# jaredhuling/oem

Measured on AMD Instinct MI355X. Metric: full-lambda-path solves/sec (n=1e6 p=100 lasso, 100 lambdas, tol 1e-10), higher is better.
Workload: dtype f64; 1 GPU; config 1: oem() lasso (penalty='elastic.net', alpha=1), dense Gaussian X~N(0,9), intercept, no standardize, 100-lambda path supplied, tol 1e-10 (README benchmark); n=1000000, p=100, nlambda=100, rows_per_gpu=1000000

## Files before the change

### include/oemgpu.h

```cpp
#ifndef OEMGPU_H
#define OEMGPU_H

#include <stdint.h>

#ifdef __cplusplus
extern "C" {
#endif

#define OEMGPU_OK              0
#define OEMGPU_ERR_ARG        -1
#define OEMGPU_ERR_NO_DEVICE  -2
#define OEMGPU_ERR_HIP        -3
#define OEMGPU_ERR_UNSUPPORTED -4
#define OEMGPU_ERR_INTERNAL   -5
#define OEMGPU_ERR_INTERRUPTED -6

enum {
    OEMGPU_ELASTIC_NET = 0, OEMGPU_LASSO = 1, OEMGPU_OLS = 2, OEMGPU_MCP = 3, OEMGPU_SCAD = 4,
    OEMGPU_MCP_NET = 5, OEMGPU_SCAD_NET = 6, OEMGPU_GRP_LASSO = 7, OEMGPU_GRP_LASSO_NET = 8,
    OEMGPU_GRP_MCP = 9, OEMGPU_GRP_SCAD = 10, OEMGPU_GRP_MCP_NET = 11, OEMGPU_GRP_SCAD_NET = 12,
    OEMGPU_SPARSE_GRP_LASSO = 13, OEMGPU_NPENALTIES = 14
};

typedef struct oemgpu_opts {
// ... 103 lines not shown
int oemgpu_fit_dense_rm_dev(oemgpu_ctx *ctx, const void *x_dev, int32_t dtype, int64_t n, int64_t ldr, int32_t p, const double *y_dev,
                            int32_t standardize, int32_t intercept, const oemgpu_opts *o,
                            double *beta, double *lambda_out, int32_t *niter, double *loss, double *d);
int oemgpu_selftest_gram_rm_plan(int64_t n, int32_t p, int32_t num_cu, int64_t *out );

int oemgpu_fit_dense_multi_dev(oemgpu_ctx *ctx, const double *x_dev, int64_t n, int64_t ld, int32_t p,
                               const double *y_dev, int64_t y_rs, int64_t y_cs, int32_t m,
                               int32_t standardize, int32_t intercept, const oemgpu_opts *o,
                               double *beta, double *lambda_out, int32_t *niter, double *loss, double *d, int32_t *route);
int oemgpu_fit_dense_multi_rm_dev(oemgpu_ctx *ctx, const void *x_dev, int32_t dtype, int64_t n, int64_t ldr, int32_t p,
                                  const double *y_dev, int64_t y_rs, int64_t y_cs, int32_t m,
                                  int32_t standardize, int32_t intercept, const oemgpu_opts *o,
                                  double *beta, double *lambda_out, int32_t *niter, double *loss, double *d, int32_t *route);
int oemgpu_selftest_multi_plan(int64_t n, int32_t p, int32_t m, int32_t npen, int32_t layout, int32_t num_cu, int64_t *out );
int oemgpu_selftest_multi_moments_dev(oemgpu_ctx *ctx, const void *x_dev, int32_t dtype, int64_t n, int64_t ld, int32_t p,
                                      const double *y_dev, int64_t y_rs, int64_t y_cs, int32_t m, double *moments_out_dev);

int oemgpu_fit_dense_weighted_dev(oemgpu_ctx *ctx, const double *x_dev, int64_t n, int64_t ld, int32_t p, const double *y_dev,
                                  const double *weights_dev, int32_t standardize, int32_t intercept, const oemgpu_opts *opts,
                                  double *beta, double *lambda_out, int32_t *niter, double *loss, double *d);

int oemgpu_fit_xtx_dev(oemgpu_ctx *ctx, const double *xtx_dev, const double *xty_dev, int32_t p,
                       const double *scale_factor, const oemgpu_opts *o,
                       double *beta, double *lambda_out, int32_t *niter, double *loss, double *d);

int oemgpu_last_shift_advised(oemgpu_ctx *ctx);

int oemgpu_xval_dense_dev(oemgpu_ctx *ctx, const double *x_dev, int64_t n, int64_t ld, int32_t p, const double *y_dev,
                          const double *weights_dev , const int32_t *foldid_dev, int32_t nfolds, int32_t standardize, int32_t intercept,
                          int32_t type_measure, const oemgpu_opts *o,
                          double *beta, double *lambda_out, int32_t *niter, double *loss, double *d,
                          double *cvm, double *cvsd);

int64_t oemgpu_xval_moments_len(int32_t p, int32_t nfolds, int32_t weighted);
int oemgpu_xval_fold_moments_dev(oemgpu_ctx *ctx, const double *x_dev, int64_t n_local, int64_t ld, int32_t p, const double *y_dev,
                                 const double *weights_dev , const int32_t *foldid_dev, int32_t nfolds, const oemgpu_opts *o,
                                 double *fold_moments_dev, int64_t *fold_n);
int oemgpu_xval_solve_folds_dev(oemgpu_ctx *ctx, const double *fold_moments_dev, const int64_t *fold_n_total, int64_t n_local, int32_t p,
                                int32_t nfolds, int32_t weighted, int32_t standardize, int32_t intercept, const oemgpu_opts *o,
                                double *beta, double *lambda_out, int32_t *niter, double *loss, double *d);
int oemgpu_xval_cv_triples_dev(oemgpu_ctx *ctx, int64_t n_local, int32_t p, int32_t nfolds, int32_t weighted, int32_t type_measure,
                               const oemgpu_opts *o, double *triples);
int oemgpu_xval_merge(const double *triples, int32_t nsets, const oemgpu_opts *o, double *cvm, double *cvsd);

int oemgpu_selftest_xval_cv_error_dev(oemgpu_ctx *ctx, const double *x_dev, int64_t n, int64_t ld, int32_t p, const double *y_dev,
                                      const double *weights_dev , const int32_t *foldid_dev, int32_t nfolds,
                                      const double *coef, int32_t npen, int32_t nl, int32_t type_measure, double *cvm, double *cvsd,
                                      double *triples );
int oemgpu_cv_fold_fits_dev(oemgpu_ctx *ctx, const double *x_dev, int64_t n, int64_t ld, int32_t p, const double *y_dev,
                            const int32_t *foldid_dev, int32_t nfolds, int32_t standardize, int32_t intercept, const oemgpu_opts *o,
                            double *beta, double *lambda_out, int32_t *niter, double *loss, double *d, int64_t *fold_n);
int oemgpu_cv_score_dev(oemgpu_ctx *ctx, int64_t n, int32_t p, int32_t nfolds, const double *coef, int32_t npen, int32_t nl,
                        const int32_t *ncol, int32_t type_measure, double *triples, double *predmat_dev );
int oemgpu_selftest_cv_score_dev(oemgpu_ctx *ctx, const double *x_dev, int64_t n, int64_t ld, int32_t p, const double *y_dev,
                                 const int32_t *foldid_dev, int32_t nfolds, const double *coef, int32_t npen, int32_t nl,
                                 const int32_t *ncol, int32_t type_measure, double *triples, double *predmat_dev );
int oemgpu_xval_dense_rm_dev(oemgpu_ctx *ctx, const void *x_dev, int32_t dtype, int64_t n, int64_t ldr, int32_t p, const double *y_dev,
                             const double *weights_dev , const int32_t *foldid_dev, int32_t nfolds, int32_t standardize,
                             int32_t intercept, int32_t type_measure, const oemgpu_opts *o,
                             double *beta, double *lambda_out, int32_t *niter, double *loss, double *d,
                             double *cvm, double *cvsd);
int oemgpu_cv_fold_fits_rm_dev(oemgpu_ctx *ctx, const void *x_dev, int32_t dtype, int64_t n, int64_t ldr, int32_t p, const double *y_dev,
                               const int32_t *foldid_dev, int32_t nfolds, int32_t standardize, int32_t intercept, const oemgpu_opts *o,
                               double *beta, double *lambda_out, int32_t *niter, double *loss, double *d, int64_t *fold_n);
int oemgpu_selftest_fold_gather_rm_dev(oemgpu_ctx *ctx, const void *x_dev, int32_t dtype, int64_t n, int64_t ldr, int32_t p,
                                       const double *y_dev, const int32_t *foldid_dev, int32_t nfolds, double *xo_dev, int64_t ldo,
                                       double *yo_dev, int64_t *fold_n, int64_t *fold_start);
int oemgpu_selftest_xval_cv_plan(int64_t n, int32_t p, int32_t nfolds, int32_t npen, int32_t nl, int32_t num_cu, int64_t *out );

int oemgpu_xval_dense_multi_dev(oemgpu_ctx *ctx, const double *x_dev, int64_t n, int64_t ld, int32_t p,
                                const double *y_dev, int64_t y_rs, int64_t y_cs, int32_t m,
                                const int32_t *foldid_dev, int32_t nfolds, int32_t standardize, int32_t intercept,
                                int32_t type_measure, const oemgpu_opts *o,
                                double *beta, double *lambda_out, int32_t *niter, double *loss, double *d,
                                double *cvm, double *cvsd, int32_t *route);
int oemgpu_xval_dense_multi_rm_dev(oemgpu_ctx *ctx, const void *x_dev, int32_t dtype, int64_t n, int64_t ldr, int32_t p,
                                   const double *y_dev, int64_t y_rs, int64_t y_cs, int32_t m,
                                   const int32_t *foldid_dev, int32_t nfolds, int32_t standardize, int32_t intercept,
                                   int32_t type_measure, const oemgpu_opts *o,
                                   double *beta, double *lambda_out, int32_t *niter, double *loss, double *d,
                                   double *cvm, double *cvsd, int32_t *route);
#define OEMGPU_XVM_NPHASES 6
int oemgpu_last_xval_multi_timings(double *ms );
#define OEMGPU_XVM_PLAN_LEN 20
int oemgpu_selftest_xval_multi_plan(int64_t n, int32_t p, int32_t nfolds, int32_t m, int32_t npen, int32_t nl, int32_t num_cu,
                                    int64_t *out );
int oemgpu_selftest_xval_multi_fold_moments_dev(oemgpu_ctx *ctx, const void *x_dev, int32_t dtype, int64_t n, int64_t ld, int32_t p,
                                                const double *y_dev, int64_t y_rs, int64_t y_cs, int32_t m,
                                                const int32_t *foldid_dev, int32_t nfolds, double *moments_out_dev);

int oemgpu_last_eigen_info(oemgpu_ctx *ctx, int32_t *steps, int32_t *capped);

enum {
    OEMGPU_ENGINE_NONE = 0,
    OEMGPU_ENGINE_ROWS = 1,
    OEMGPU_ENGINE_COOP = 2,
    OEMGPU_ENGINE_ROWCOOP = 3,
    OEMGPU_ENGINE_SYMCOOP = 4,
    OEMGPU_ENGINE_LAUNCHES = 5,
    OEMGPU_ENGINE_WCOOP = 6,
    OEMGPU_ENGINE_WRES = 7,
    OEMGPU_ENGINE_WSTREAM = 8,
    OEMGPU_ENGINE_WLAUNCHES = 9,
    OEMGPU_ENGINE_SPARSE_WIDE = 10
};
int oemgpu_last_path_engine(oemgpu_ctx *ctx, int32_t *engine, int32_t *persistent_fallbacks);
int oemgpu_last_host_path_engine(int32_t *engine);
int oemgpu_last_placement(oemgpu_ctx *ctx);

int oemgpu_last_path_rounds(oemgpu_ctx *ctx, int64_t *short_rounds, int64_t *rounds);

int oemgpu_last_shift_in_effect(oemgpu_ctx *ctx);

int oemgpu_eig_max_dev(oemgpu_ctx *ctx, const double *a_dev, int32_t p, double *lambda_max);

#define OEMGPU_T_SHIFT   0
#define OEMGPU_T_MOMENTS 1
#define OEMGPU_T_FINAL   2
#define OEMGPU_T_EIGPATH 3
#define OEMGPU_T_GRAMK   4
#define OEMGPU_T_FOLDORDER 5
#define OEMGPU_T_PATHCYC 6
#define OEMGPU_T_PATHTICKS 7
#define OEMGPU_NTIMERS   8
int oemgpu_last_timings(oemgpu_ctx *ctx, double *ms );
int oemgpu_set_timing(oemgpu_ctx *ctx, int32_t on);

void oemgpu_row_split(int64_t n, int32_t G, int32_t g, int64_t *r0, int64_t *r1);

#define OEMGPU_NHOSTSTATS 9
int oemgpu_last_host_stats(double *out );

void oemgpu_release_cache(void);

int oemgpu_selftest_wcoop_sizing(int32_t n, int32_t p, int32_t npen, int32_t num_cu);

int oemgpu_selftest_plan(int32_t p, int32_t q, int32_t semantics, int32_t intercept, const oemgpu_opts *o, int32_t has_scale, int32_t nbatch,
                         int64_t wide_n, int32_t num_cu, int32_t *engine, int64_t *frame_bytes, int64_t *reserved_bytes,
                         int64_t *scratch_need_doubles, int64_t *scratch_have_doubles);

int oemgpu_selftest_gram_plan(int64_t n, int32_t p, int32_t num_cu, int64_t *out );

enum {
    OEMGPU_GRAM_FORM_TRI = 0,
    OEMGPU_GRAM_FORM_RING_SADDR = 1,
    OEMGPU_GRAM_FORM_RING_LANE = 2,
    OEMGPU_GRAM_FORM_SB = 3,
    OEMGPU_GRAM_FORM_WD3 = 4,
    OEMGPU_GRAM_FORM_WD4 = 5,
    OEMGPU_GRAM_FORM_WD_UNITS = 6,
    OEMGPU_GRAM_FORM_BLK = 7
};
int oemgpu_selftest_gram_form(int64_t n, int64_t ld, int32_t p, int32_t aligned, int32_t num_cu, int64_t *out );

int oemgpu_fit_logistic_dense(const double *x, int64_t n, int32_t p, const double *y, int32_t standardize, int32_t intercept,
                              int32_t hessian_full, int32_t irls_maxit, double irls_tol, const oemgpu_opts *opts,
                              double *beta, double *lambda_out, int32_t *niter, double *loss, double *d);
int oemgpu_fit_logistic_dense_dev(oemgpu_ctx *ctx, const double *x_dev, int64_t n, int64_t ld, int32_t p, const double *y_dev,
                                  int32_t standardize, int32_t intercept, int32_t hessian_full, int32_t irls_maxit, double irls_tol,
                                  const oemgpu_opts *opts, double *beta, double *lambda_out, int32_t *niter, double *loss, double *d);
int oemgpu_fit_logistic_dense_fold_dev(oemgpu_ctx *ctx, const double *x_dev, int64_t n, int64_t ld, int32_t p, const double *y_dev,
                                       const int32_t *foldid_dev, int32_t nfolds, int32_t leave_out, int32_t standardize, int32_t intercept,
                                       int32_t hessian_full, int32_t irls_maxit, double irls_tol, const oemgpu_opts *opts,
                                       double *beta, double *lambda_out, int32_t *niter, double *loss, double *d);
int oemgpu_logistic_cv_score_dev(oemgpu_ctx *ctx, const double *x_dev, int64_t n, int64_t ld, int32_t p, const double *y_dev, double y_hi,
                                 const int32_t *foldid_dev, int32_t nfolds, const double *coef, int32_t ncol, double *sums, int64_t *counts,
                                 double *predmat_dev);
int oemgpu_selftest_cv_score_plan(int64_t n, int32_t p, int32_t ncol, int32_t num_cu, int64_t *out );
int oemgpu_logistic_cv_auc_dev(oemgpu_ctx *ctx, const double *predmat_dev, int64_t n, int32_t ncol, const double *y_dev, double y_hi,
                               const int32_t *foldid_dev, int32_t nfolds, int64_t *u, int64_t *n1, int64_t *n0);
int oemgpu_selftest_cv_auc_plan(int64_t n, int32_t nfolds, int32_t ncol, int32_t num_cu, int64_t longest_fold, int64_t *out );
int oemgpu_selftest_logistic_plan(int64_t n, int32_t p, int32_t intercept, int32_t hessian_full, int32_t num_cu, int64_t *out );
int oemgpu_fit_logistic_dense_rm_dev(oemgpu_ctx *ctx, const void *x_dev, int32_t dtype, int64_t n, int64_t ldr, int32_t p, const double *y_dev,
                                     int32_t standardize, int32_t intercept, int32_t hessian_full, int32_t irls_maxit, double irls_tol,
                                     const oemgpu_opts *opts, double *beta, double *lambda_out, int32_t *niter, double *loss, double *d);
int oemgpu_fit_logistic_dense_fold_rm_dev(oemgpu_ctx *ctx, const void *x_dev, int32_t dtype, int64_t n, int64_t ldr, int32_t p, const double *y_dev,
                                          const int32_t *foldid_dev, int32_t nfolds, int32_t leave_out, int32_t standardize, int32_t intercept,
                                          int32_t hessian_full, int32_t irls_maxit, double irls_tol, const oemgpu_opts *opts,
                                          double *beta, double *lambda_out, int32_t *niter, double *loss, double *d);
int oemgpu_logistic_cv_score_rm_dev(oemgpu_ctx *ctx, const void *x_dev, int32_t dtype, int64_t n, int64_t ldr, int32_t p, const double *y_dev,
                                    double y_hi, const int32_t *foldid_dev, int32_t nfolds, const double *coef, int32_t ncol, double *sums,
                                    int64_t *counts, double *predmat_dev);
int oemgpu_selftest_logistic_rm_plan(int64_t n, int32_t p, int32_t dtype, int32_t intercept, int32_t num_cu, int64_t *out );
int oemgpu_fit_logistic_sparse(int64_t n, int32_t p, const int64_t *colptr, const int32_t *rowidx, const double *values, const double *y,
                               int32_t standardize, int32_t intercept, int32_t irls_maxit, double irls_tol, const oemgpu_opts *opts,
                               double *beta, double *lambda_out, int32_t *niter, double *loss, double *d);
int oemgpu_selftest_logistic_sparse_plan(int64_t n, int32_t p, int64_t nnz, int32_t intercept, int32_t num_cu, int64_t *out );
typedef struct oemgpu_sparse_x oemgpu_sparse_x;
int oemgpu_sparse_x_create(oemgpu_ctx *ctx, int64_t n, int32_t p, const int64_t *colptr, const int32_t *rowidx, const double *values,
                           oemgpu_sparse_x **out);
void oemgpu_sparse_x_destroy(oemgpu_sparse_x *x);
int64_t oemgpu_sparse_x_bytes(const oemgpu_sparse_x *x);
#define OEMGPU_SPARSE_CSC 0
#define OEMGPU_SPARSE_CSR 1
#define OEMGPU_I32 0
#define OEMGPU_I64 1
int oemgpu_sparse_x_create_dev(oemgpu_ctx *ctx, int64_t n, int32_t p, int32_t layout, const void *ptr_dev, int32_t ptr_dtype,
                               const void *idx_dev, int32_t idx_dtype, const void *val_dev, int32_t val_dtype, int64_t nnz,
                               oemgpu_sparse_x **out);
int oemgpu_selftest_sparse_build_plan(int64_t n, int32_t p, int64_t nnz, int32_t layout, int32_t num_cu, int64_t *out );
int oemgpu_sparse_x_export(const oemgpu_sparse_x *x, int64_t *colptr, int32_t *rowidx, double *val, int64_t *rowptr, int32_t *ccol,
                           double *cval, int32_t *cptr);
int oemgpu_sparse_x_dims(const oemgpu_sparse_x *x, int64_t *out );
int oemgpu_last_sparse_build_timings(double *ms );
int oemgpu_fit_sparse_res(oemgpu_ctx *ctx, const oemgpu_sparse_x *x, const double *y_dev, int32_t standardize, int32_t intercept,
                          const oemgpu_opts *opts, double *beta, double *lambda_out, int32_t *niter, double *loss, double *d);
int oemgpu_xval_sparse_res(oemgpu_ctx *ctx, const oemgpu_sparse_x *x, const double *y_dev, const int32_t *foldid_dev, int32_t nfolds,
                           int32_t standardize, int32_t intercept, int32_t type_measure, const oemgpu_opts *opts, double *beta,
                           double *lambda_out, int32_t *niter, double *loss, double *d, double *cvm, double *cvsd);
int oemgpu_fit_logistic_sparse_fold_res(oemgpu_ctx *ctx, const oemgpu_sparse_x *x, const double *y_dev, const int32_t *foldid_dev, int32_t nfolds,
                                        int32_t leave_out, int32_t standardize, int32_t intercept, int32_t irls_maxit, double irls_tol,
                                        const oemgpu_opts *opts, double *beta, double *lambda_out, int32_t *niter, double *loss, double *d);
int oemgpu_fit_sparse_wide_res(oemgpu_ctx *ctx, const oemgpu_sparse_x *x, const double *y_dev, int32_t standardize, const oemgpu_opts *opts,
                               double *beta, double *lambda_out, int32_t *niter, double *loss, double *d);
int oemgpu_selftest_sparse_wide_plan(int64_t n, int32_t p, int64_t nnz, int64_t longest_row, int64_t longest_col, int32_t num_cu,
                                     int64_t *out );
int oemgpu_fit_sparse_wide_fold_res(oemgpu_ctx *ctx, const oemgpu_sparse_x *x, const double *y_dev, const int32_t *foldid_dev, int32_t nfolds,
                                    int32_t leave_out, int32_t standardize, const oemgpu_opts *opts, double *beta, double *lambda_out,
                                    int32_t *niter, double *loss, double *d, int64_t *kept);
enum { OEMGPU_SPW_PASS_ROWS = 0, OEMGPU_SPW_PASS_COLS = 1, OEMGPU_SPW_PASS_STATS = 2, OEMGPU_SPW_PASS_LOSS = 3 };
int oemgpu_selftest_sparse_wide_pass(oemgpu_ctx *ctx, const oemgpu_sparse_x *x, int32_t pass, int32_t row_lanes, int32_t col_lanes,
                                     const int32_t *foldid_dev, int32_t nfolds, int32_t leave_out, int32_t standardize, double scale,
                                     const double *in_dev, const double *coef_dev, int32_t ncoef, double *out_dev, double *out2_dev,
                                     double *stats_dev, int64_t *info , int32_t *long_rows, int32_t *long_cols);
int oemgpu_cv_sparse_wide_score_res(oemgpu_ctx *ctx, const oemgpu_sparse_x *x, const double *y_dev, const int32_t *foldid_dev, int32_t nfolds,
                                    const double *coef, int32_t npen, int32_t nl, const int32_t *ncol, int32_t type_measure, double *triples,
                                    double *predmat_dev );
int oemgpu_selftest_cv_sparse_wide_score_plan(int64_t n, int32_t p, int32_t nfolds, int32_t npen, int32_t nl, int32_t num_cu,
                                              int64_t *out );
int oemgpu_logistic_cv_score_sparse_res(oemgpu_ctx *ctx, const oemgpu_sparse_x *x, const double *y_dev, double y_hi, const int32_t *foldid_dev,
                                        int32_t nfolds, const double *coef, int32_t ncol, double *sums, int64_t *counts, double *predmat_dev);
int oemgpu_selftest_logistic_sparse_res_plan(int64_t n, int32_t p, int64_t nnz, int32_t intercept, int32_t num_cu, int64_t *out );
int oemgpu_cv_sparse_fold_fits_res(oemgpu_ctx *ctx, const oemgpu_sparse_x *x, const double *y_dev, const int32_t *foldid_dev, int32_t nfolds,
                                   int32_t standardize, int32_t intercept, const oemgpu_opts *opts,
                                   double *beta, double *lambda_out, int32_t *niter, double *loss, double *d, int64_t *fold_n);
int oemgpu_cv_sparse_score_res(oemgpu_ctx *ctx, int64_t n, int32_t p, int32_t nfolds, const double *coef, int32_t npen, int32_t nl,
                               const int32_t *ncol, int32_t type_measure, double *triples, double *predmat_dev );
int oemgpu_selftest_cv_sparse_score(oemgpu_ctx *ctx, const oemgpu_sparse_x *x, const double *y_dev, const int32_t *foldid_dev, int32_t nfolds,
                                    const double *coef, int32_t npen, int32_t nl, const int32_t *ncol, int32_t type_measure, double *triples,
                                    double *predmat_dev );
int oemgpu_selftest_cv_sparse_plan(int64_t n, int32_t p, int64_t nnz, int32_t nfolds, int32_t npen, int32_t nl, int32_t num_cu,
                                   int64_t *out );
int oemgpu_selftest_csc_plan(int64_t n, int32_t p, int64_t *out );
int oemgpu_last_logistic_stats(double *out );

int oemgpu_predict_dev(oemgpu_ctx *ctx, const double *x_dev, int64_t n, int64_t ld, int32_t p, const double *coef, int32_t ncol, int32_t type,
                       double *out_dev);
int oemgpu_predict_rm_dev(oemgpu_ctx *ctx, const void *x_dev, int32_t dtype, int64_t n, int64_t ldr, int32_t p, const double *coef, int32_t ncol,
                          int32_t type, double *out_dev);
int oemgpu_predict_sparse_res(oemgpu_ctx *ctx, const oemgpu_sparse_x *x, const double *coef, int32_t ncol, int32_t type, double *out_dev);
int oemgpu_selftest_predict_plan(int64_t n, int32_t p, int32_t ncol, int32_t layout, int32_t num_cu, int64_t *out );

int oemgpu_selftest_hold_cus(oemgpu_ctx *ctx, int32_t blocks, double ms);

int oemgpu_selftest_group_permutation(const oemgpu_opts *o, int32_t q, int32_t *perm);

int oemgpu_selftest_symcoop_owners(int32_t q, int32_t num_cu, const int32_t *runs, int32_t nruns, int32_t *owner_c0, int32_t *owner_n, int32_t *frag,
                                   int32_t *nowners, int32_t *split);

int oemgpu_selftest_coop_slots(int32_t num_cu, int32_t W, int32_t ninst, int32_t calls, int32_t *bases, int32_t *peak);

int oemgpu_selftest_sympk_gemv(oemgpu_ctx *ctx, const double *xx_dev, int32_t q, const double *vec_dev, double *out_dev, int32_t reps,
                               double *us_per_product);

void        oemgpu_reload_switches(void);
const char *oemgpu_switch_names(void);

const char *oemgpu_last_error(void);
const char *oemgpu_version(void);
int         oemgpu_device_count(void);

#ifdef __cplusplus
}
#endif
#endif
```

### oem_amd/_lib.py

```python
import ctypes as C
import os
from pathlib import Path

_HERE = Path(__file__).resolve().parent
LIB_PATH = Path(os.environ.get("OEMGPU_LIB", _HERE / "liboemgpu.so"))

_dp = C.POINTER(C.c_double)
_ip = C.POINTER(C.c_int32)

PENALTIES = ["elastic.net", "lasso", "ols", "mcp", "scad", "mcp.net", "scad.net",
             "grp.lasso", "grp.lasso.net", "grp.mcp", "grp.scad", "grp.mcp.net",
             "grp.scad.net", "sparse.grp.lasso"]

OEMGPU_SEM_DENSE, OEMGPU_SEM_BIG = 0, 1
OEMGPU_F64, OEMGPU_F32 = 0, 1
OEMGPU_SPARSE_CSC, OEMGPU_SPARSE_CSR = 0, 1
OEMGPU_I32, OEMGPU_I64 = 0, 1
RM_P_MAX = 1024
ERR_INTERRUPTED = -6
NHOSTSTATS = 9
NTIMERS = 8
T_SHIFT, T_MOMENTS, T_FINAL, T_EIGPATH, T_GRAMK = 0, 1, 2, 3, 4


# ... 34 lines not shown
                                                 C.c_int32, C.c_int32, C.c_double, C.POINTER(OemgpuOpts)] + _OUT),
    "oemgpu_fit_logistic_dense_fold_dev": (C.c_int, [C.c_void_p, C.c_void_p, C.c_int64, C.c_int64, C.c_int32, C.c_void_p, C.c_void_p, C.c_int32,
                                                      C.c_int32, C.c_int32, C.c_int32, C.c_int32, C.c_int32, C.c_double, C.POINTER(OemgpuOpts)] + _OUT),
    "oemgpu_logistic_cv_score_dev": (C.c_int, [C.c_void_p, C.c_void_p, C.c_int64, C.c_int64, C.c_int32, C.c_void_p, C.c_double, C.c_void_p, C.c_int32,
                                                _dp, C.c_int32, _dp, C.POINTER(C.c_int64), C.c_void_p]),
    "oemgpu_fit_logistic_dense_rm_dev": (C.c_int, [C.c_void_p, C.c_void_p, C.c_int32, C.c_int64, C.c_int64, C.c_int32, C.c_void_p, C.c_int32, C.c_int32,
                                                    C.c_int32, C.c_int32, C.c_double, C.POINTER(OemgpuOpts)] + _OUT),
    "oemgpu_fit_logistic_dense_fold_rm_dev": (C.c_int, [C.c_void_p, C.c_void_p, C.c_int32, C.c_int64, C.c_int64, C.c_int32, C.c_void_p, C.c_void_p,
                                                         C.c_int32, C.c_int32, C.c_int32, C.c_int32, C.c_int32, C.c_int32, C.c_double,
                                                         C.POINTER(OemgpuOpts)] + _OUT),
    "oemgpu_logistic_cv_score_rm_dev": (C.c_int, [C.c_void_p, C.c_void_p, C.c_int32, C.c_int64, C.c_int64, C.c_int32, C.c_void_p, C.c_double, C.c_void_p,
                                                   C.c_int32, _dp, C.c_int32, _dp, C.POINTER(C.c_int64), C.c_void_p]),
    "oemgpu_selftest_logistic_rm_plan": (C.c_int, [C.c_int64, C.c_int32, C.c_int32, C.c_int32, C.c_int32, C.POINTER(C.c_int64)]),
    "oemgpu_selftest_cv_score_plan": (C.c_int, [C.c_int64, C.c_int32, C.c_int32, C.c_int32, C.POINTER(C.c_int64)]),
    "oemgpu_logistic_cv_auc_dev": (C.c_int, [C.c_void_p, C.c_void_p, C.c_int64, C.c_int32, C.c_void_p, C.c_double, C.c_void_p, C.c_int32,
                                              C.POINTER(C.c_int64), C.POINTER(C.c_int64), C.POINTER(C.c_int64)]),
    "oemgpu_selftest_cv_auc_plan": (C.c_int, [C.c_int64, C.c_int32, C.c_int32, C.c_int32, C.c_int64, C.POINTER(C.c_int64)]),
    "oemgpu_selftest_logistic_plan": (C.c_int, [C.c_int64, C.c_int32, C.c_int32, C.c_int32, C.c_int32, C.POINTER(C.c_int64)]),
    "oemgpu_fit_logistic_sparse": (C.c_int, [C.c_int64, C.c_int32, C.c_void_p, C.c_void_p, C.c_void_p, C.c_void_p, C.c_int32, C.c_int32, C.c_int32, C.c_double,
                                              C.POINTER(OemgpuOpts)] + _OUT),
    "oemgpu_selftest_logistic_sparse_plan": (C.c_int, [C.c_int64, C.c_int32, C.c_int64, C.c_int32, C.c_int32, C.POINTER(C.c_int64)]),
    "oemgpu_selftest_logistic_sparse_res_plan": (C.c_int, [C.c_int64, C.c_int32, C.c_int64, C.c_int32, C.c_int32, C.POINTER(C.c_int64)]),
    "oemgpu_sparse_x_create": (C.c_int, [C.c_void_p, C.c_int64, C.c_int32, C.c_void_p, C.c_void_p, C.c_void_p, C.POINTER(C.c_void_p)]),
    "oemgpu_sparse_x_destroy": (None, [C.c_void_p]),
    "oemgpu_sparse_x_bytes": (C.c_int64, [C.c_void_p]),
    "oemgpu_sparse_x_create_dev": (C.c_int, [C.c_void_p, C.c_int64, C.c_int32, C.c_int32, C.c_void_p, C.c_int32, C.c_void_p, C.c_int32, C.c_void_p,
                                             C.c_int32, C.c_int64, C.POINTER(C.c_void_p)]),
    "oemgpu_selftest_sparse_build_plan": (C.c_int, [C.c_int64, C.c_int32, C.c_int64, C.c_int32, C.c_int32, C.POINTER(C.c_int64)]),
    "oemgpu_sparse_x_export": (C.c_int, [C.c_void_p] + [C.c_void_p] * 7),
    "oemgpu_sparse_x_dims": (C.c_int, [C.c_void_p, C.POINTER(C.c_int64)]),
    "oemgpu_last_sparse_build_timings": (C.c_int, [_dp]),
    "oemgpu_fit_sparse_res": (C.c_int, [C.c_void_p, C.c_void_p, C.c_void_p, C.c_int32, C.c_int32, C.POINTER(OemgpuOpts)] + _OUT),
    "oemgpu_xval_sparse_res": (C.c_int, [C.c_void_p, C.c_void_p, C.c_void_p, C.c_void_p, C.c_int32, C.c_int32, C.c_int32, C.c_int32,
                                         C.POINTER(OemgpuOpts)] + _OUT + [_dp, _dp]),
    "oemgpu_fit_logistic_sparse_fold_res": (C.c_int, [C.c_void_p, C.c_void_p, C.c_void_p, C.c_void_p, C.c_int32, C.c_int32, C.c_int32, C.c_int32, C.c_int32,
                                                       C.c_double, C.POINTER(OemgpuOpts)] + _OUT),
    "oemgpu_logistic_cv_score_sparse_res": (C.c_int, [C.c_void_p, C.c_void_p, C.c_void_p, C.c_double, C.c_void_p, C.c_int32, _dp, C.c_int32, _dp,
                                                       C.POINTER(C.c_int64), C.c_void_p]),
    "oemgpu_predict_dev": (C.c_int, [C.c_void_p, C.c_void_p, C.c_int64, C.c_int64, C.c_int32, _dp, C.c_int32, C.c_int32, C.c_void_p]),
    "oemgpu_predict_rm_dev": (C.c_int, [C.c_void_p, C.c_void_p, C.c_int32, C.c_int64, C.c_int64, C.c_int32, _dp, C.c_int32, C.c_int32, C.c_void_p]),
    "oemgpu_predict_sparse_res": (C.c_int, [C.c_void_p, C.c_void_p, _dp, C.c_int32, C.c_int32, C.c_void_p]),
    "oemgpu_selftest_predict_plan": (C.c_int, [C.c_int64, C.c_int32, C.c_int32, C.c_int32, C.c_int32, C.POINTER(C.c_int64)]),
    "oemgpu_selftest_csc_plan": (C.c_int, [C.c_int64, C.c_int32, C.POINTER(C.c_int64)]),
    "oemgpu_last_logistic_stats": (C.c_int, [_dp]),
    "oemgpu_fit_xtx": (C.c_int, [_dp, _dp, C.c_int32, _dp, C.POINTER(OemgpuOpts)] + _OUT),
    "oemgpu_fit_big": (C.c_int, [C.POINTER(_dp), C.POINTER(C.c_int64), C.c_int32, C.c_int32, C.POINTER(_dp), C.c_int32,
                                 C.c_int32, C.POINTER(OemgpuOpts)] + _OUT),
    "oemgpu_create": (C.c_void_p, [C.c_int32, C.c_void_p]),
    "oemgpu_destroy": (None, [C.c_void_p]),
    "oemgpu_synchronize": (C.c_int, [C.c_void_p]),
    "oemgpu_shift_sums_dev": (C.c_int, [C.c_void_p, C.c_void_p, C.c_int64, C.c_int64, C.c_int32, C.c_void_p, C.c_void_p]),
    "oemgpu_moments_dev": (C.c_int, [C.c_void_p, C.c_void_p, C.c_int64, C.c_int64, C.c_int32, C.c_void_p, C.c_void_p, C.c_void_p]),
    "oemgpu_sum_in_order_dev": (C.c_int, [C.c_void_p, C.c_void_p, C.c_int32, C.c_int64, C.c_void_p]),
    "oemgpu_solve_moments_dev": (C.c_int, [C.c_void_p, C.c_void_p, C.c_void_p, C.c_int32, C.c_int32, C.c_int32, C.c_int32,
                                           C.POINTER(OemgpuOpts)] + _OUT),
    "oemgpu_fit_dense_dev": (C.c_int, [C.c_void_p, C.c_void_p, C.c_int64, C.c_int64, C.c_int32, C.c_void_p, C.c_int32,
                                       C.c_int32, C.POINTER(OemgpuOpts)] + _OUT),
    "oemgpu_shift_sums_rm_dev": (C.c_int, [C.c_void_p, C.c_void_p, C.c_int32, C.c_int64, C.c_int64, C.c_int32, C.c_void_p, C.c_void_p]),
    "oemgpu_moments_rm_dev": (C.c_int, [C.c_void_p, C.c_void_p, C.c_int32, C.c_int64, C.c_int64, C.c_int32, C.c_void_p, C.c_void_p, C.c_void_p]),
    "oemgpu_fit_dense_rm_dev": (C.c_int, [C.c_void_p, C.c_void_p, C.c_int32, C.c_int64, C.c_int64, C.c_int32, C.c_void_p, C.c_int32,
                                          C.c_int32, C.POINTER(OemgpuOpts)] + _OUT),
    "oemgpu_selftest_gram_rm_plan": (C.c_int, [C.c_int64, C.c_int32, C.c_int32, C.POINTER(C.c_int64)]),
    "oemgpu_fit_dense_multi_dev": (C.c_int, [C.c_void_p, C.c_void_p, C.c_int64, C.c_int64, C.c_int32, C.c_void_p, C.c_int64, C.c_int64, C.c_int32,
                                             C.c_int32, C.c_int32, C.POINTER(OemgpuOpts)] + _OUT + [_ip]),
    "oemgpu_fit_dense_multi_rm_dev": (C.c_int, [C.c_void_p, C.c_void_p, C.c_int32, C.c_int64, C.c_int64, C.c_int32, C.c_void_p, C.c_int64, C.c_int64,
                                                C.c_int32, C.c_int32, C.c_int32, C.POINTER(OemgpuOpts)] + _OUT + [_ip]),
    "oemgpu_selftest_multi_plan": (C.c_int, [C.c_int64, C.c_int32, C.c_int32, C.c_int32, C.c_int32, C.c_int32, C.POINTER(C.c_int64)]),
    "oemgpu_selftest_multi_moments_dev": (C.c_int, [C.c_void_p, C.c_void_p, C.c_int32, C.c_int64, C.c_int64, C.c_int32, C.c_void_p, C.c_int64, C.c_int64,
                                                    C.c_int32, C.c_void_p]),
    "oemgpu_xval_dense_multi_dev": (C.c_int, [C.c_void_p, C.c_void_p, C.c_int64, C.c_int64, C.c_int32, C.c_void_p, C.c_int64, C.c_int64, C.c_int32,
                                              C.c_void_p, C.c_int32, C.c_int32, C.c_int32, C.c_int32, C.POINTER(OemgpuOpts)] + _OUT + [_dp, _dp, _ip]),
    "oemgpu_xval_dense_multi_rm_dev": (C.c_int, [C.c_void_p, C.c_void_p, C.c_int32, C.c_int64, C.c_int64, C.c_int32, C.c_void_p, C.c_int64, C.c_int64,
                                                 C.c_int32, C.c_void_p, C.c_int32, C.c_int32, C.c_int32, C.c_int32, C.POINTER(OemgpuOpts)] + _OUT +
                                       [_dp, _dp, _ip]),
    "oemgpu_last_xval_multi_timings": (C.c_int, [_dp]),
    "oemgpu_selftest_xval_multi_plan": (C.c_int, [C.c_int64, C.c_int32, C.c_int32, C.c_int32, C.c_int32, C.c_int32, C.c_int32, C.POINTER(C.c_int64)]),
    "oemgpu_selftest_xval_multi_fold_moments_dev": (C.c_int, [C.c_void_p, C.c_void_p, C.c_int32, C.c_int64, C.c_int64, C.c_int32, C.c_void_p, C.c_int64,
                                                              C.c_int64, C.c_int32, C.c_void_p, C.c_int32, C.c_void_p]),
    "oemgpu_fit_xtx_dev": (C.c_int, [C.c_void_p, C.c_void_p, C.c_void_p, C.c_int32, _dp, C.POINTER(OemgpuOpts)] + _OUT),
    "oemgpu_last_shift_in_effect": (C.c_int, [C.c_void_p]),
    "oemgpu_last_shift_advised": (C.c_int, [C.c_void_p]),
    "oemgpu_last_eigen_info": (C.c_int, [C.c_void_p, C.POINTER(C.c_int32), C.POINTER(C.c_int32)]),
    "oemgpu_last_path_engine": (C.c_int, [C.c_void_p, C.POINTER(C.c_int32), C.POINTER(C.c_int32)]),
    "oemgpu_last_host_path_engine": (C.c_int, [C.POINTER(C.c_int32)]),
    "oemgpu_last_placement": (C.c_int, [C.c_void_p]),
    "oemgpu_last_path_rounds": (C.c_int, [C.c_void_p, C.POINTER(C.c_int64), C.POINTER(C.c_int64)]),
    "oemgpu_fit_sparse": (C.c_int, [C.c_int64, C.c_int32, C.c_void_p, C.c_void_p, C.c_void_p, C.c_void_p, C.c_int32, C.c_int32,
                                    C.POINTER(OemgpuOpts)] + _OUT),
    "oemgpu_fit_sparse_wide_res": (C.c_int, [C.c_void_p, C.c_void_p, C.c_void_p, C.c_int32, C.POINTER(OemgpuOpts)] + _OUT),
    "oemgpu_selftest_sparse_wide_plan": (C.c_int, [C.c_int64, C.c_int32, C.c_int64, C.c_int64, C.c_int64, C.c_int32, C.POINTER(C.c_int64)]),
    "oemgpu_fit_sparse_wide_fold_res": (C.c_int, [C.c_void_p, C.c_void_p, C.c_void_p, C.c_void_p, C.c_int32, C.c_int32, C.c_int32,
                                                  C.POINTER(OemgpuOpts)] + _OUT + [C.POINTER(C.c_int64)]),
    "oemgpu_selftest_sparse_wide_pass": (C.c_int, [C.c_void_p, C.c_void_p, C.c_int32, C.c_int32, C.c_int32, C.c_void_p, C.c_int32, C.c_int32, C.c_int32,
                                                   C.c_double, C.c_void_p, C.c_void_p, C.c_int32, C.c_void_p, C.c_void_p, C.c_void_p,
                                                   C.POINTER(C.c_int64), C.c_void_p, C.c_void_p]),
    "oemgpu_cv_sparse_wide_score_res": (C.c_int, [C.c_void_p, C.c_void_p, C.c_void_p, C.c_void_p, C.c_int32, _dp, C.c_int32, C.c_int32, _ip,
                                                  C.c_int32, _dp, C.c_void_p]),
    "oemgpu_selftest_cv_sparse_wide_score_plan": (C.c_int, [C.c_int64, C.c_int32, C.c_int32, C.c_int32, C.c_int32, C.c_int32, C.POINTER(C.c_int64)]),
    "oemgpu_xval_dense": (C.c_int, [C.c_void_p, C.c_int64, C.c_int32, C.c_void_p, C.c_void_p, C.c_void_p, C.c_int32, C.c_int32, C.c_int32,
                                    C.c_int32, C.POINTER(OemgpuOpts)] + _OUT + [_dp, _dp]),
    "oemgpu_xval_sparse": (C.c_int, [C.c_int64, C.c_int32, C.c_void_p, C.c_void_p, C.c_void_p, C.c_void_p, C.c_void_p, C.c_int32, C.c_int32, C.c_int32,
                                     C.c_int32, C.POINTER(OemgpuOpts)] + _OUT + [_dp, _dp]),
    "oemgpu_last_xval_sparse_timings": (C.c_int, [_dp]),
    "oemgpu_selftest_xval_sparse_plan": (C.c_int, [C.c_int64, C.c_int32, C.c_int64, C.c_int32, C.c_int32, C.c_int32, C.c_int32, C.POINTER(C.c_int64)]),
    "oemgpu_selftest_xval_sparse_fold_moments": (C.c_int, [C.c_int64, C.c_int32, C.c_void_p, C.c_void_p, C.c_void_p, C.c_void_p, C.c_void_p, C.c_int32, _dp]),
    "oemgpu_selftest_xval_sparse_cv_error": (C.c_int, [C.c_int64, C.c_int32, C.c_void_p, C.c_void_p, C.c_void_p, C.c_void_p, C.c_void_p, C.c_int32, _dp,
                                                       C.c_int32, C.c_int32, C.c_int32, _dp, _dp, _dp]),
    "oemgpu_xval_dense_dev": (C.c_int, [C.c_void_p, C.c_void_p, C.c_int64, C.c_int64, C.c_int32, C.c_void_p, C.c_void_p, C.c_void_p, C.c_int32,
                                        C.c_int32, C.c_int32, C.c_int32, C.POINTER(OemgpuOpts)] + _OUT + [_dp, _dp]),
    "oemgpu_xval_moments_len": (C.c_int64, [C.c_int32, C.c_int32, C.c_int32]),
    "oemgpu_xval_fold_moments_dev": (C.c_int, [C.c_void_p, C.c_void_p, C.c_int64, C.c_int64, C.c_int32, C.c_void_p, C.c_void_p, C.c_void_p,
                                               C.c_int32, C.POINTER(OemgpuOpts), C.c_void_p, C.POINTER(C.c_int64)]),
    "oemgpu_xval_solve_folds_dev": (C.c_int, [C.c_void_p, C.c_void_p, C.POINTER(C.c_int64), C.c_int64, C.c_int32, C.c_int32, C.c_int32,
                                              C.c_int32, C.c_int32, C.POINTER(OemgpuOpts)] + _OUT),
    "oemgpu_xval_cv_triples_dev": (C.c_int, [C.c_void_p, C.c_int64, C.c_int32, C.c_int32, C.c_int32, C.c_int32, C.POINTER(OemgpuOpts), _dp]),
    "oemgpu_selftest_xval_cv_error_dev": (C.c_int, [C.c_void_p, C.c_void_p, C.c_int64, C.c_int64, C.c_int32, C.c_void_p, C.c_void_p, C.c_void_p, C.c_int32,
                                                    _dp, C.c_int32, C.c_int32, C.c_int32, _dp, _dp, _dp]),
    "oemgpu_selftest_xval_cv_plan": (C.c_int, [C.c_int64, C.c_int32, C.c_int32, C.c_int32, C.c_int32, C.c_int32, C.POINTER(C.c_int64)]),
    "oemgpu_cv_fold_fits_dev": (C.c_int, [C.c_void_p, C.c_void_p, C.c_int64, C.c_int64, C.c_int32, C.c_void_p, C.c_void_p, C.c_int32, C.c_int32,
                                          C.c_int32, C.POINTER(OemgpuOpts)] + _OUT + [C.POINTER(C.c_int64)]),
    "oemgpu_cv_score_dev": (C.c_int, [C.c_void_p, C.c_int64, C.c_int32, C.c_int32, _dp, C.c_int32, C.c_int32, _ip, C.c_int32, _dp,
                                      C.c_void_p]),
    "oemgpu_selftest_cv_score_dev": (C.c_int, [C.c_void_p, C.c_void_p, C.c_int64, C.c_int64, C.c_int32, C.c_void_p, C.c_void_p, C.c_int32, _dp,
                                               C.c_int32, C.c_int32, _ip, C.c_int32, _dp, C.c_void_p]),
    "oemgpu_xval_dense_rm_dev": (C.c_int, [C.c_void_p, C.c_void_p, C.c_int32, C.c_int64, C.c_int64, C.c_int32, C.c_void_p, C.c_void_p, C.c_void_p,
                                           C.c_int32, C.c_int32, C.c_int32, C.c_int32, C.POINTER(OemgpuOpts)] + _OUT + [_dp, _dp]),
    "oemgpu_cv_fold_fits_rm_dev": (C.c_int, [C.c_void_p, C.c_void_p, C.c_int32, C.c_int64, C.c_int64, C.c_int32, C.c_void_p, C.c_void_p, C.c_int32,
                                             C.c_int32, C.c_int32, C.POINTER(OemgpuOpts)] + _OUT + [C.POINTER(C.c_int64)]),
    "oemgpu_selftest_fold_gather_rm_dev": (C.c_int, [C.c_void_p, C.c_void_p, C.c_int32, C.c_int64, C.c_int64, C.c_int32, C.c_void_p, C.c_void_p,
                                                     C.c_int32, C.c_void_p, C.c_int64, C.c_void_p, C.POINTER(C.c_int64), C.POINTER(C.c_int64)]),
    "oemgpu_cv_sparse_fold_fits_res": (C.c_int, [C.c_void_p, C.c_void_p, C.c_void_p, C.c_void_p, C.c_int32, C.c_int32, C.c_int32,
                                                 C.POINTER(OemgpuOpts)] + _OUT + [C.POINTER(C.c_int64)]),
    "oemgpu_cv_sparse_score_res": (C.c_int, [C.c_void_p, C.c_int64, C.c_int32, C.c_int32, _dp, C.c_int32, C.c_int32, _ip, C.c_int32, _dp,
                                             C.c_void_p]),
    "oemgpu_selftest_cv_sparse_score": (C.c_int, [C.c_void_p, C.c_void_p, C.c_void_p, C.c_void_p, C.c_int32, _dp, C.c_int32, C.c_int32, _ip,
                                                  C.c_int32, _dp, C.c_void_p]),
    "oemgpu_selftest_cv_sparse_plan": (C.c_int, [C.c_int64, C.c_int32, C.c_int64, C.c_int32, C.c_int32, C.c_int32, C.c_int32, C.POINTER(C.c_int64)]),
    "oemgpu_xval_merge": (C.c_int, [_dp, C.c_int32, C.POINTER(OemgpuOpts), _dp, _dp]),
    "oemgpu_eig_max_dev": (C.c_int, [C.c_void_p, C.c_void_p, C.c_int32, _dp]),
    "oemgpu_last_timings": (C.c_int, [C.c_void_p, _dp]),
    "oemgpu_set_timing": (C.c_int, [C.c_void_p, C.c_int32]),
    "oemgpu_row_split": (None, [C.c_int64, C.c_int32, C.c_int32, C.POINTER(C.c_int64), C.POINTER(C.c_int64)]),
    "oemgpu_last_host_stats": (C.c_int, [_dp]),
    "oemgpu_release_cache": (None, []),
    "oemgpu_selftest_hold_cus": (C.c_int, [C.c_void_p, C.c_int32, C.c_double]),
    "oemgpu_selftest_group_permutation": (C.c_int, [C.c_void_p, C.c_int32, C.POINTER(C.c_int32)]),
    "oemgpu_selftest_symcoop_owners": (C.c_int, [C.c_int32, C.c_int32, C.POINTER(C.c_int32), C.c_int32, C.POINTER(C.c_int32), C.POINTER(C.c_int32),
                                       C.POINTER(C.c_int32), C.POINTER(C.c_int32), C.POINTER(C.c_int32)]),
    "oemgpu_selftest_coop_slots": (C.c_int, [C.c_int32, C.c_int32, C.c_int32, C.c_int32, C.POINTER(C.c_int32), C.POINTER(C.c_int32)]),
    "oemgpu_selftest_sympk_gemv": (C.c_int, [C.c_void_p, C.c_void_p, C.c_int32, C.c_void_p, C.c_void_p, C.c_int32, C.POINTER(C.c_double)]),
    "oemgpu_selftest_wcoop_sizing": (C.c_int, [C.c_int32, C.c_int32, C.c_int32, C.c_int32]),
    "oemgpu_selftest_gram_plan": (C.c_int, [C.c_int64, C.c_int32, C.c_int32, C.POINTER(C.c_int64)]),
    "oemgpu_selftest_gram_form": (C.c_int, [C.c_int64, C.c_int64, C.c_int32, C.c_int32, C.c_int32, C.POINTER(C.c_int64)]),
    "oemgpu_selftest_plan": (C.c_int, [C.c_int32, C.c_int32, C.c_int32, C.c_int32, C.c_void_p, C.c_int32, C.c_int32, C.c_int64, C.c_int32,
                             C.POINTER(C.c_int32), C.POINTER(C.c_int64), C.POINTER(C.c_int64), C.POINTER(C.c_int64), C.POINTER(C.c_int64)]),
    "oemgpu_reload_switches": (None, []),
    "oemgpu_switch_names": (C.c_char_p, []),
    "oemgpu_last_error": (C.c_char_p, []),
    "oemgpu_version": (C.c_char_p, []),
    "oemgpu_device_count": (C.c_int, []),
}
EXPORTS = sorted(_SIGS)


def lib():
    global _lib
    if _lib is None:
        try:
            import torch
        except ImportError:
            pass
        if not LIB_PATH.exists():
            raise OSError(f"{LIB_PATH} is missing: build it with `python -m oem_amd.build` "
                          "(oem_amd has no CPU fallback)")
        L = C.CDLL(str(LIB_PATH))
        for name, (res, args) in _SIGS.items():
            fn = getattr(L, name)
            fn.restype = res
            fn.argtypes = args
        _lib = L
    return _lib


_env_seen = None


def sync_switches():
    global _env_seen
    cur = tuple(sorted((k, v) for k, v in os.environ.items() if k.startswith(("OEM_", "OEMGPU_"))))
    if cur != _env_seen:
        _env_seen = cur
        reload_switches()


def reload_switches():
    if _lib is not None:
        _lib.oemgpu_reload_switches()


def check(rc):
    if rc != 0:
        raise OemgpuError(rc, lib().oemgpu_last_error().decode())


def host_stats():
    out = (C.c_double * NHOSTSTATS)()
    check(lib().oemgpu_last_host_stats(out))
    keys = ["call_ms", "upload_moments_ms", "solve_ms", "bytes_staged", "devices", "row_blocks", "resident", "allocations", "host_staged_handovers"]
    return dict(zip(keys, list(out)))


def sums_len(p):
    return 2 * (p + 1) + 2


def moments_len(p):
    return (p + 2) * (p + 2)
```

### oem_amd/csrc/api.hip

```cpp
#include "paths.hpp"
#include "dense_src.hpp"
#include "multi.hpp"
#include "logistic.hpp"

#include <atomic>
#include <cmath>
#include <cstdarg>
#include <cstdio>
#include <cstring>
#include <functional>
#include <mutex>
#include <string>
#include <thread>
#include <vector>

namespace oemgpu {

static std::mutex g_sw_mu;
static std::atomic<const Switches *> g_sw{nullptr};
static unsigned g_sw_generation = 0;
static const Switches *sw_parse()
{
    Switches *t = new Switches();
    auto read = [](const char *name, Switch &v) {
// ... 23 lines not shown
}

static thread_local char g_err[512] = "";
void set_error(const char *fmt, ...)
{
    va_list ap;
    va_start(ap, fmt);
    vsnprintf(g_err, sizeof g_err, fmt, ap);
    va_end(ap);
}

int lds_limit_once(const void *fn, size_t bytes)
{
    struct Key { const void *fn; int dev; size_t bytes; };
    static std::mutex mu;
    static std::vector<Key> seen;
    int dev = 0;
    (void)hipGetDevice(&dev);
    {
        std::lock_guard<std::mutex> lk(mu);
        for (const Key &k : seen) if (k.fn == fn && k.dev == dev && k.bytes >= bytes) return 0;
    }
    OEM_HIP(hipFuncSetAttribute(fn, hipFuncAttributeMaxDynamicSharedMemorySize, (int)bytes));
    std::lock_guard<std::mutex> lk(mu);
    for (Key &k : seen) if (k.fn == fn && k.dev == dev) { if (k.bytes < bytes) k.bytes = bytes; return 0; }
    seen.push_back(Key{fn, dev, bytes});
    return 0;
}

}

using namespace oemgpu;

namespace oemgpu {

int ctx_reserve(oemgpu_ctx *c, size_t bytes)
{
    if (bytes <= c->ws_bytes) return 0;
    if (c->ws) { OEM_HIP(hipStreamSynchronize(c->stream)); OEM_HIP(hipFree(c->ws)); c->ws = nullptr; c->ws_bytes = 0; }
    bytes = bytes + bytes / 8 + (1 << 20);
    OEM_HIP(hipMalloc((void **)&c->ws, bytes)); ++g_alloc_count;
    c->ws_bytes = bytes;
    return 0;
}

int ctx_grow(oemgpu_ctx *c, char **buf, size_t *have, size_t bytes)
{
    if (bytes <= *have) return 0;
    if (*buf) { OEM_HIP(hipStreamSynchronize(c->stream)); OEM_HIP(hipFree(*buf)); *buf = nullptr; *have = 0; }
    OEM_HIP(hipMalloc((void **)buf, bytes)); ++g_alloc_count;
    *have = bytes;
    return 0;
}

int set_device(const oemgpu_ctx *c) { OEM_HIP(hipSetDevice(c->device)); return 0; }

static std::mutex g_cache_mu;
static std::vector<oemgpu_ctx *> g_cache;

oemgpu_ctx *ctx_acquire(int device)
{
    if (device < 0) { if (hipGetDevice(&device) != hipSuccess) device = 0; }
    {
        std::lock_guard<std::mutex> lk(g_cache_mu);
        for (oemgpu_ctx *c : g_cache)
            if (c->device == device && !c->busy) { c->busy = true; (void)hipSetDevice(device); return c; }
    }
    oemgpu_ctx *c = oemgpu_create(device, nullptr);
    if (!c) return nullptr;
    c->cached = true; c->busy = true;
    std::lock_guard<std::mutex> lk(g_cache_mu);
    g_cache.push_back(c);
    return c;
}

void ctx_release(oemgpu_ctx *c)
{
    if (!c) return;
    size_t keep = c->hbm_total / 8;
    if (sw().OEMGPU_CACHE_KEEP_BYTES.set && sw().OEMGPU_CACHE_KEEP_BYTES.num >= 0) keep = (size_t)sw().OEMGPU_CACHE_KEEP_BYTES.num;
    if (c->xres_bytes > keep || c->aux_bytes > keep || c->pack_bytes > keep) {
        (void)hipSetDevice(c->device);
        if (c->xres_bytes > keep) { (void)hipFree(c->xres); c->xres = nullptr; c->xres_bytes = 0; }
        if (c->aux_bytes > keep) { (void)hipFree(c->aux); c->aux = nullptr; c->aux_bytes = 0; }
        if (c->pack_bytes > keep) { (void)hipFree(c->pack_buf); c->pack_buf = nullptr; c->pack_bytes = 0; }
    }
    std::lock_guard<std::mutex> lk(g_cache_mu);
    c->busy = false;
}

int ctx_pinned(oemgpu_ctx *c, size_t bytes)
{
    if (bytes <= c->pinned_bytes) return 0;
    if (c->pinned) { OEM_HIP(hipStreamSynchronize(c->stream)); OEM_HIP(hipHostFree(c->pinned)); c->pinned = nullptr; c->pinned_bytes = 0; }
    bytes = bytes + bytes / 8 + 4096;
    OEM_HIP(hipHostMalloc((void **)&c->pinned, bytes, hipHostMallocDefault)); ++g_alloc_count;
    c->pinned_bytes = bytes;
    return 0;
}

}

namespace {

int check_opts(const oemgpu_opts *o, int p, int ngroupvars_expected)
{
    if (!o) { set_error("opts is NULL"); return OEMGPU_ERR_ARG; }
    if (o->npen < 1 || !o->penalty) { set_error("at least one penalty is required"); return OEMGPU_ERR_ARG; }
    bool any_grp = false;
    for (int k = 0; k < o->npen; ++k) {
        if (o->penalty[k] < 0 || o->penalty[k] >= OEMGPU_NPENALTIES) { set_error("unknown penalty code %d", o->penalty[k]); return OEMGPU_ERR_ARG; }
        any_grp |= pen_is_grp(o->penalty[k]);
    }
    if (p < 2) { set_error("x must have at least two columns"); return OEMGPU_ERR_ARG; }
    if (nl_of(o) < 1) { set_error("nlambda must be a positive integer"); return OEMGPU_ERR_ARG; }
    if (!(o->lambda_user && o->nlambda_user > 0) && !(o->lambda_min_ratio > 0.0 && o->lambda_min_ratio < 1.0)) {
        set_error("lambda.min.ratio must be between 0 and 1"); return OEMGPU_ERR_ARG;
    }
    if (o->maxit <= 0) { set_error("maxit and irls.maxit should be positive"); return OEMGPU_ERR_ARG; }
    if (o->tol < 0) { set_error("tol and irls.tol should be nonnegative"); return OEMGPU_ERR_ARG; }
    if (!o->penalty_factor) { set_error("penalty.factor must have same length as number of columns in x"); return OEMGPU_ERR_ARG; }
    if (any_grp) {
        if (!o->groups || o->ngroupvars != ngroupvars_expected) {
            set_error("If any group penalty is used groups must have same length as number of columns in x");
            return OEMGPU_ERR_ARG;
        }
        if (!o->unique_groups || o->ngroups < 1) { set_error("unique_groups is empty"); return OEMGPU_ERR_ARG; }
        if (o->n_group_weights > 0 && o->n_group_weights != o->ngroups) {
            set_error("group.weights must have same length as the number of groups"); return OEMGPU_ERR_ARG;
        }
    }
    return 0;
}

}

int oemgpu::check_opts_export(const oemgpu_opts *o, int p, int ngroupvars_expected) { return check_opts(o, p, ngroupvars_expected); }

#ifdef OEM_HOST_TIMING
namespace { struct HostT { double acc[8] = {0}; long n = 0; ~HostT() { if (n) fprintf(stderr, "host timing over %ld calls (us): entry->moments enqueued %.2f | ->path enqueued %.2f | ->copy enqueued %.2f | ->synced %.2f | ->unpacked/returned %.2f\n", n, acc[0] / n, acc[1] / n, acc[2] / n, acc[3] / n, acc[4] / n); } } g_ht; }
double oemgpu::g_tp[6];
#endif
namespace oemgpu {
__global__ __launch_bounds__(256) void sum_in_order_kernel(const double *__restrict__ parts, int nparts, size_t len, double *__restrict__ out)
{
    for (size_t i = (size_t)blockIdx.x * blockDim.x + threadIdx.x; i < len; i += (size_t)gridDim.x * blockDim.x) {
        double s = parts[i];
        for (int r = 1; r < nparts; ++r) s += parts[(size_t)r * len + i];
        out[i] = s;
    }
}

int shard_moments(oemgpu_ctx *c, const GramPlan &pl, const double *x, int64_t n, int64_t ld, const double *y,
                  const double *sums, double *tpart, double *vpart, double *moments)
{
    {
        Timer t(c, OEMGPU_T_GRAMK);
        int rc = launch_gram(c->stream, pl, x, n, ld, y, sums, tpart, vpart);
        if (rc) return rc;
    }
    return launch_moments_reduce(c->stream, pl, tpart, vpart, moments);
}

static_assert(GRAM_RM_P_MAX == OEMGPU_RM_P_MAX, "the header's limit is the kernel's");

int dense_src_check(const char *who, const DenseSrc &X, int64_t n, int32_t p)
{
    if (X.colmajor()) {
        if (X.ld < n) { set_error("%s: ld < n", who); return OEMGPU_ERR_ARG; }
        return 0;
    }
    if (X.dtype != OEMGPU_F64 && X.dtype != OEMGPU_F32) { set_error("%s: dtype is neither OEMGPU_F64 nor OEMGPU_F32", who); return OEMGPU_ERR_ARG; }
    if (X.ld < p) { set_error("%s: ldr < p", who); return OEMGPU_ERR_ARG; }
    const int el = X.dtype == OEMGPU_F32 ? 4 : 8;
    if ((uintptr_t)X.x % el) { set_error("%s: x_dev is not aligned to its %d-byte elements", who, el); return OEMGPU_ERR_ARG; }
    return 0;
}

int dense_src_shift_sums(hipStream_t s, const DenseSrc &X, int64_t n, int p, const double *y, double *sums)
{
    if (X.colmajor()) return launch_shift_sums(s, X.cm(), n, X.ld, p, y, sums);
    return launch_shift_sums_rm(s, X.x, X.dtype, n, X.ld, p, y, sums);
}

int dense_src_gather(hipStream_t s, const DenseSrc &X, int64_t n, int p, const double *y, const int32_t *foldid, int K, const int *pos,
                     double *xo, int64_t ldo, double *yo)
{
    if (X.colmajor()) return launch_gather_rows(s, X.cm(), n, X.ld, p, y, pos, xo, ldo, yo);
    return launch_gather_rows_rm(s, X.x, X.dtype, n, X.ld, p, y, foldid, K, pos, xo, ldo, yo);
}

static int rm_p_refusal(const char *who, int32_t p)
{
    if (p <= GRAM_RM_P_MAX) return 0;
    set_error("%s: the row-major pass takes p <= %d; larger p takes the column-major entry (oemgpu_fit_dense_dev / oemgpu_moments_dev)", who, GRAM_RM_P_MAX);
    return OEMGPU_ERR_UNSUPPORTED;
}

static int moment_plan_cus(const char *who, int num_cu, bool colmajor, int64_t n, int32_t p, MomentPlan *pl)
{
    Bump B;
    if (colmajor) {
        pl->cm = gram_plan(n, p, num_cu);
        B.take(pl->cm.tpart_doubles * 8); B.take(pl->cm.vpart_doubles * 8);
    } else {
        if (int rc = rm_p_refusal(who, p)) return rc;
        pl->rm = gram_rm_plan(n, p, num_cu);
        B.take(pl->rm.tpart_doubles * 8);
    }
    pl->scratch_bytes = B.off;
    return 0;
}

int dense_src_moment_plan(const char *who, const oemgpu_ctx *c, const DenseSrc &X, int64_t n, int32_t p, MomentPlan *pl)
{
    if (!X.colmajor()) if (int rc = rm_p_refusal(who, p)) return rc;
    return moment_plan_cus(who, c->num_cu, X.colmajor(), n, p, pl);
}

int dense_src_moments(oemgpu_ctx *c, const MomentPlan &pl, const DenseSrc &X, int64_t n, const double *y, const double *sums, char *scratch,
                      double *moments)
{
    double *tpart = (double *)scratch;
    if (X.colmajor()) {
        Bump B; B.take(pl.cm.tpart_doubles * 8);
        return shard_moments(c, pl.cm, X.cm(), n, X.ld, y, sums, tpart, (double *)(scratch + B.off), moments);
    }
    {
        Timer t(c, OEMGPU_T_GRAMK);
        int rc = launch_gram_rm(c->stream, pl.rm, X.x, X.dtype, n, X.ld, y, sums, tpart);
        if (rc) return rc;
    }
    return launch_gram_rm_reduce(c->stream, pl.rm, tpart, moments);
}

__global__ __launch_bounds__(256) void hold_cus_kernel(unsigned long long ticks, int *sink)
{
    extern __shared__ int hold_lds[];
    hold_lds[threadIdx.x] = (int)threadIdx.x;
    const unsigned long long t0 = __builtin_amdgcn_s_memrealtime();
    while (__builtin_amdgcn_s_memrealtime() - t0 < ticks) __builtin_amdgcn_s_sleep(32);
    if (hold_lds[threadIdx.x] == -1 && sink) *sink = 1;
}
}

#pragma GCC visibility push(default)
extern "C" {

void oemgpu_reload_switches(void) { sw_reload(); }

const char *oemgpu_switch_names(void)
{
#define OEM_SW_NAME(name) #name " "
    return OEM_SWITCH_TABLE(OEM_SW_NAME);
#undef OEM_SW_NAME
}

const char *oemgpu_last_error(void) { return g_err; }
const char *oemgpu_version(void) { return "oemgpu 0.1 (gfx950)"; }

int oemgpu_device_count(void)
{
    int n = 0;
    if (hipGetDeviceCount(&n) != hipSuccess) return 0;
    return n;
}

oemgpu_ctx *oemgpu_create(int32_t device, void *stream)
{
    int n = 0;
    if (hipGetDeviceCount(&n) != hipSuccess || n < 1) { set_error("no HIP device available (liboemgpu has no CPU fallback)"); return nullptr; }
    if (device < 0) { if (hipGetDevice(&device) != hipSuccess) device = 0; }
    if (device >= n) { set_error("device %d out of range (%d devices)", device, n); return nullptr; }
    hipDeviceProp_t prop;
    if (hipGetDeviceProperties(&prop, device) != hipSuccess) { set_error("hipGetDeviceProperties failed"); return nullptr; }
    if (strncmp(prop.gcnArchName, "gfx950", 6) != 0) {
        set_error("device %d is %s; liboemgpu is built for gfx950 only", device, prop.gcnArchName);
        return nullptr;
    }
    if (hipSetDevice(device) != hipSuccess) { set_error("hipSetDevice(%d) failed", device); return nullptr; }
    oemgpu_ctx *c = new oemgpu_ctx();
    c->device = device;
    c->num_cu = prop.multiProcessorCount;
    c->hbm_total = prop.totalGlobalMem;
    if (stream) { c->stream = (hipStream_t)stream; c->own_stream = false; }
    else {
        if (hipStreamCreateWithFlags(&c->stream, hipStreamNonBlocking) != hipSuccess) { set_error("hipStreamCreate failed"); delete c; return nullptr; }
        c->own_stream = true; ++g_alloc_count;
    }
    for (int i = 0; i < OEMGPU_NTIMERS; ++i) { c->ev_used[i] = false; c->ms[i] = 0.0; }
    return c;
}

void oemgpu_destroy(oemgpu_ctx *c)
{
    if (!c) return;
    (void)hipSetDevice(c->device);
    (void)hipStreamSynchronize(c->stream);
    if (c->ws) (void)hipFree(c->ws);
    if (c->pinned) (void)hipHostFree(c->pinned);
    if (c->pinned_in) (void)hipHostFree(c->pinned_in);
    if (c->aux) (void)hipFree(c->aux);
    if (c->xres) (void)hipFree(c->xres);
    if (c->blob_buf) (void)hipFree(c->blob_buf);
    if (c->pack_buf) (void)hipFree(c->pack_buf);
    if (c->perm_buf) (void)hipFree(c->perm_buf);
    if (c->abort_host) (void)hipHostFree(c->abort_host);
    if (c->acc) (void)hipFree(c->acc);
    for (oemgpu_lane &l : c->lanes) {
        for (int k = 0; k < 2; ++k) {
            if (l.slot[k]) (void)hipHostFree(l.slot[k]);
            if (l.slot_ev[k]) (void)hipEventDestroy(l.slot_ev[k]);
            if (l.blk_ev[k]) (void)hipEventDestroy(l.blk_ev[k]);
        }
        if (l.s) (void)hipStreamDestroy(l.s);
    }
    for (int k = 0; k < 2; ++k) if (c->done_ev[k]) (void)hipEventDestroy(c->done_ev[k]);
    if (c->xfer_ev) (void)hipEventDestroy(c->xfer_ev);
    if (c->xfer_host) (void)hipHostFree(c->xfer_host);
    for (oemgpu_ctx *k : c->kids) oemgpu_destroy(k);
    if (c->fork_ev) (void)hipEventDestroy(c->fork_ev);
    if (c->ev_made) for (int i = 0; i < 2 * OEMGPU_NTIMERS; ++i) (void)hipEventDestroy(c->ev[i]);
    if (c->xvs_ev_made) for (int i = 0; i <= OEMGPU_XVS_NPHASES; ++i) (void)hipEventDestroy(c->xvs_ev[i]);
    if (c->own_stream) (void)hipStreamDestroy(c->stream);
    delete c;
}

void oemgpu_release_cache(void)
{
    std::vector<oemgpu_ctx *> drop;
    {
        std::lock_guard<std::mutex> lk(g_cache_mu);
        std::vector<oemgpu_ctx *> keep;
        for (oemgpu_ctx *c : g_cache) (c->busy ? keep : drop).push_back(c);
        g_cache.swap(keep);
    }
    for (oemgpu_ctx *c : drop) oemgpu_destroy(c);
}

int oemgpu_synchronize(oemgpu_ctx *c)
{
    if (!c) { set_error("ctx is NULL"); return OEMGPU_ERR_ARG; }
    OEM_HIP(hipStreamSynchronize(c->stream));
    return 0;
}

int oemgpu_selftest_gram_plan(int64_t n, int32_t p, int32_t num_cu, int64_t *out)
{
    if (n < 1 || p < 1 || num_cu < 1 || !out) { set_error("selftest_gram_plan: bad argument"); return OEMGPU_ERR_ARG; }
    const GramPlan pl = gram_plan(n, p, num_cu);
    const int64_t n8 = pl.n8, n6 = pl.n6, n4 = pl.n4;
    out[0] = pl.ntc; out[1] = n8; out[2] = n6; out[3] = pl.nchunk; out[4] = pl.steps;
    out[5] = 64 * (n8 * (n8 - 1) / 2) + 48 * n8 * n6 + 32 * n8 * n4 + 24 * n6 * n4 + 36 * n8 + 24 * n6 + 12 * n4;
    out[7] = n4;
    if (pl.wd) { out[1] = out[2] = out[7] = -1; out[5] = pl.wd == 4 ? 136 * pl.wd_units + 128 * pl.wd_units * (pl.wd_units - 1) : 80; }
    out[6] = (int64_t)pl.ntc * (pl.ntc + 1) / 2;
    const GramPlan bd = gram_plan_bound(n, p, num_cu);
    for (int64_t d = 1; d <= 4096 && n / d >= 1; d = d < 16 ? d + 1 : d * 2) {
        for (int64_t m : {n / d, n / d + 1, n - n / (d + 1)}) {
            if (m < 1 || m > n) continue;
            const GramPlan q = gram_plan(m, p, num_cu);
            if (q.tpart_doubles > bd.tpart_doubles || q.vpart_doubles > bd.vpart_doubles) {
                set_error("selftest_gram_plan: the plan of %lld rows (%d chunks) does not fit the bound for %lld (%d chunks)", (long long)m, q.nchunk, (long long)n, bd.nchunk);
                return OEMGPU_ERR_INTERNAL;
            }
        }
    }
    return 0;
}

int oemgpu_selftest_gram_form(int64_t n, int64_t ld, int32_t p, int32_t aligned, int32_t num_cu, int64_t *out)
{
    if (n < 1 || ld < 1 || p < 1 || num_cu < 1 || !out) { set_error("selftest_gram_form: bad argument"); return OEMGPU_ERR_ARG; }
    const GramForm f = gram_form(gram_plan(n, p, num_cu), n, ld, aligned != 0);
    out[0] = f.form; out[1] = f.strips;
    return 0;
}

int oemgpu_selftest_hold_cus(oemgpu_ctx *c, int32_t blocks, double ms)
{
    if (!c || blocks < 1 || blocks > 4096 || !(ms > 0.0) || ms > 30000.0) { set_error("hold_cus: bad argument"); return OEMGPU_ERR_ARG; }
    if (set_device(c)) return OEMGPU_ERR_HIP;
    const int lds = 150 * 1024;
    OEM_HIP(hipFuncSetAttribute(reinterpret_cast<const void *>(&hold_cus_kernel), hipFuncAttributeMaxDynamicSharedMemorySize, lds));
    hipLaunchKernelGGL(hold_cus_kernel, dim3(blocks), dim3(256), lds, c->stream, (unsigned long long)(ms * 1e5), (int *)nullptr);
    OEM_HIP(hipGetLastError());
    return 0;
}

int oemgpu_sum_in_order_dev(oemgpu_ctx *c, const double *parts_dev, int32_t nparts, int64_t len, double *out_dev)
{
    if (!c || !parts_dev || !out_dev || nparts < 1 || len < 1) { set_error("sum_in_order: bad argument"); return OEMGPU_ERR_ARG; }
    if (set_device(c)) return OEMGPU_ERR_HIP;
    const int blocks = (int)std::min<int64_t>((len + 255) / 256, 2048);
    hipLaunchKernelGGL(sum_in_order_kernel, dim3(blocks), dim3(256), 0, c->stream, parts_dev, (int)nparts, (size_t)len, out_dev);
    OEM_HIP(hipGetLastError());
    return 0;
}

int oemgpu_selftest_sympk_gemv(oemgpu_ctx *c, const double *xx_dev, int32_t q, const double *vec_dev, double *out_dev, int32_t reps, double *us_per_product)
{
    if (!c || !xx_dev || !vec_dev || !out_dev || q <= 4096 || reps < 0 || reps > 100000) { set_error("selftest_sympk_gemv: bad argument (q > 4096)"); return OEMGPU_ERR_ARG; }
    if (set_device(c)) return OEMGPU_ERR_HIP;
    if (ctx_grow(c, &c->pack_buf, &c->pack_bytes, sympk_doubles(q) * sizeof(double))) return OEMGPU_ERR_HIP;
    return sympk_gemv_probe(c->stream, xx_dev, q, (double *)c->pack_buf, vec_dev, out_dev, reps, us_per_product);
}

int oemgpu_set_timing(oemgpu_ctx *c, int32_t on)
{
    if (!c) { set_error("ctx is NULL"); return OEMGPU_ERR_ARG; }
    if (set_device(c)) return OEMGPU_ERR_HIP;
    if (on && !c->ev_made) {
        for (int i = 0; i < 2 * OEMGPU_NTIMERS; ++i) OEM_HIP(hipEventCreate(&c->ev[i]));
        c->ev_made = true;
    }
    c->timing = on != 0;
    return 0;
}

int oemgpu_last_timings(oemgpu_ctx *c, double *ms)
{
    if (!c || !ms) { set_error("NULL argument"); return OEMGPU_ERR_ARG; }
    OEM_HIP(hipStreamSynchronize(c->stream));
    for (int i = 0; i < OEMGPU_NTIMERS; ++i) {
        ms[i] = 0.0;
        if (c->ev_made && c->ev_used[i]) {
            float f = 0.f;
            if (hipEventElapsedTime(&f, c->ev[2 * i], c->ev[2 * i + 1]) == hipSuccess) ms[i] = f;
        }
    }
    ms[OEMGPU_T_PATHCYC] = c->diag[0];
    ms[OEMGPU_T_PATHTICKS] = c->diag[1];
    return 0;
}

static int src_args_check(const char *who, const oemgpu_ctx *c, const DenseSrc &X, int64_t n, int32_t p, const void *y_dev, bool outputs)
{
    if (!c || !X.x || !y_dev || !outputs) { set_error("%s: NULL argument", who); return OEMGPU_ERR_ARG; }
    if (n < 1 || p < 1) { set_error("%s: bad n / p (n >= 1, p >= 1)", who); return OEMGPU_ERR_ARG; }
    return dense_src_check(who, X, n, p);
}

static int shift_sums_src(const char *who, oemgpu_ctx *c, const DenseSrc &X, int64_t n, int32_t p, const double *y_dev, double *sums_dev)
{
    if (int rc = src_args_check(who, c, X, n, p, y_dev, sums_dev != nullptr)) return rc;
    if (set_device(c)) return OEMGPU_ERR_HIP;
    Timer t(c, OEMGPU_T_SHIFT);
    return dense_src_shift_sums(c->stream, X, n, p, y_dev, sums_dev);
}

int oemgpu_shift_sums_dev(oemgpu_ctx *c, const double *x_dev, int64_t n, int64_t ld, int32_t p, const double *y_dev,
                          double *sums_dev)
{
    return shift_sums_src("shift_sums", c, dense_src_cm(x_dev, ld), n, p, y_dev, sums_dev);
}

int oemgpu_shift_sums_rm_dev(oemgpu_ctx *c, const void *x_dev, int32_t dtype, int64_t n, int64_t ldr, int32_t p, const double *y_dev,
                             double *sums_dev)
{
    return shift_sums_src("shift_sums_rm", c, dense_src_rm(x_dev, dtype, ldr), n, p, y_dev, sums_dev);
}

static int moments_src(const char *who, oemgpu_ctx *c, const DenseSrc &X, int64_t n, int32_t p, const double *y_dev, const double *sums_dev,
                       double *moments_dev)
{
    if (int rc = src_args_check(who, c, X, n, p, y_dev, moments_dev != nullptr)) return rc;
    MomentPlan pl;
    if (int rc = dense_src_moment_plan(who, c, X, n, p, &pl)) return rc;
    if (set_device(c)) return OEMGPU_ERR_HIP;
    if (ctx_reserve(c, pl.scratch_bytes)) return OEMGPU_ERR_HIP;
    Timer t(c, OEMGPU_T_MOMENTS);
    return dense_src_moments(c, pl, X, n, y_dev, sums_dev, c->ws, moments_dev);
}

int oemgpu_moments_dev(oemgpu_ctx *c, const double *x_dev, int64_t n, int64_t ld, int32_t p, const double *y_dev,
                       const double *sums_dev, double *moments_dev)
{
    return moments_src("moments", c, dense_src_cm(x_dev, ld), n, p, y_dev, sums_dev, moments_dev);
}

int oemgpu_moments_rm_dev(oemgpu_ctx *c, const void *x_dev, int32_t dtype, int64_t n, int64_t ldr, int32_t p, const double *y_dev,
                          const double *sums_dev, double *moments_dev)
{
    return moments_src("moments_rm", c, dense_src_rm(x_dev, dtype, ldr), n, p, y_dev, sums_dev, moments_dev);
}

static int run_paths_parts(oemgpu_ctx *c, Bump B, const double *xx, const double *xy, const double *st, int p, int q, int sem, int standardize, int intercept,
                           const oemgpu_opts *o, double *beta, double *lambda_out, int32_t *niter, double *loss, double *d,
                           const WideArgs *wd, const double *lmax_xy);

static int solve_moments_impl(oemgpu_ctx *c, const double *moments_dev, const double *sums_dev, int32_t p,
                              int32_t semantics, int32_t standardize, int32_t intercept, const oemgpu_opts *o,
                              double *beta, double *lambda_out, int32_t *niter, double *loss, double *d, const double *wpatch,
                              const PathExtras *ex = nullptr, const double *lmax_xy = nullptr, size_t extra_ws = 0, double *big_xy_std = nullptr);

int oemgpu_solve_moments_dev(oemgpu_ctx *c, const double *moments_dev, const double *sums_dev, int32_t p,
                             int32_t semantics, int32_t standardize, int32_t intercept, const oemgpu_opts *o,
                             double *beta, double *lambda_out, int32_t *niter, double *loss, double *d)
{
    return solve_moments_impl(c, moments_dev, sums_dev, p, semantics, standardize, intercept, o, beta, lambda_out, niter, loss, d, nullptr);
}

static int solve_moments_impl(oemgpu_ctx *c, const double *moments_dev, const double *sums_dev, int32_t p,
                              int32_t semantics, int32_t standardize, int32_t intercept, const oemgpu_opts *o,
                              double *beta, double *lambda_out, int32_t *niter, double *loss, double *d, const double *wpatch,
                              const PathExtras *ex, const double *lmax_xy, size_t extra_ws, double *big_xy_std)
{
    if (!c || !moments_dev || !beta || !lambda_out || !niter || !loss || !d) { set_error("solve_moments: NULL argument"); return OEMGPU_ERR_ARG; }
    if (semantics != OEMGPU_SEM_DENSE && semantics != OEMGPU_SEM_BIG && semantics != OEMGPU_SEM_XVAL) { set_error("unknown semantics %d", semantics); return OEMGPU_ERR_ARG; }
    const int q = p + ((semantics != OEMGPU_SEM_DENSE && intercept) ? 1 : 0);
    int rc = check_opts(o, p, q);
    if (rc) return rc;
    if (semantics == OEMGPU_SEM_BIG && o->compute_loss) {
        set_error("compute.loss is not available for big.oem: the reference expression is ill-formed (src/oem_big.h:899-921)");
        return OEMGPU_ERR_UNSUPPORTED;
    }
    if (set_device(c)) return OEMGPU_ERR_HIP;
    Bump B;
    const size_t a_xx = B.take((size_t)q * q * 8), a_xy = B.take((size_t)q * 8), a_st = B.take((size_t)stats_len(p) * 8);
    size_t base = 0;
    if ((const char *)moments_dev >= c->ws && (const char *)moments_dev < c->ws + c->ws_bytes)
        base = ((const char *)moments_dev - c->ws) + (size_t)oemgpu_moments_len(p) * 8;
    if (sums_dev && (const char *)sums_dev >= c->ws && (const char *)sums_dev < c->ws + c->ws_bytes) {
        size_t e = ((const char *)sums_dev - c->ws) + (size_t)oemgpu_sums_len(p) * 8;
        if (e > base) base = e;
    }
    base = (base + 255) / 256 * 256;
    const size_t need = base + B.off + paths_ws_bytes(p, q, o) + extra_ws + 4096;
    if (need > c->ws_bytes) {
        if (base != 0) { set_error("internal: workspace frame too small"); return OEMGPU_ERR_INTERNAL; }
        if (ctx_reserve(c, need)) return OEMGPU_ERR_HIP;
    }
    Bump B2; B2.off = base + B.off;
    double *xx = (double *)(c->ws + base + a_xx), *xy = (double *)(c->ws + base + a_xy), *st = (double *)(c->ws + base + a_st);
    {
        Timer t(c, OEMGPU_T_FINAL);
        const bool plain = wpatch || big_xy_std;
        rc = launch_finalize(c->stream, moments_dev, sums_dev, p, semantics, plain ? 0 : standardize, plain ? 0 : intercept, xx, xy, st);
        if (!rc && wpatch) rc = launch_weighted_patch_stats(c->stream, wpatch, p, st);
        if (!rc && big_xy_std) { rc = launch_big_gram_scales(c->stream, xx, xy, p, standardize, st, big_xy_std); lmax_xy = big_xy_std; }
        if (rc) return rc;
    }
    if (!ex) return run_paths_parts(c, B2, xx, xy, st, p, q, semantics, standardize, intercept, o, beta, lambda_out, niter, loss, d, nullptr, lmax_xy);
    PathExtras x = *ex;
    x.lmax_xy_dev = lmax_xy;
    return run_paths(c, B2, xx, xy, st, p, q, semantics, standardize, intercept, o, nullptr, beta, lambda_out, niter, loss, d, x);
}

static bool wide_pays(int64_t n, int32_t p, const oemgpu_opts *o)
{
    if (n > p || n > WIDE_MAX_N) return false;
    if (sw().OEM_NO_WIDE.set) return false;
    if (sw().OEM_WIDE.set) return true;
    if (p > 1024 && p <= 2048 && o && o->npen == 1 && !pen_is_grp(o->penalty[0]) && !o->accelerate && !o->compute_loss &&
        !sw().OEM_NO_ROWCOOP.set && !sw().OEM_NO_SYMCOOP.set && !sw().OEM_NO_COOP.set) return false;
    if (p <= 1024) return false;
    const int g = path_wcoop_workgroups((int)n, p);
    const bool wc = n <= 1024 && g >= 1 && g <= WCOOP_GMAX && !sw().OEM_NO_WCOOP.set;
    if (p <= 4096 && !sw().OEM_NO_SYMCOOP.set && !sw().OEM_NO_COOP.set) return wc;
    if (2 * n < p) return true;
    return wc;
}

static int run_paths_parts(oemgpu_ctx *c, Bump B, const double *xx, const double *xy, const double *st, int p, int q, int sem, int standardize, int intercept,
                           const oemgpu_opts *o, double *beta, double *lambda_out, int32_t *niter, double *loss, double *d,
                           const WideArgs *wd, const double *lmax_xy)
{
    std::vector<int> ie, ig;
    for (int k = 0; k < o->npen; ++k) (pen_is_grp(o->penalty[k]) ? ig : ie).push_back(k);
    bool split = !ie.empty() && !ig.empty() && !o->accelerate && !sw().OEM_NO_PENALTY_SPLIT.set;
    if (split && wd && wd->sparse) split = false;
    else if (split && wd) {
        const int gw = path_wres_workgroups(wd->n, p);
        const bool wcoop_fits = path_wcoop_workgroups(wd->n, p) >= 1 && path_wcoop_workgroups(wd->n, p) <= (c->num_cu * 3 / 4 < WCOOP_GMAX ? c->num_cu * 3 / 4 : WCOOP_GMAX);
        split = !wcoop_fits && gw >= 1 && gw <= c->num_cu - 8 && path_wres_xchg_doubles(wd->n, p) > 0 && !sw().OEM_NO_WRES.set && !sw().OEM_NO_WCOOP.set;
    } else if (split)
        split = q > 1024 && q <= 2048 && sem == OEMGPU_SEM_DENSE && path_rowcoop_workgroups(q) <= c->num_cu * 3 / 4 &&
                !sw().OEM_NO_ROWCOOP.set && !sw().OEM_NO_SYMCOOP.set && !sw().OEM_NO_COOP.set;
    PathExtras x;
    x.wide = wd; x.lmax_xy_dev = lmax_xy;
    if (!split) return run_paths(c, B, xx, xy, st, p, q, sem, standardize, intercept, o, nullptr, beta, lambda_out, niter, loss, d, x);
    const int nl = nl_of(o), rows = p + 1;
    const bool user = o->lambda_user && o->nlambda_user > 0;
    bool first = true;
    for (const std::vector<int> *part : {&ie, &ig}) {
        const int m = (int)part->size();
        std::vector<int32_t> pen(m);
        std::vector<double> lam(user ? (size_t)m * nl : 0);
        for (int k = 0; k < m; ++k) {
            pen[k] = o->penalty[(*part)[k]];
            if (user) memcpy(&lam[(size_t)k * nl], o->lambda_user + (size_t)(*part)[k] * nl, sizeof(double) * nl);
        }
        oemgpu_opts os = *o;
        os.npen = m; os.penalty = pen.data(); os.lambda_user = user ? lam.data() : nullptr;
        std::vector<double> b((size_t)m * nl * rows), lo((size_t)m * nl), ls((size_t)m * nl);
        std::vector<int32_t> ni((size_t)m * nl);
        double dd = 0.0;
        Bump Bp = B;
        const int rc = run_paths(c, Bp, xx, xy, st, p, q, sem, standardize, intercept, &os, nullptr, b.data(), lo.data(), ni.data(), ls.data(), &dd, x);
        if (rc) return rc;
        for (int k = 0; k < m; ++k) {
            const size_t dst = (size_t)(*part)[k] * nl, src = (size_t)k * nl;
            memcpy(beta + dst * rows, &b[src * rows], sizeof(double) * (size_t)nl * rows);
            memcpy(lambda_out + dst, &lo[src], sizeof(double) * nl);
            memcpy(loss + dst, &ls[src], sizeof(double) * nl);
            memcpy(niter + dst, &ni[src], sizeof(int32_t) * nl);
        }
        if (first) *d = dd;
        first = false;
    }
    return 0;
}

static size_t moments_solve_ws(size_t frame, size_t pass_end, int32_t p, const oemgpu_opts *o, size_t extra = 0)
{
    const size_t solve = frame + ((size_t)p * p + p + stats_len(p)) * 8 + 1024 + paths_ws_bytes(p, p, o) + extra + 4096;
    return solve > pass_end ? solve : pass_end;
}

static int wide_stage(oemgpu_ctx *c, int64_t n, int32_t p, WideArgs *wd, double **xs, double **ys)
{
    const WideLayout lay = wide_layout(n);
    Bump X;
    const size_t a_xs = X.take(sizeof(double) * (size_t)lay.rows() * p), a_ys = X.take(sizeof(double) * (size_t)lay.rows()),
                 a_sc = X.take(sizeof(double) * wide_scratch_doubles((int)n, p));
    ctx_void_cv(c);
    if (ctx_grow(c, &c->aux, &c->aux_bytes, X.off)) return OEMGPU_ERR_HIP;
    *xs = (double *)(c->aux + a_xs); *ys = (double *)(c->aux + a_ys);
    wd->xs = *xs; wd->ys = *ys; wd->lay = lay; wd->n = (int)n; wd->scratch = (double *)(c->aux + a_sc);
    return 0;
}

static int fit_dense_wide_dev(oemgpu_ctx *c, const double *x_dev, int64_t n, int64_t ld, int32_t p, const double *y_dev,
                              int32_t standardize, int32_t intercept, const oemgpu_opts *o,
                              double *beta, double *lambda_out, int32_t *niter, double *loss, double *d)
{
    if (set_device(c)) return OEMGPU_ERR_HIP;
    WideArgs wd;
    double *xs, *ys;
    int rc = wide_stage(c, n, p, &wd, &xs, &ys);
    if (rc) return rc;
    Bump B;
    const size_t a_xy = B.take((size_t)p * 8), a_st = B.take((size_t)stats_len(p) * 8);
    if (ctx_reserve(c, B.off + paths_ws_bytes(p, p, o) + 4096)) return OEMGPU_ERR_HIP;
    double *xy = (double *)(c->ws + a_xy), *st = (double *)(c->ws + a_st);
    {
        Timer t(c, OEMGPU_T_MOMENTS);
        rc = launch_wide_standardize(c->stream, x_dev, n, ld, p, y_dev, standardize, intercept, wd.lay, xs, ys, xy, st);
        if (rc) return rc;
    }
    return run_paths_parts(c, B, nullptr, xy, st, p, p, OEMGPU_SEM_DENSE, standardize, intercept, o, beta, lambda_out, niter, loss, d, &wd, nullptr);
}

static int big_wide_sparse_loss(oemgpu_ctx *c, const double *x_dev, int64_t n, int64_t ld, int32_t p, const double *y_dev, const oemgpu_opts *o,
                                const double *beta, const int32_t *niter, double *loss)
{
    const size_t nk = (size_t)o->npen * nl_of(o), nchunk = (size_t)((n + 2047) / 2048);
    Bump L;
    const size_t a_b = L.take(nk * (size_t)(p + 1) * 8), a_p = L.take(nk * nchunk * 8), a_l = L.take(nk * 8);
    if (ctx_reserve(c, L.off + 4096)) return OEMGPU_ERR_HIP;
    double *bd = (double *)(c->ws + a_b), *ld_ = (double *)(c->ws + a_l);
    OEM_HIP(hipMemcpyAsync(bd, beta, nk * (size_t)(p + 1) * 8, hipMemcpyHostToDevice, c->stream));
    int rc;
    if ((rc = launch_resid_loss(c->stream, x_dev, n, ld, p, y_dev, bd, p + 1, (int)nk, (double *)(c->ws + a_p), ld_))) return rc;
    OEM_HIP(hipMemcpyAsync(loss, ld_, nk * 8, hipMemcpyDeviceToHost, c->stream));
    OEM_HIP(hipStreamSynchronize(c->stream));
    for (size_t k = 0; k < nk; ++k) if (niter[k] == 0) loss[k] = 1e99;
    return 0;
}

static int fit_big_wide_dev(oemgpu_ctx *c, const double *x_dev, int64_t n, int64_t ld, int32_t p, const double *y_dev, int32_t standardize,
                            const oemgpu_opts *o, double *beta, double *lambda_out, int32_t *niter, double *loss, double *d, bool sparse_loss = false)
{
    if (set_device(c)) return OEMGPU_ERR_HIP;
    if (n < 2) { set_error("big.oem / sparse x with p >= n: at least two rows"); return OEMGPU_ERR_UNSUPPORTED; }
    int rc;
    if (!wide_pays(n, p, o)) {
        const GramPlan pl = gram_plan(n, p, c->num_cu);
        Bump B;
        const size_t a_xs2 = B.take((size_t)p * 8), a_mom = B.take((size_t)oemgpu_moments_len(p) * 8);
        const size_t frame = B.off;
        const size_t a_t = B.take(pl.tpart_doubles * 8), a_v = B.take(pl.vpart_doubles * 8);
        if (ctx_reserve(c, moments_solve_ws(frame, B.off, p, o))) return OEMGPU_ERR_HIP;
        double *mom = (double *)(c->ws + a_mom);
        {
            Timer t(c, OEMGPU_T_MOMENTS);
            rc = shard_moments(c, pl, x_dev, n, ld, y_dev, nullptr, (double *)(c->ws + a_t), (double *)(c->ws + a_v), mom);
            if (rc) return rc;
        }
        oemgpu_opts og = *o;
        og.compute_loss = 0;
        rc = solve_moments_impl(c, mom, nullptr, p, OEMGPU_SEM_BIG, standardize, 0, &og, beta, lambda_out, niter, loss, d, nullptr, nullptr, nullptr, 0,
                                (double *)(c->ws + a_xs2));
        return (rc || !sparse_loss) ? rc : big_wide_sparse_loss(c, x_dev, n, ld, p, y_dev, o, beta, niter, loss);
    }
    WideArgs wd;
    double *xs, *ys;
    if ((rc = wide_stage(c, n, p, &wd, &xs, &ys))) return rc;
    Bump B;
    const size_t a_xs2 = B.take((size_t)p * 8), a_xy = B.take((size_t)p * 8), a_st = B.take((size_t)stats_len(p) * 8);
    if (ctx_reserve(c, B.off + paths_ws_bytes(p, p, o) + 4096)) return OEMGPU_ERR_HIP;
    double *xy = (double *)(c->ws + a_xy), *st = (double *)(c->ws + a_st), *xy_std = (double *)(c->ws + a_xs2);
    {
        Timer t(c, OEMGPU_T_MOMENTS);
        rc = launch_wide_standardize(c->stream, x_dev, n, ld, p, y_dev, 0, 0, wd.lay, xs, ys, xy, st);
        if (!rc && standardize) rc = launch_big_wide_scales(c->stream, x_dev, n, ld, p, xy, st, xy_std);
        if (rc) return rc;
    }
    rc = run_paths_parts(c, B, nullptr, xy, st, p, p, OEMGPU_SEM_BIG, standardize, 0, o, beta, lambda_out, niter, loss, d, &wd, standardize ? xy_std : nullptr);
    return (rc || !sparse_loss) ? rc : big_wide_sparse_loss(c, x_dev, n, ld, p, y_dev, o, beta, niter, loss);
}

static int fit_big_wide_host(const double *x, int64_t n, int32_t p, const double *y, int32_t standardize, const oemgpu_opts *o,
                             double *beta, double *lambda_out, int32_t *niter, double *loss, double *d, bool sparse_loss = false)
{
    oemgpu_ctx *c = ctx_acquire(o->device);
    if (!c) return OEMGPU_ERR_NO_DEVICE;
    double *xd = nullptr, *yd = nullptr;
    int64_t ld = 0;
    int rc = host_upload_resident(c, x, n, p, y, o, &xd, &ld, &yd, 0, true);
    if (!rc) rc = fit_big_wide_dev(c, xd, n, ld, p, yd, standardize, o, beta, lambda_out, niter, loss, d, sparse_loss);
    (void)hipStreamSynchronize(c->stream);
    ctx_release(c);
    return rc;
}

static int fit_dense_src(const char *who, oemgpu_ctx *c, const DenseSrc &X, int64_t n, int32_t p, const double *y_dev,
                         int32_t standardize, int32_t intercept, const oemgpu_opts *o,
                         double *beta, double *lambda_out, int32_t *niter, double *loss, double *d)
{
    HT(0);
    int rc = src_args_check(who, c, X, n, p, y_dev, beta && lambda_out && niter && loss && d);
    if (!rc) rc = check_opts(o, p, p);
    if (rc) return rc;
    if (wide_pays(n, p, o)) {
        if (X.colmajor()) return fit_dense_wide_dev(c, X.cm(), n, X.ld, p, y_dev, standardize, intercept, o, beta, lambda_out, niter, loss, d);
        set_error("%s: %lld x %d is a shape of the p >= n engines, which read a column-major x: it takes the column-major entry "
                  "(oemgpu_fit_dense_dev)", who, (long long)n, p);
        return OEMGPU_ERR_UNSUPPORTED;
    }
    MomentPlan pl;
    if ((rc = dense_src_moment_plan(who, c, X, n, p, &pl))) return rc;
    if (set_device(c)) return OEMGPU_ERR_HIP;
    Bump B;
    const size_t a_sums = B.take((size_t)oemgpu_sums_len(p) * 8), a_mom = B.take((size_t)oemgpu_moments_len(p) * 8);
    const size_t frame = B.off;
    const size_t a_scr = B.take(pl.scratch_bytes);
    if (ctx_reserve(c, moments_solve_ws(frame, B.off, p, o))) return OEMGPU_ERR_HIP;
    double *sums = (double *)(c->ws + a_sums), *mom = (double *)(c->ws + a_mom);
    {
        Timer t(c, OEMGPU_T_MOMENTS);
        rc = dense_src_moments(c, pl, X, n, y_dev, nullptr, c->ws + a_scr, mom);
        if (rc) return rc;
    }
    HT(1);
    rc = oemgpu_solve_moments_dev(c, mom, nullptr, p, OEMGPU_SEM_DENSE, standardize, intercept, o, beta, lambda_out, niter, loss, d);
#ifdef OEM_HOST_TIMING
    HT(5); g_ht.acc[0] += g_tp[1] - g_tp[0]; g_ht.acc[1] += g_tp[2] - g_tp[1]; g_ht.acc[2] += g_tp[3] - g_tp[2]; g_ht.acc[3] += g_tp[4] - g_tp[3]; g_ht.acc[4] += g_tp[5] - g_tp[4]; ++g_ht.n;
#endif
    if (rc || !c->shift_advised) return rc;
    {
        Timer t(c, OEMGPU_T_SHIFT);
        rc = dense_src_shift_sums(c->stream, X, n, p, y_dev, sums);
        if (rc) return rc;
    }
    {
        Timer t(c, OEMGPU_T_MOMENTS);
        rc = dense_src_moments(c, pl, X, n, y_dev, sums, c->ws + a_scr, mom);
        if (rc) return rc;
    }
    return oemgpu_solve_moments_dev(c, mom, sums, p, OEMGPU_SEM_DENSE, standardize, intercept, o, beta, lambda_out, niter, loss, d);
}

int oemgpu_fit_dense_dev(oemgpu_ctx *c, const double *x_dev, int64_t n, int64_t ld, int32_t p, const double *y_dev,
                         int32_t standardize, int32_t intercept, const oemgpu_opts *o,
                         double *beta, double *lambda_out, int32_t *niter, double *loss, double *d)
{
    return fit_dense_src("fit_dense", c, dense_src_cm(x_dev, ld), n, p, y_dev, standardize, intercept, o, beta, lambda_out, niter, loss, d);
}

int oemgpu_fit_dense_rm_dev(oemgpu_ctx *c, const void *x_dev, int32_t dtype, int64_t n, int64_t ldr, int32_t p, const double *y_dev,
                            int32_t standardize, int32_t intercept, const oemgpu_opts *o,
                            double *beta, double *lambda_out, int32_t *niter, double *loss, double *d)
{
    return fit_dense_src("fit_dense_rm", c, dense_src_rm(x_dev, dtype, ldr), n, p, y_dev, standardize, intercept, o, beta, lambda_out, niter, loss, d);
}

int oemgpu_selftest_gram_rm_plan(int64_t n, int32_t p, int32_t num_cu, int64_t *out)
{
    if (n < 1 || p < 1 || num_cu < 1 || !out) { set_error("selftest_gram_rm_plan: bad argument"); return OEMGPU_ERR_ARG; }
    if (int rc = rm_p_refusal("selftest_gram_rm_plan", p)) return rc;
    const GramRmPlan pl = gram_rm_plan(n, p, num_cu);
    out[0] = pl.ntc; out[1] = pl.nblk; out[2] = pl.nchunk; out[3] = pl.steps; out[4] = (int64_t)pl.nchunk * pl.nblk;
    out[5] = (int64_t)pl.tpart_doubles; out[6] = (int64_t)(pl.nchunk - 1) * pl.steps * 16; out[7] = GRAM_RM_P_MAX;
    return 0;
}

static int fit_dense_weighted_impl(oemgpu_ctx *c, const double *x_dev, int64_t n, int64_t ld, int32_t p, const double *y_dev, const double *w_dev,
                                   const double *w_host, int32_t standardize, int32_t intercept, const oemgpu_opts *o,
                                   double *beta, double *lambda_out, int32_t *niter, double *loss, double *d)
{
    if (!c || !x_dev || !y_dev || (!w_dev && !w_host)) { set_error("fit_dense_weighted: NULL argument"); return OEMGPU_ERR_ARG; }
    int rc = check_opts(o, p, p);
    if (rc) return rc;
    if (n < 1 || ld < n) { set_error("fit_dense_weighted: bad n / ld"); return OEMGPU_ERR_ARG; }
    const bool wide = n <= p;
    if (set_device(c)) return OEMGPU_ERR_HIP;
    const int flag = (standardize ? 1 : 0) + 2 * (intercept ? 1 : 0);
    const int64_t ldz = (n + 63) / 64 * 64;
    Bump Z;
    const size_t a_z = Z.take(sizeof(double) * (size_t)ldz * p), a_yz = Z.take(sizeof(double) * (size_t)ldz), a_ws = Z.take(sizeof(double) * (size_t)(2 + 2 * p)),
                 a_w = Z.take(sizeof(double) * (size_t)n);
    const size_t a_xx1 = wide ? Z.take(sizeof(double) * (size_t)p * p) : 0, a_xy1 = wide ? Z.take(sizeof(double) * (size_t)p) : 0,
                 a_st1 = wide ? Z.take(sizeof(double) * (size_t)stats_len(p)) : 0;
    ctx_void_cv(c);
    if (ctx_grow(c, &c->aux, &c->aux_bytes, Z.off)) return OEMGPU_ERR_HIP;
    double *z = (double *)(c->aux + a_z), *yz = (double *)(c->aux + a_yz), *wsd = (double *)(c->aux + a_ws);
    if (w_host) {
        for (int64_t i = 0; i < n; ++i)
            if (!(w_host[i] >= 0.0) || !std::isfinite(w_host[i])) { set_error("fit_dense_weighted: weights must be finite and >= 0"); return OEMGPU_ERR_ARG; }
        OEM_HIP(hipMemcpyAsync(c->aux + a_w, w_host, sizeof(double) * (size_t)n, hipMemcpyHostToDevice, c->stream));
        w_dev = (const double *)(c->aux + a_w);
    }
    const GramPlan pl = gram_plan(n, p, c->num_cu);
    Bump B;
    const size_t a_mom = B.take((size_t)oemgpu_moments_len(p) * 8);
    const size_t frame = B.off;
    const size_t a_t = B.take(pl.tpart_doubles * 8), a_v = B.take(pl.vpart_doubles * 8);
    const size_t large_ws = wide ? path_large_work_doubles(p, 128) * 8 + 4096 : 0;
    const size_t need = moments_solve_ws(frame, B.off, p, o, large_ws);
    if (ctx_reserve(c, need)) return OEMGPU_ERR_HIP;
    double *mom = (double *)(c->ws + a_mom);
    {
        Timer t(c, OEMGPU_T_MOMENTS);
        rc = launch_weighted_stats(c->stream, x_dev, n, ld, p, y_dev, w_dev, flag, wsd);
        if (!rc) rc = launch_weighted_apply(c->stream, x_dev, n, ld, p, y_dev, w_dev, flag, wsd, 0, z, ldz, yz);
        if (!rc) rc = shard_moments(c, pl, z, n, ldz, yz, nullptr, (double *)(c->ws + a_t), (double *)(c->ws + a_v), mom);
        if (rc) return rc;
    }
    if (!wide) return solve_moments_impl(c, mom, nullptr, p, OEMGPU_SEM_DENSE, standardize, intercept, o, beta, lambda_out, niter, loss, d, wsd);
    double *xx1 = (double *)(c->aux + a_xx1), *xy1 = (double *)(c->aux + a_xy1), *st1 = (double *)(c->aux + a_st1);
    rc = launch_finalize(c->stream, mom, nullptr, p, OEMGPU_SEM_DENSE, 0, 0, xx1, xy1, st1);
    if (!rc) rc = launch_weighted_patch_stats(c->stream, wsd, p, st1);
    double lam1 = 0.0;
    if (!rc) rc = oemgpu_eig_max_dev(c, xx1, p, &lam1);
    if (rc) return rc;
    if (ctx_reserve(c, need)) return OEMGPU_ERR_HIP;
    mom = (double *)(c->ws + a_mom);
    {
        Timer t(c, OEMGPU_T_MOMENTS);
        rc = launch_weighted_apply(c->stream, x_dev, n, ld, p, y_dev, w_dev, flag, wsd, 1, z, ldz, yz);
        if (!rc) rc = shard_moments(c, pl, z, n, ldz, yz, nullptr, (double *)(c->ws + a_t), (double *)(c->ws + a_v), mom);
        if (rc) return rc;
    }
    PathExtras ex;
    ex.d_fixed = lam1 * 1.005;
    ex.loss_xx = xx1; ex.loss_xy = xy1; ex.loss_stats = st1;
    return solve_moments_impl(c, mom, nullptr, p, OEMGPU_SEM_DENSE, standardize, intercept, o, beta, lambda_out, niter, loss, d, wsd, &ex, xy1, large_ws);
}

int oemgpu_fit_dense_weighted_dev(oemgpu_ctx *c, const double *x_dev, int64_t n, int64_t ld, int32_t p, const double *y_dev, const double *w_dev,
                                  int32_t standardize, int32_t intercept, const oemgpu_opts *o,
                                  double *beta, double *lambda_out, int32_t *niter, double *loss, double *d)
{
    return fit_dense_weighted_impl(c, x_dev, n, ld, p, y_dev, w_dev, nullptr, standardize, intercept, o, beta, lambda_out, niter, loss, d);
}

int oemgpu_fit_dense_weighted(const double *x, int64_t n, int32_t p, const double *y, const double *weights, int32_t standardize, int32_t intercept,
                              const oemgpu_opts *o, double *beta, double *lambda_out, int32_t *niter, double *loss, double *d)
{
    if (!x || !y || !weights || !o || !beta || !lambda_out || !niter || !loss || !d) { set_error("fit_dense_weighted: NULL argument"); return OEMGPU_ERR_ARG; }
    int rc = check_opts(o, p, p);
    if (rc) return rc;
    if (n < 1) { set_error("fit_dense_weighted: bad n"); return OEMGPU_ERR_ARG; }
    oemgpu_ctx *c = ctx_acquire(o->device);
    if (!c) return OEMGPU_ERR_NO_DEVICE;
    double *xd = nullptr, *yd = nullptr;
    int64_t ld = 0;
    rc = host_upload_resident(c, x, n, p, y, o, &xd, &ld, &yd, 0, true);
    if (!rc) rc = fit_dense_weighted_impl(c, xd, n, ld, p, yd, nullptr, weights, standardize, intercept, o, beta, lambda_out, niter, loss, d);
    (void)hipStreamSynchronize(c->stream);
    ctx_release(c);
    return rc;
}

int oemgpu_fit_xtx_dev(oemgpu_ctx *c, const double *xtx_dev, const double *xty_dev, int32_t p, const double *scale_factor,
                       const oemgpu_opts *o, double *beta, double *lambda_out, int32_t *niter, double *loss, double *d)
{
    if (!c || !xtx_dev || !xty_dev || !beta || !lambda_out || !niter || !loss || !d) { set_error("fit_xtx: NULL argument"); return OEMGPU_ERR_ARG; }
    int rc = check_opts(o, p, p);
    if (rc) return rc;
    if (set_device(c)) return OEMGPU_ERR_HIP;
    Bump B;
    const size_t a_xx = B.take((size_t)p * p * 8), a_xy = B.take((size_t)p * 8), a_sf = B.take((size_t)p * 8),
                 a_st = B.take((size_t)stats_len(p) * 8);
    if (ctx_reserve(c, B.off + paths_ws_bytes(p, p, o) + 4096)) return OEMGPU_ERR_HIP;
    double *xx = (double *)(c->ws + a_xx), *xy = (double *)(c->ws + a_xy), *st = (double *)(c->ws + a_st), *sf = (double *)(c->ws + a_sf);
    std::vector<double> sinv;
    if (scale_factor) {
        sinv.resize(p);
        for (int j = 0; j < p; ++j) sinv[j] = 1 / scale_factor[j];
        OEM_HIP(hipMemcpyAsync(sf, sinv.data(), sizeof(double) * p, hipMemcpyHostToDevice, c->stream));
        OEM_HIP(hipStreamSynchronize(c->stream));
    }
    {
        Timer t(c, OEMGPU_T_FINAL);
        rc = launch_xtx_prepare(c->stream, xtx_dev, xty_dev, scale_factor ? sf : nullptr, p, xx, xy, st);
        if (rc) return rc;
    }
    return run_paths(c, B, xx, xy, st, p, p, SEM_XTX, 0, 0, o, scale_factor, beta, lambda_out, niter, loss, d);
}

int oemgpu_last_shift_in_effect(oemgpu_ctx *c) { return c ? c->shifted : -1; }
int oemgpu_last_shift_advised(oemgpu_ctx *c) { return c ? c->shift_advised : -1; }

int oemgpu_eig_max_dev(oemgpu_ctx *c, const double *a_dev, int32_t p, double *lambda_max)
{
    if (!c || !a_dev || !lambda_max || p < 1) { set_error("eig_max: bad argument"); return OEMGPU_ERR_ARG; }
    if (set_device(c)) return OEMGPU_ERR_HIP;
    Bump B;
    const size_t a_z = B.take((size_t)(p + 8) * 8), a_o = B.take(256);
    const int lan = 2 * p < 32 ? 32 : (2 * p < 288 ? 2 * p : 288);
    size_t work_d = p <= SMALL_P_MAX ? path_small_xchg_bytes() / 8 : path_large_work_doubles(p, lan);
    const bool coop = path_coop_eligible(p, false, false, 0, 1);
// ... 2206 lines not shown
```

### oem_amd/csrc/common.hpp

```cpp
#pragma once

#include <hip/hip_runtime.h>
#include <stdint.h>

#include <vector>

#include "../../include/oemgpu.h"
#include "path_large_layout.hpp"
#include "switches.hpp"

namespace oemgpu {

typedef double v4d __attribute__((ext_vector_type(4)));
typedef double v2d __attribute__((ext_vector_type(2)));

void set_error(const char *fmt, ...);
#define OEM_HIP(call)                                                                         \
    do {                                                                                      \
        hipError_t e__ = (call);                                                              \
        if (e__ != hipSuccess) {                                                              \
            oemgpu::set_error("%s failed: %s (%s:%d)", #call, hipGetErrorString(e__), __FILE__, __LINE__); \
            return OEMGPU_ERR_HIP;                                                            \
        }                                                                                     \
    } while (0)

struct GramPlan {
    int p;
    int ntc;
    int ntile;
    int tri;
    int nblk;
    int wd_units;
    int wd;
    int n8, n6, n4;
    int nchunk;
    int steps;
    size_t tpart_doubles;
    size_t vpart_doubles;
};
GramPlan gram_plan(int64_t n, int p, int num_cu);
GramPlan gram_plan_bound(int64_t nmax, int p, int num_cu);
void gram_sb_deal(int ntc, int *n8, int *n6, int *n4);
enum { GRAM_FORM_TRI = OEMGPU_GRAM_FORM_TRI, GRAM_FORM_RING_SADDR = OEMGPU_GRAM_FORM_RING_SADDR, GRAM_FORM_RING_LANE = OEMGPU_GRAM_FORM_RING_LANE,
       GRAM_FORM_SB = OEMGPU_GRAM_FORM_SB, GRAM_FORM_WD3 = OEMGPU_GRAM_FORM_WD3, GRAM_FORM_WD4 = OEMGPU_GRAM_FORM_WD4,
       GRAM_FORM_WD_UNITS = OEMGPU_GRAM_FORM_WD_UNITS, GRAM_FORM_BLK = OEMGPU_GRAM_FORM_BLK };
struct GramForm { int form, strips; };
GramForm gram_form(const GramPlan &pl, int64_t n, int64_t ld, bool aligned);

int launch_shift_sums(hipStream_t s, const double *x, int64_t n, int64_t ld, int p, const double *y, double *sums);
int launch_gram(hipStream_t s, const GramPlan &pl, const double *x, int64_t n, int64_t ld, const double *y,
                const double *sums , double *tpart, double *vpart);
int launch_moments_reduce(hipStream_t s, const GramPlan &pl, const double *tpart, const double *vpart, double *moments);

constexpr int GRAM_RM_P_MAX = 1024;
constexpr int GRAM_RM_MIN_ROWS = 1024;
constexpr int64_t GRAM_RM_PART_BYTES = 512 << 20;
constexpr int64_t GRAM_RM_CHUNK_BYTES = 16 << 20;
struct GramRmPlan {
    int p;
    int ntc;
    int nb;
    int nblk;
    int nchunk;
    int64_t steps;
    size_t tpart_doubles;
};
GramRmPlan gram_rm_plan(int64_t n, int p, int num_cu);
int launch_shift_sums_rm(hipStream_t s, const void *x, int dtype, int64_t n, int64_t ldr, int p, const double *y, double *sums);
int launch_gram_rm(hipStream_t s, const GramRmPlan &pl, const void *x, int dtype, int64_t n, int64_t ldr, const double *y,
                   const double *sums , double *tpart);
int launch_gram_rm_reduce(hipStream_t s, const GramRmPlan &pl, const double *tpart, double *moments);

__host__ __device__ static inline int stats_len(int p) { return 4 + 2 * p + 2; }
__host__ __device__ static inline int stats_shift_flag(int p) { return 4 + 2 * p; }
int launch_finalize(hipStream_t s, const double *moments, const double *sums, int p, int sem, int standardize,
                    int intercept, double *xx , double *xy , double *stats);
int launch_xtx_prepare(hipStream_t s, const double *xtx, const double *xty, const double *sf_inv , int p,
                       double *xx, double *xy, double *stats);

int shard_moments(oemgpu_ctx *c, const GramPlan &pl, const double *x, int64_t n, int64_t ld, const double *y, const double *sums,
                  double *tpart, double *vpart, double *moments);
int launch_moments_add(hipStream_t s, double *acc, const double *m, size_t len, bool first);

int64_t csc_check(const char *who, int64_t n, int p, const int64_t *colptr, const int32_t *rowidx, const double *values,
                  std::vector<int64_t> *rowcount);
constexpr int CSC_CHUNK = 8192;
struct SparseRoute { bool csc; int64_t rows, ld; };
SparseRoute sparse_route(int64_t n, int p, int64_t nnz);
bool sparse_wide_route(int64_t n, int p, int64_t nnz);
int csc_tile_moments(oemgpu_ctx *c, const SparseRoute &R, const int64_t *colptr, const int32_t *rowidx, const double *val, const double *w,
                     const double *y, int64_t n, int p, int64_t maxcol, double *tile, double *tpart, double *vpart, double *mtile, double *M,
                     int64_t row0 = 0, int64_t nrows = -1);
int64_t csc_tiles(const SparseRoute &R, int64_t nrows);
void csc_tile_rows(const SparseRoute &R, int64_t row0, int64_t nrows, int64_t t, int64_t *r0, int64_t *r1);
size_t csc_moments_work_bytes(int64_t n, int p);
bool csc_moments_fits(int p);
int launch_csc_moments(hipStream_t s, const int64_t *colptr, const int32_t *rowidx, const double *val, const double *y, int64_t n, int p,
                       void *work, double *moments);
int csc_chunks(int64_t n);
size_t csc_wgram_work_bytes(int64_t n, int p);
int launch_csc_chunk_ptr(hipStream_t s, const int64_t *colptr, const int32_t *rowidx, int64_t n, int p, int32_t *cptr);
int launch_csc_to_csr(hipStream_t s, const int64_t *colptr, const int32_t *rowidx, const double *val, const int32_t *cptr, int64_t n, int p,
                      const int64_t *rowptr, int32_t *ccol, double *cval);
int launch_csc_wgram(hipStream_t s, const int64_t *colptr, const int32_t *rowidx, const double *val, const double *w, const int32_t *cptr,
                     int64_t n, int p, double *part, double *M);
int launch_weighted_stats(hipStream_t s, const double *x, int64_t n, int64_t ld, int p, const double *y, const double *w, int flag, double *ws);
int launch_weighted_apply(hipStream_t s, const double *x, int64_t n, int64_t ld, int p, const double *y, const double *w, int flag, const double *ws,
                          int squared, double *z, int64_t ldz, double *yz);
int launch_weighted_patch_stats(hipStream_t s, const double *ws, int p, double *stats);
int launch_gram_loss(hipStream_t s, const double *xx, const double *xy, const double *stats, int q, const double *beta, const double *sinv,
                     const int *niter, double *loss, int nk);
int launch_resid_loss(hipStream_t s, const double *x, int64_t n, int64_t ld, int p, const double *y, const double *beta, int rows, int nk,
                      double *part, double *loss);

size_t fold_layout_ints(int64_t n, int K);
int launch_fold_layout(hipStream_t s, const int *foldid, int64_t n, int K, int *blockcnt, int64_t *fold_n, int64_t *fold_start,
                       int *pos, int *bad, int align = 16);
int launch_gather_rows(hipStream_t s, const double *x, int64_t n, int64_t ld, int p, const double *y, const int *pos,
                       double *xo, int64_t ldo, double *yo);
int launch_gather_rows_rm(hipStream_t s, const void *x, int dtype, int64_t n, int64_t ldr, int p, const double *y, const int *foldid, int K,
                          const int *pos, double *xo, int64_t ldo, double *yo);
int launch_gather_responses(hipStream_t s, const double *y, int64_t rs, int64_t cs, int64_t n, int m, const int *pos, double *yo, int64_t ldo);
int launch_fold_sum(hipStream_t s, const double *M, int K, size_t len, int skip , double *out);
enum { CV_FORM_SINGLE = 0, CV_FORM_MULTI = 1, CV_FORM_CHUNK = 2 };
struct CvErrPlan {
    int K4, ntile, lt, passes, form, chunks, last, nwg;
    size_t lds;
};
CvErrPlan cv_error_plan(int64_t n, int p, int K, int npen, int nl, int num_cu);
size_t cv_part_doubles(int nwg, int K, int npen, int nl);
int launch_cv_error(hipStream_t s, const double *xp, int64_t ldp, const double *yp, const int64_t *fold_start, const int64_t *fold_n,
                    int K, int p, const double *B, int npen, int nl, int mae, int wmode, const CvErrPlan &P, double n, double *part, double *out,
                    bool triples = false);
int launch_cv_finish(hipStream_t s, const double *part, int nparts, int npen, int nl, double n, double *out, bool triples);
CvErrPlan cv_error_plan_many(int64_t n, int p, int K, int npen, int nl, int nb, int num_cu);
int launch_cv_error_many(hipStream_t s, const double *xp, int64_t ldp, const double *Yp, const int64_t *fold_start, const int64_t *fold_n,
                         int K, int p, const double *B, int npen, int nl, int mae, const CvErrPlan &P, double n, int nb, double *part, double *out);
int launch_fold_inverse(hipStream_t s, const int *pos, int64_t n, int64_t ldp, int *inv);
int launch_cv_fold_error(hipStream_t s, const double *xp, int64_t ldp, const double *yp, const int64_t *fold_start, const int64_t *fold_n,
                         int K, int p, const double *B, int npen, int nl, int mae, const CvErrPlan &P, double *part, const int *ncol,
                         double *triples, double *predmat, const int *inv, int64_t n);
int launch_cv_fold_finish(hipStream_t s, const double *part, int per_fold, int K, int npen, int nl, const int *ncol, double *triples);

constexpr int XVS_CVW = 4;
struct XvalSparsePlan {
    SparseRoute R;
    int64_t n, nnz, npad_max;
    int p, K, npen, nl, nl16;
    int nchunk_max, per, nrange_max, rpf_max, cv_nwg, cv_waves, cv_lblk;
    GramPlan plmax;
    size_t a_col, a_row, a_val, a_y, a_fid, a_prow, a_pval, a_cfo, a_cptr, a_rowptr, a_ccol, a_cval, a_gpart, a_ypart, a_rtab, a_bt, a_tile,
           a_mtile, bytes;
};
XvalSparsePlan xval_sparse_plan(int64_t n, int p, int64_t nnz, int K, int npen, int nl, int num_cu, bool resident = false);
int xval_sparse_ranges(const XvalSparsePlan &P, const int64_t *fold_n, std::vector<int32_t> &rtab, std::vector<int32_t> &frange, int64_t *npad);
int launch_csc_fold_permute(hipStream_t s, const int64_t *colptr, const int32_t *rowidx, const double *val, const double *y, const int32_t *foldid,
                            const int *pos, int64_t n, int p, int K, int64_t npad, int32_t *cfo, int32_t *prow, double *pval, double *yp);
int launch_csc_fold_moments(hipStream_t s, const int64_t *colptr, const int32_t *prow, const double *pval, const double *yp, const int32_t *cptr,
                            const int32_t *cfo, const int64_t *fold_start, const int64_t *fold_n, int p, int K, int nchunk, int nrange,
                            const int32_t *rtab, const int32_t *frange, double *gpart, double *ypart, double *mfold);
int launch_csr_rowptr(hipStream_t s, const int64_t *colptr, const int32_t *prow, const int32_t *cptr, int p, int nchunk, int64_t *rowptr);
int launch_csr_cv_error(hipStream_t s, const XvalSparsePlan &P, const int64_t *rowptr, const int32_t *ccol, const double *cval, const double *yp,
                        const int64_t *fold_start, const int64_t *fold_n, const double *B, double *bt, int mae, double *part, double *out,
                        bool triples);
constexpr size_t CVS_PART_MAX = 64000000;
struct CvSparseScorePlan {
    int K, npen, nl, nl16, nwg, waves, lblk;
    size_t part_bytes;
};
CvSparseScorePlan cv_sparse_score_plan(int64_t n, int K, int npen, int nl, int num_cu);
int launch_csr_cv_fold_score(hipStream_t s, const CvSparseScorePlan &P, int p, const int64_t *rowptr, const int32_t *ccol, const double *cval,
                             const double *yp, const int64_t *fold_start, const int64_t *fold_n, const double *B, double *bt, int mae,
                             double *part, const int *ncol, double *triples, double *predmat, const int *inv, int64_t n);
struct CvWideScorePlan {
    int K, npen, nl, nl16, nwg, waves, lblk;
    size_t table_bytes, part_bytes, a_list, a_raw, a_bt, a_part, a_tri, a_ncol, bytes;
};
CvWideScorePlan cv_wide_score_plan(int64_t n, int p, int K, int npen, int nl, int num_cu);
int launch_csr_cv_wide_score_fold(hipStream_t s, const CvWideScorePlan &P, int p, const int64_t *rowptr, const int32_t *ccol, const double *cval,
                                  const double *y, const int32_t *list, int nk, const double *raw, double *bt, int mae, const int *ncol,
                                  double *part_k, double *predmat, int64_t n);
int launch_csc_gram_ranges(hipStream_t s, const int64_t *colptr, const int32_t *rowidx, const double *val, const int32_t *cptr, int p, int nchunk,
                           int nrange, const int32_t *rtab, double *part);
size_t csc_gram_lds_bytes(int p);
int csc_range_budget(int64_t n, int p);

int launch_weight_scale(hipStream_t s, double *xp, int64_t ldp, double *yp, int p, int K, const int64_t *fold_start, const int64_t *fold_n,
                        double *csq);
int launch_finalize_weighted(hipStream_t s, const double *Mw, const double *cs, int p, int standardize, int intercept, double *xx,
                             double *xy, double *stats);

struct PathArgs {
    int p;
    int npen, nl, user_lambda, maxit, accelerate, compute_loss;
    int ngroups;
    int lanczos_steps;
    int yscale;
    int lmax_from;
    double alpha, gamma, tau, tol, lambda_min_ratio;
    const double *xx;
    const double *xy;
    const double *stats;
    const int *penalty;
    const double *lambda_user;
    const double *pf;
    const double *sinv;
    const int *gid;
    const int *gstart;
    const int *gidx;
    const double *gw;
    const int *gzero;
    int grp_head;
    const int *grun;
    const double *gwc;
    double *beta;
    double *lambda_out;
    int *niter;
    double *loss;
    double *d_out;
    double *work;
    double *sympk;
    int nbatch;
    long long bs_xx, bs_xy, bs_stats, bs_out, bs_work;
    int pen_split, pen_lo, pen_hi;
    int lmax_group;
    const double *lmax_xy;
    double *stats_out;
    int stats_n;
    double d_fixed;
    const int *abort_word;
    int one_xcd, xcd_base;
    int no_active_prefix;
};

// ... 146 lines not shown
```

### oem_amd/csrc/dense_src.hpp

```cpp
#pragma once

#include "ctx.hpp"

namespace oemgpu {

struct DenseSrc {
    const void *x;
    int dtype;
    int64_t ld;
    bool colmajor() const { return dtype < 0; }
    const double *cm() const { return (const double *)x; }
};
inline DenseSrc dense_src_cm(const double *x_dev, int64_t ld) { return DenseSrc{x_dev, -1, ld}; }
inline DenseSrc dense_src_rm(const void *x_dev, int dtype, int64_t ldr) { return DenseSrc{x_dev, dtype < 0 ? INT32_MAX : dtype, ldr}; }

int dense_src_check(const char *who, const DenseSrc &X, int64_t n, int32_t p);
int dense_src_shift_sums(hipStream_t s, const DenseSrc &X, int64_t n, int p, const double *y, double *sums);
int dense_src_gather(hipStream_t s, const DenseSrc &X, int64_t n, int p, const double *y, const int32_t *foldid, int K, const int *pos,
                     double *xo, int64_t ldo, double *yo);
struct MomentPlan {
    GramPlan cm{};
    GramRmPlan rm{};
    size_t scratch_bytes = 0;
};
int dense_src_moment_plan(const char *who, const oemgpu_ctx *c, const DenseSrc &X, int64_t n, int32_t p, MomentPlan *pl);
int dense_src_moments(oemgpu_ctx *c, const MomentPlan &pl, const DenseSrc &X, int64_t n, const double *y, const double *sums, char *scratch,
                      double *moments);

}
```

### oem_amd/csrc/gram.hip

```cpp
#include <cstdlib>
#include "common.hpp"
#include "gram_dev.hpp"
#include <vector>

#include <type_traits>

namespace oemgpu {

__global__ __launch_bounds__(256) void shift_sums_kernel(const double *__restrict__ x, int64_t n, int64_t ld, int p,
                                                          const double *__restrict__ y, double *__restrict__ sums)
{
    __shared__ double sh[3][256];
    const int j = blockIdx.x;
    const double *col = (j < p) ? x + (size_t)j * ld : y;
    const int64_t nch = (n + 15) / 16;
    const int64_t nsamp = nch < 256 ? nch : 256;
    const int k = threadIdx.x;
    double s = 0.0, ss = 0.0, cnt = 0.0;
    if (k < nsamp) {
        const int64_t c = (nsamp > 1) ? ((int64_t)k * (nch - 1)) / (nsamp - 1) : 0;
        const int64_t r0 = c * 16;
        if (r0 + 16 <= n) {
            double v[16];
#pragma unroll
// ... 465 lines not shown
        fetch(sa, ua, ra1, ra2, 0);
        slot = next(slot);
    }
    GSTAMP(0);
    auto steady = [&](Slab<NF> &use, Slab<NF> &nxt, v2d (&uuse)[SB > 0 ? SB : 1], v2d (&unxt)[SB > 0 ? SB : 1],
                      v2d (&r1use)[NR], v2d (&r2use)[NR], v2d (&r1nxt)[NR], v2d (&r2nxt)[NR]) {
        const unsigned dst = ring + (unsigned)islot * SLOT_B;
        const v2d *src = ring_rd + (slot * SLOT_B) / 16;
        const v2d *srcA = ring_rdA + (slot * SLOT_B) / 16;
        const v2d *src1 = ring_rd1 + (slot * SLOT_B) / 16;
        const int sl16 = (slot * SLOT_B) / 16;
        auto hook = [&](auto M_) {
            constexpr int m = decltype(M_)::value;
            if constexpr (OEM_GRAM_EXP != 1 && m == 1) set_m0(dst + CEN * 1024);
            if constexpr (OEM_GRAM_EXP != 1 && m >= 1 && m <= NF) dma(std::integral_constant<int, m - 1>{});
            if constexpr (m == NF + 1) {
                if constexpr (OEM_GRAM_EXP != 4) bump();
                if constexpr (OEM_GRAM_EXP != 3 && OEM_GRAM_EXP != 1) wait_vm<(NSLOT - 2) * NF>();
            }
            if constexpr (OEM_GRAM_EXP != 2 && m >= NF + 2 && m <= 2 * NF + 1) nxt.v[m - NF - 2] = src[((m - NF - 2) * 1024) / 16];
            if constexpr (OEM_GRAM_EXP != 2 && SB > 0 && m >= 2 * NF + 2 && m < 2 * NF + 2 + SB) unxt[m - 2 * NF - 2] = srcA[4 * (m - 2 * NF - 2)];
            if constexpr (DG && m >= 2 * NF + 2 + SB && m < 2 * NF + 2 + SB + (NT - 1)) {
                constexpr int f = m - (2 * NF + 2 + SB);
                r1nxt[DG ? f : 0] = src1[(f * 1024) / 16]; r2nxt[DG ? f : 0] = r2_src(std::integral_constant<int, DG ? f : 0>{})[sl16];
            }
        };
        if constexpr (DG) consume_ring_dg<NT, SB, (SB == 0)>(use, uuse, r1use, r2use, hook);
        else if constexpr (SB > 0) consume_ring_strip<NT, SB>(use, uuse, hook);
        else consume_slab<NT, NT, true, false, false, true, SHIFT>(V, use, X, cy, 0, n, hook);
        islot = next(islot); slot = next(slot);
    };
    static_assert(SB == 0 || 2 * NF + 2 + SB <= (NT - 1) * NT, "not enough 16x16x4 MFMAs per slab to carry the hooks");
    static_assert(2 * NF + 1 < NT * (NT + 1), "not enough MFMAs per slab to carry the hooks");
    static_assert(!DG || 2 * NF + 2 + SB + (NT - 1) <= (NT - 1) * NT, "not enough hook slots per slab for the rotated reads");
    while (k + NSLOT + 1 <= ns) {
        steady(sa, sb, ua, ub, ra1, ra2, rb1, rb2);
        GSTAMP(4);
        steady(sb, sa, ub, ua, rb1, rb2, ra1, ra2);
        GSTAMP(4);
        issued += 2; k += 2;
    }
    while (issued < ns) { issue(islot); islot = next(islot); ++issued; }
    wait_vm<0>();
    for (; k < ns; ++k) {
        if (k + 1 < ns) { fetch(sb, ub, rb1, rb2, slot); slot = next(slot); }
        if constexpr (DG) consume_ring_dg<NT, SB, (SB == 0)>(sa, ua, ra1, ra2);
        else if constexpr (SB > 0) consume_ring_strip<NT, SB>(sa, ua);
        else consume_slab<NT, NT, true, false, false, true, SHIFT>(V, sa, X, cy, 0, n);
        if (k + 1 < ns) {
#pragma unroll
            for (int f = 0; f < NF; ++f) sa.v[f] = sb.v[f];
#pragma unroll
            for (int a = 0; a < SB; ++a) ua[a] = ub[a];
            if constexpr (DG) {
#pragma unroll
                for (int f = 0; f < NT - 1; ++f) { ra1[f] = rb1[f]; ra2[f] = rb2[f]; }
            }
        }
    }
    GSTAMP(5);
    __syncthreads();
    if (ns < nslab && w0 + 32 * (int64_t)ns < n) {
        const int64_t r = w0 + 32 * (int64_t)ns + 2 * q;
        const int64_t o0 = (r < n ? r : n - 1) - r, o1 = (r + 1 < n ? r + 1 : n - 1) - r;
#pragma unroll
        for (int f = 0; f < NF; ++f) {
            if (f == NF - 1 && const_lane) { sa.v[f] = v2d{1.0, 1.0}; continue; }
            const gptr_t pf = (SADDR && f < NF - 1)
                                  ? (gptr_t)((const char __attribute__((address_space(1))) *)sbase + voff[f]) + (f - CEN) * 128
                                  : cur[f] + (f - CEN) * 128;
            sa.v[f].x = pf[o0]; sa.v[f].y = pf[o1];
        }
        if constexpr (DG) {
            const double m0 = (r < n) ? 1.0 : 0.0, m1 = (r + 1 < n) ? 1.0 : 0.0;
#pragma unroll
            for (int f = 0; f < NF; ++f) { sa.v[f].x *= m0; sa.v[f].y *= m1; }
            v2d *ring_wr = reinterpret_cast<v2d *>(reinterpret_cast<char *>(lds) + w * (NSLOT * SLOT_B)) + lane;
#pragma unroll
            for (int f = 0; f < NT - 1; ++f) ring_wr[(f * 1024) / 16] = sa.v[f];
            __builtin_amdgcn_fence(__ATOMIC_RELEASE, "wavefront");
#pragma unroll
            for (int f = 0; f < NT - 1; ++f) ra1[f] = ring_rd1[(f * 1024) / 16];
            static_for<NT - 1>([&](auto E_) { ra2[decltype(E_)::value] = r2_src(E_)[0]; });
            asm volatile("s_nop 3" ::: "memory");
            consume_ring_dg<NT, SB, true>(sa, ua, ra1, ra2);
        } else consume_slab<NT, NT, true, true, false, true, SHIFT>(V, sa, X, cy, r, n);
    }
    asm volatile("s_nop 15\n\ts_nop 7" ::: "memory");
    constexpr int TPP = (NTILES + 1) / 2;
    static_for<2>([&](auto P_) {
        constexpr int pass = decltype(P_)::value, t0 = pass * TPP, t1 = (t0 + TPP < NTILES) ? t0 + TPP : NTILES;
        static_for<(t1 - t0)>([&](auto T_) {
            constexpr int tt = t0 + decltype(T_)::value;
            constexpr bool isdiag = DG && [] { for (int I = 0; I < NT - 1; ++I) if (I * (I + 3) / 2 == tt) return true; return false; }();
            if constexpr (isdiag) {
                double *tl = lds + (size_t)w * (TPP * 256) + (size_t)(tt - t0) * 256;
                static_for<4>([&](auto R_) { tl[decltype(R_)::value * 64 + lane] = 0.0; });
                const int b4 = i >> 2;
                constexpr int I = [] { for (int I2 = 0; I2 < NT - 1; ++I2) if (I2 * (I2 + 3) / 2 == tt) return I2; return 0; }();
                static_for<2>([&](auto R_) {
                    constexpr int r = decltype(R_)::value;
                    const double v = AccTile<tt>::template read<r>();
                    int reg = (b4 + r) & 3, ln = lane;
                    if (r == 1 && b4 == 3) { reg = 3; ln = ((lane & 3) << 4) | q; }
                    tl[reg * 64 + ln] = v;
                });
                if constexpr (I >= 2 * ((NT - 1) / 2)) tl[((b4 + 2) & 3) * 64 + lane] = AccTile<tt>::template read<2>();
                else if constexpr (I % 2 == 0) { const double v = AccTile<tt>::template read<2>(); if (b4 < 2) tl[(b4 + 2) * 64 + lane] = v; }
                else {
                    constexpr int ttl = (I - 1) * (I + 2) / 2;
                    const double v = AccTile<ttl>::template read<2>();
                    if (b4 >= 2) tl[b4 * 64 + (((lane & 3) << 4) | ((b4 - 2) << 2) | q)] = v;
                }
            } else {
                static_for<4>([&](auto R_) {
                    constexpr int r = decltype(R_)::value;
                    lds[(size_t)w * (TPP * 256) + ((tt - t0) * 4 + r) * 64 + lane] = AccTile<tt>::template read<r>();
                });
            }
        });
        static_for<SB * NT>([&](auto S_) {
            constexpr int sidx = decltype(S_)::value, a = sidx / NT, T = sidx % NT, tt = (NT - 1) * NT / 2 + T;
            if constexpr (tt >= t0 && tt < t1)
                lds[(size_t)w * (TPP * 256) + ((tt - t0) * 4 + a) * 64 + lane] += AccStrip<sidx>::read();
        });
        __syncthreads();
        for (int e = tid; e < (t1 - t0) * 256; e += 256) {
            const double a0 = lds[e], a1 = lds[TPP * 256 + e], a2 = lds[2 * TPP * 256 + e], a3 = lds[3 * TPP * 256 + e];
            tdst[(size_t)t0 * 256 + e] = (a0 + a1) + (a2 + a3);
        }
        __syncthreads();
    });
#ifdef OEM_GRAM_DIAG
    GSTAMP(6);
    if (blockIdx.x == 7 && tid == 0) { gd[7] = (unsigned long long)ns; for (int j = 0; j < 8; ++j) g_gram_diag[j] = gd[j]; }
#endif
}

#ifdef OEM_GRAM_DIAG
extern "C" __attribute__((visibility("default"))) int oemgpu_gram_diag_read(unsigned long long *out)
{
    return hipMemcpyFromSymbol(out, HIP_SYMBOL(g_gram_diag), sizeof(unsigned long long) * 8) == hipSuccess ? 0 : -1;
}
#endif


template <int NT, bool ALIGNED>
__global__ __launch_bounds__(256) void gram_tri_kernel(const double *__restrict__ x, const double *__restrict__ y,
                                                        const double *__restrict__ sums, double *__restrict__ tpart,
                                                        double *__restrict__ vpart, GramDims a)
{
    extern __shared__ __attribute__((aligned(16))) double lds[];
    const int chunk = blockIdx.x;
    gram_body<NT, NT, true, ALIGNED, false, true>(x, a.n, a.ld, a.p, y, sums, a.ntc, 0, 0,
                                                  (int64_t)chunk * a.steps * 64, a.steps, true,
                                                  tpart + (size_t)chunk * a.ntile * 256, vpart, lds);
}

template <int NT, int SB, bool SADDR>
__global__ __launch_bounds__(256) void gram_ring_kernel(const double *__restrict__ x, const double *__restrict__ y,
                                                         const double *__restrict__ sums, double *__restrict__ tpart,
                                                         double *__restrict__ vpart, GramDims a)
{
    extern __shared__ __attribute__((aligned(16))) double lds[];
    (void)vpart;
    const int chunk = blockIdx.x;
    if (shift_needed_wave(sums, a.p))
        gram_tri_ring_body<NT, true, 0, SADDR>(x, a.n, a.ld, a.p, y, sums, (int64_t)chunk * a.steps * 64, a.steps,
                                               tpart + (size_t)chunk * a.ntile * 256, lds);
    else
        gram_tri_ring_body<NT, false, SB, SADDR>(x, a.n, a.ld, a.p, y, sums, (int64_t)chunk * a.steps * 64, a.steps,
                                                 tpart + (size_t)chunk * a.ntile * 256, lds);
}

template <bool ALIGNED>
__global__ __launch_bounds__(256) void gram_blk_kernel(const double *__restrict__ x, const double *__restrict__ y,
                                                        const double *__restrict__ sums, double *__restrict__ tpart,
                                                        double *__restrict__ vpart, GramDims a)
{
    extern __shared__ __attribute__((aligned(16))) double lds[];
    const int L = blockIdx.x, xcd = L & 7, s = L >> 3;
    const int tb = s % a.nblk, chunk = (s / a.nblk) * 8 + xcd;
    int BI = (int)((sqrtf(8.0f * (float)tb + 1.0f) - 1.0f) * 0.5f);
    while (BI * (BI + 1) / 2 > tb) --BI;
    while ((BI + 1) * (BI + 2) / 2 <= tb) ++BI;
    const int BJ = tb - BI * (BI + 1) / 2;
    const int64_t row_begin = (int64_t)chunk * a.steps * 64;
    double *tdst = tpart + (size_t)chunk * a.ntile * 256;
    double *vdst = vpart + (size_t)chunk * (32 * a.ntc + 4);
    if (BI == BJ)
        gram_body<4, 4, true, ALIGNED, true, false>(x, a.n, a.ld, a.p, y, sums, a.ntc, 4 * BI, 4 * BI, row_begin,
                                                    a.steps, BI == 0, tdst, vdst, lds);
    else
        gram_body<4, 4, false, ALIGNED, false, false>(x, a.n, a.ld, a.p, y, sums, a.ntc, 4 * BI, 4 * BJ,
                                                      row_begin, a.steps, false, tdst, vdst, lds);
}

void gram_sb_deal(int ntc, int *n8_out, int *n6_out, int *n4_out)
{
    int best8 = (ntc + 7) / 8, best6 = 0, best4 = 0;
    long best = -1;
    for (int n4 = 0; n4 <= 1; ++n4)
        for (int n6 = 0; n6 <= 1; ++n6) {
            const int rest = ntc - 6 * n6 - 4 * n4, n8 = rest > 0 ? (rest + 7) / 8 : 0;
            if (n8 + n6 + n4 == 0 || 8 * n8 + 6 * n6 + 4 * n4 - ntc >= 4) continue;
            const long cost = 64L * n8 * (n8 - 1) / 2 + 48L * n8 * n6 + 32L * n8 * n4 + 24L * n6 * n4 + 36L * n8 + 24L * n6 + 12L * n4;
            if (best < 0 || cost < best || (cost == best && n8 + n6 + n4 < best8 + best6 + best4)) { best = cost; best8 = n8; best6 = n6; best4 = n4; }
        }
    *n8_out = best8; *n6_out = best6; *n4_out = best4;
}

constexpr int GRAM_MAX_ROUNDS = 12;
static inline int gram_max_rounds(const GramPlan &pl) { return pl.wd ? (pl.wd_units == 1 ? 2 : 6) : GRAM_MAX_ROUNDS; }

static GramPlan gram_plan_compute(int64_t n, int p, int num_cu)
{
    GramPlan pl;
    pl.p = p;
    pl.tri = (p + 2 + 15) / 16 <= 7;
    pl.n8 = pl.n6 = pl.n4 = 0; pl.wd = 0; pl.wd_units = 0;
    pl.ntc = pl.tri ? (p + 2 + 15) / 16 : (p + 15) / 16;
    pl.ntile = pl.ntc * (pl.ntc + 1) / 2;
    const int64_t nsteps = (n + 63) / 64;
    if (pl.tri) {
        pl.nblk = 1;
        int64_t c = nsteps < num_cu ? nsteps : num_cu;
        if (c < 1) c = 1;
        pl.steps = (int)((nsteps + c - 1) / c);
        if (pl.steps < 1) pl.steps = 1;
        pl.nchunk = (int)((nsteps + pl.steps - 1) / pl.steps);
        if (pl.nchunk < 1) pl.nchunk = 1;
    } else {
        const int nb = (pl.ntc + 3) / 4;
        pl.nblk = nb * (nb + 1) / 2;
        int n8 = 0, n6 = 0, n4 = 0;
        gram_sb_deal(pl.ntc, &n8, &n6, &n4);
        pl.n8 = n8; pl.n6 = n6; pl.n4 = n4;
        pl.wd = (pl.ntc == 15 || pl.ntc == 16) ? 4 : ((pl.ntc == 11 || pl.ntc == 12) ? 3 : 0);
        pl.wd_units = pl.wd ? 1 : 0;
        if (pl.ntc >= 31 && (pl.ntc % 16 == 0 || pl.ntc % 16 == 15)) { pl.wd = 4; pl.wd_units = (pl.ntc + 15) / 16; }
        const int nsb = n8 + n6 + n4, nsblk = pl.wd ? pl.wd_units * pl.wd_units : nsb * (nsb + 1) / 2;
        const int64_t cnt[SB_KINDS] = {(int64_t)n8 * (n8 - 1) / 2, (int64_t)n6 * n8, n8, (int64_t)n4 * n8, (int64_t)n4 * n6, n6, n4};
        const double per_slab[SB_KINDS] = {2136.0, 1680.0, 1284.0, 1160.0, 890.0, 890.0, 520.0};
        int64_t c = 0;
        double best = 0.0;
        for (int rounds = 1; rounds <= gram_max_rounds(pl); ++rounds) {
            int64_t cc = ((int64_t)num_cu * rounds) / nsblk;
            if (cc > nsteps) cc = nsteps;
            if (cc < 1) cc = 1;
            cc = (cc + 7) / 8 * 8;
            const double slabs = (double)((nsteps + cc - 1) / cc) * 8.0;
            std::vector<std::pair<double, int64_t>> grp{{0.0, (int64_t)num_cu}};
            double end = 0.0;
            for (int kind = 0; kind < SB_KINDS; ++kind) {
                const double d = slabs * (pl.wd == 4 ? (kind == 0 ? 4500.0 : 4250.0) : (pl.wd == 3 ? 2700.0 : per_slab[kind])) + 25000.0;
                for (int64_t m = pl.wd ? (kind == 0 ? cc * pl.wd_units : (kind == 1 ? cc * pl.wd_units * (pl.wd_units - 1) : 0)) : cc * cnt[kind]; m > 0;) {
                    const double t = grp.front().first + d;
                    const int64_t take = grp.front().second < m ? grp.front().second : m;
                    if ((grp.front().second -= take) == 0) grp.erase(grp.begin());
                    size_t at = grp.size();
                    while (at > 0 && grp[at - 1].first > t) --at;
                    if (at > 0 && grp[at - 1].first == t) grp[at - 1].second += take; else grp.insert(grp.begin() + at, {t, take});
                    m -= take;
                    if (t > end) end = t;
                }
            }
            const double cost = end + (double)cc * pl.ntile * 2048.0 / 3.5e12 * 2.1e9;
            if (c == 0 || cost < best * 0.995) { c = cc; best = cost; }
            if (cc >= nsteps) break;
        }
        pl.steps = (int)((nsteps + c - 1) / c);
        if (pl.steps < 1) pl.steps = 1;
        pl.nchunk = (int)c;
    }
    pl.tpart_doubles = (size_t)pl.nchunk * pl.ntile * 256;
    pl.vpart_doubles = (size_t)pl.nchunk * (32 * pl.ntc + 4);
    return pl;
}

GramPlan gram_plan(int64_t n, int p, int num_cu)
{
    struct Memo { int64_t n; int p, cu; unsigned gen; GramPlan pl; };
    static thread_local Memo memo[4] = {{-1, 0, 0, 0u, {}}, {-1, 0, 0, 0u, {}}, {-1, 0, 0, 0u, {}}, {-1, 0, 0, 0u, {}}};
    static thread_local unsigned next = 0;
    const unsigned gen = sw().generation;
    for (const Memo &m : memo) if (m.n == n && m.p == p && m.cu == num_cu && m.gen == gen) return m.pl;
    Memo &m = memo[next++ & 3];
    m.n = n; m.p = p; m.cu = num_cu; m.gen = gen; m.pl = gram_plan_compute(n, p, num_cu);
    return m.pl;
}

GramPlan gram_plan_bound(int64_t nmax, int p, int num_cu)
{
    GramPlan pl = gram_plan(nmax, p, num_cu);
    if (!pl.tri) {
        const int nsb = pl.n8 + pl.n6 + pl.n4, nsblk = pl.wd ? pl.wd_units * pl.wd_units : nsb * (nsb + 1) / 2;
        const int64_t nsteps = (nmax + 63) / 64;
        int64_t cc = ((int64_t)num_cu * gram_max_rounds(pl)) / nsblk;
        if (cc > nsteps) cc = nsteps;
        if (cc < 1) cc = 1;
        cc = (cc + 7) / 8 * 8;
        if (cc > pl.nchunk) pl.nchunk = (int)cc;
    } else {
        const int64_t nsteps = (nmax + 63) / 64;
        const int64_t cc = nsteps < num_cu ? (nsteps < 1 ? 1 : nsteps) : num_cu;
        if (cc > pl.nchunk) pl.nchunk = (int)cc;
    }
    pl.tpart_doubles = (size_t)pl.nchunk * pl.ntile * 256;
    pl.vpart_doubles = (size_t)pl.nchunk * (32 * pl.ntc + 4);
    return pl;
}

GramForm gram_form(const GramPlan &pl, int64_t n, int64_t ld, bool aligned)
{
    GramForm f;
    f.strips = 0;
    if (pl.tri) {
        f.form = GRAM_FORM_TRI;
        if (aligned && pl.ntc >= 4 && n >= 64) {
            const int rem = pl.p + 2 - 16 * (pl.ntc - 1);
            const bool saddr = pl.p >= 16 * (pl.ntc - 1) && (double)pl.p * (double)ld * 8.0 + 65536.0 < 4294967296.0;
            f.form = saddr ? GRAM_FORM_RING_SADDR : GRAM_FORM_RING_LANE;
            f.strips = !saddr ? 0 : (rem <= 4 ? 1 : (rem <= 8 ? 2 : 0));
        }
        return f;
    }
    if (aligned && n >= 64 && (double)ld * 16.0 * 8.0 < 4294967296.0)
        f.form = !pl.wd ? GRAM_FORM_SB : (pl.wd_units > 1 ? GRAM_FORM_WD_UNITS : (pl.wd == 3 ? GRAM_FORM_WD3 : GRAM_FORM_WD4));
    else
        f.form = GRAM_FORM_BLK;
    return f;
}

template <bool ALIGNED>
static int launch_gram_t(hipStream_t s, const GramPlan &pl, const double *x, const double *y, const double *sums,
                         double *tpart, double *vpart, const GramDims &a)
{
    const size_t tile_bytes = 256 * sizeof(double);
    const GramForm gf = gram_form(pl, a.n, a.ld, ALIGNED);
#define OEM_TRI(NT)                                                                                       \
    case NT: {                                                                                            \
        size_t sh = (size_t)(NT * (NT + 1) / 2) * tile_bytes;                                             \
        size_t vb = (size_t)4 * (2 * 16 * NT + 4) * sizeof(double);                                       \
        if (sh < vb) sh = vb;                                                                             \
        hipLaunchKernelGGL((gram_tri_kernel<NT, ALIGNED>), dim3(pl.nchunk), dim3(256), sh, s, x, y, sums, tpart, vpart, a);          \
        break;                                                                                            \
    }
    if (gf.form == GRAM_FORM_RING_SADDR || gf.form == GRAM_FORM_RING_LANE) {
        size_t sh = (size_t)pl.ntile * tile_bytes;
        const size_t rb = (size_t)4 * 5 * pl.ntc * 1024;
        if (sh < rb) sh = rb;
        const bool saddr = gf.form == GRAM_FORM_RING_SADDR;
        const int sb = gf.strips;
#define OEM_RING(NT, SB, SA)                                                                                                   \
    if (pl.ntc == NT && sb == SB && saddr == SA) {                                                                             \
        if (sh > 64 * 1024 && lds_limit_once(reinterpret_cast<const void *>(&gram_ring_kernel<NT, SB, SA>), sh)) return OEMGPU_ERR_HIP; \
        hipLaunchKernelGGL((gram_ring_kernel<NT, SB, SA>), dim3(pl.nchunk), dim3(256), sh, s, x, y, sums, tpart, vpart, a);   \
        OEM_HIP(hipGetLastError());                                                                                            \
        return 0;                                                                                                              \
    }
        OEM_RING(4, 0, true) OEM_RING(5, 0, true) OEM_RING(6, 0, true) OEM_RING(7, 0, true)
        OEM_RING(4, 1, true) OEM_RING(5, 1, true) OEM_RING(6, 1, true) OEM_RING(7, 1, true)
        OEM_RING(4, 2, true) OEM_RING(5, 2, true) OEM_RING(6, 2, true) OEM_RING(7, 2, true)
        OEM_RING(4, 0, false) OEM_RING(5, 0, false) OEM_RING(6, 0, false) OEM_RING(7, 0, false)
#undef OEM_RING
    }
    if (pl.tri) {
        switch (pl.ntc) {
            OEM_TRI(1) OEM_TRI(2) OEM_TRI(3) OEM_TRI(4) OEM_TRI(5) OEM_TRI(6) OEM_TRI(7)
        default: set_error("gram: bad tile count %d", pl.ntc); return OEMGPU_ERR_INTERNAL;
        }
    } else {
        if (gf.form != GRAM_FORM_BLK) {
            if (pl.wd) return launch_gram_wd(s, pl, x, y, sums, tpart, vpart, a);
            return launch_gram_sb(s, pl, x, y, sums, tpart, vpart, a);
        }
        size_t sh = 16 * tile_bytes;
        size_t vb = (size_t)4 * (2 * 16 * 4 + 4) * sizeof(double);
        if (sh < vb) sh = vb;
        hipLaunchKernelGGL((gram_blk_kernel<ALIGNED>), dim3(pl.nchunk * pl.nblk), dim3(256), sh, s, x, y, sums, tpart, vpart, a);
    }
#undef OEM_TRI
    OEM_HIP(hipGetLastError());
    return 0;
}

int launch_gram(hipStream_t s, const GramPlan &pl, const double *x, int64_t n, int64_t ld, const double *y,
                const double *sums, double *tpart, double *vpart)
{
    GramDims a;
    a.n = n; a.ld = ld; a.p = pl.p;
    a.ntc = pl.ntc; a.ntile = pl.ntile; a.nblk = pl.nblk; a.nchunk = pl.nchunk; a.steps = pl.steps;
    const bool aligned = (((uintptr_t)x | (uintptr_t)y) & 15) == 0 && (ld & 1) == 0;
    return aligned ? launch_gram_t<true>(s, pl, x, y, sums, tpart, vpart, a)
                   : launch_gram_t<false>(s, pl, x, y, sums, tpart, vpart, a);
}

template <int SPL>
__global__ __launch_bounds__(1024) void moments_reduce_split_kernel(const double *__restrict__ tpart, int p, int ntile, int nchunk,
                                                                     double *__restrict__ M)
{
    constexpr int EB = 256 / SPL, NG = 4 * SPL;
    __shared__ double part[NG][EB];
    const int q = p + 2;
    const int tile = blockIdx.x / SPL, e = threadIdx.x % EB, grp = threadIdx.x / EB, el = (blockIdx.x % SPL) * EB + e;
    int I = (int)((sqrtf(8.0f * (float)tile + 1.0f) - 1.0f) * 0.5f);
    while (I * (I + 1) / 2 > tile) --I;
    while ((I + 1) * (I + 2) / 2 <= tile) ++I;
    const int J = tile - I * (I + 1) / 2;
    double s = 0.0;
    const double *src = tpart + (size_t)tile * 256 + el;
    const size_t stride = (size_t)ntile * 256;
    int c = grp;
    for (; c + 7 * NG < nchunk; c += 8 * NG) {
        double t[8];
#pragma unroll
        for (int k = 0; k < 8; ++k) t[k] = src[(size_t)(c + NG * k) * stride];
#pragma unroll
        for (int k = 0; k < 8; ++k) s += t[k];
    }
    for (; c < nchunk; c += NG) s += src[(size_t)c * stride];
    part[grp][e] = s;
    __syncthreads();
    if (grp == 0) {
        double t[NG];
#pragma unroll
        for (int g = 0; g < NG; ++g) t[g] = part[g][e];
#pragma unroll
        for (int h = 1; h < NG; h <<= 1)
#pragma unroll
            for (int g = 0; g + h < NG; g += 2 * h) t[g] += t[g + h];
        const int reg = el >> 6, lane = el & 63;
        const int row = 16 * I + (lane >> 4) + 4 * reg, col = 16 * J + (lane & 15);
        if (row < q && col < q && row >= col) {
            M[(size_t)col * q + row] = t[0];
            M[(size_t)row * q + col] = t[0];
        }
    }
}

__global__ __launch_bounds__(1024) void moments_reduce_kernel(const double *__restrict__ tpart,
                                                               const double *__restrict__ vpart, int p, int ntc,
                                                               int ntile, int nchunk, int nchunk_v, int aug, double *__restrict__ M)
{
    __shared__ double part[4][256];
    const int q = p + 2;
    const int lim = aug ? q : p;
    const int b = blockIdx.x, e = threadIdx.x & 255, grp = threadIdx.x >> 8;
    if (b < ntile) {
        int I = (int)((sqrtf(8.0f * (float)b + 1.0f) - 1.0f) * 0.5f);
        while (I * (I + 1) / 2 > b) --I;
        while ((I + 1) * (I + 2) / 2 <= b) ++I;
        const int J = b - I * (I + 1) / 2;
        double s = 0.0;
        const double *src = tpart + (size_t)b * 256 + e;
        const size_t stride = (size_t)ntile * 256;
        int c = grp;
        for (; c + 28 < nchunk; c += 32) {
            double t[8];
#pragma unroll
            for (int k = 0; k < 8; ++k) t[k] = src[(size_t)(c + 4 * k) * stride];
#pragma unroll
            for (int k = 0; k < 8; ++k) s += t[k];
        }
        for (; c < nchunk; c += 4) s += src[(size_t)c * stride];
        part[grp][e] = s;
        __syncthreads();
        s = (part[0][e] + part[1][e]) + (part[2][e] + part[3][e]);
        const int reg = e >> 6, lane = e & 63;
        const int row = 16 * I + (lane >> 4) + 4 * reg, col = 16 * J + (lane & 15);
        if (grp == 0 && row < lim && col < lim && row >= col) {
            M[(size_t)col * q + row] = s;
            M[(size_t)row * q + col] = s;
        }
    } else if (!aug) {
        const int vw = 32 * ntc + 4;
        const int idx = (b - ntile) * 256 + e;
        double s = 0.0;
        if (idx < vw) {
            const double *src = vpart + idx;
            int c = grp;
            for (; c + 28 < nchunk_v; c += 32) {
                double t[8];
#pragma unroll
                for (int k = 0; k < 8; ++k) t[k] = src[(size_t)(c + 4 * k) * vw];
#pragma unroll
                for (int k = 0; k < 8; ++k) s += t[k];
            }
            for (; c < nchunk_v; c += 4) s += src[(size_t)c * vw];
        }
        part[grp][e] = s;
        __syncthreads();
        s = (part[0][e] + part[1][e]) + (part[2][e] + part[3][e]);
        if (grp == 0 && idx < vw) {
            if (idx < 16 * ntc) {
                if (idx < p) { M[(size_t)idx * q + (p + 1)] = s; M[(size_t)(p + 1) * q + idx] = s; }
            } else if (idx < 32 * ntc) {
                const int j = idx - 16 * ntc;
                if (j < p) { M[(size_t)j * q + p] = s; M[(size_t)p * q + j] = s; }
            } else if (idx == 32 * ntc) { M[(size_t)p * q + (p + 1)] = s; M[(size_t)(p + 1) * q + p] = s; }
            else if (idx == 32 * ntc + 1) M[(size_t)p * q + p] = s;
            else if (idx == 32 * ntc + 2) M[(size_t)(p + 1) * q + (p + 1)] = s;
        }
    }
}

int launch_moments_reduce(hipStream_t s, const GramPlan &pl, const double *tpart, const double *vpart, double *moments)
{
    const int nvblk = pl.tri ? 0 : (32 * pl.ntc + 4 + 255) / 256;
    if (pl.tri && pl.nchunk >= 64) {
        hipLaunchKernelGGL(moments_reduce_split_kernel<4>, dim3(pl.ntile * 4), dim3(1024), 0, s, tpart, pl.p, pl.ntile, pl.nchunk, moments);
        OEM_HIP(hipGetLastError());
        return 0;
    }
    hipLaunchKernelGGL(moments_reduce_kernel, dim3(pl.ntile + nvblk), dim3(1024), 0, s, tpart, vpart, pl.p,
                       pl.ntc, pl.ntile, pl.nchunk, pl.nchunk, pl.tri, moments);
    OEM_HIP(hipGetLastError());
    return 0;
}

struct Mom {
    const double *M; const double *sums; int p, q; double n;
    bool shift;
    __device__ double c(int j) const { return shift ? sums[j] / sums[p + 1] : 0.0; }
    __device__ double s(int j) const { return M[(size_t)j * q + (p + 1)]; }
    __device__ double mu(int j) const { return c(j) + s(j) / n; }
    __device__ double cen(int i, int j) const { return M[(size_t)j * q + i] - s(i) * s(j) / n; }
    __device__ bool flat(int i) const { const double t = 32.0 * 2.220446049250313e-16 * fabs(mu(i)); return cen(i, i) <= n * t * t; }
    __device__ double raw(int i, int j) const { return cen(i, j) + n * mu(i) * mu(j); }
};

__global__ __launch_bounds__(256) void finalize_kernel(const double *__restrict__ Mbuf, const double *__restrict__ sums,
                                                        int p, int sem, int standardize, int intercept,
                                                        double *__restrict__ xx, double *__restrict__ xy,
                                                        double *__restrict__ stats)
{
    Mom m; m.M = Mbuf; m.sums = sums; m.p = p; m.q = p + 2; m.n = Mbuf[(size_t)(p + 1) * (p + 2) + (p + 1)];
    {
        __shared__ int need_sh;
        if (threadIdx.x == 0) need_sh = 0;
        __syncthreads();
        if (sums) for (int j = threadIdx.x; j <= p; j += blockDim.x) if (column_needs_shift(sums, p, j)) need_sh = 1;
        __syncthreads();
        m.shift = need_sh != 0;
    }
    const double n = m.n;
    const int tid = blockIdx.x * blockDim.x + threadIdx.x, nth = gridDim.x * blockDim.x;
    __shared__ int advise;
    if (threadIdx.x == 0) advise = 0;
    __syncthreads();
    if (!sums && sem == OEMGPU_SEM_DENSE && blockIdx.x == 0) {
        const int q = p + 2;
        for (int j = threadIdx.x; j <= p; j += blockDim.x) {
            const double mean = Mbuf[(size_t)j * q + (p + 1)] / n;
            double var = Mbuf[(size_t)j * q + j] / n - mean * mean;
            if (!(var > 0.0)) var = 0.0;
            if (mean * mean > 256.0 * var) advise = 1;
        }
        __syncthreads();
    }
    if (tid == 0) { stats[stats_shift_flag(p)] = m.shift ? 1.0 : 0.0; stats[stats_shift_flag(p) + 1] = advise ? 1.0 : 0.0; }
    if (sem == OEMGPU_SEM_DENSE) {
        const int flag = (standardize ? 1 : 0) + 2 * (intercept ? 1 : 0);
        double meany = 0.0, scaley = 1.0, yy;
        const double cyy = fmax(m.cen(p, p), 0.0);
        if (flag == 1) { scaley = sqrt(cyy) / sqrt(n); yy = m.raw(p, p) / (scaley * scaley); }
        else if (flag >= 2) { meany = m.mu(p); scaley = sqrt(cyy) * (1.0 / sqrt(n)); yy = cyy / (scaley * scaley); }
        else yy = m.raw(p, p);
        if (tid == 0) { stats[0] = meany; stats[1] = scaley; stats[2] = yy; stats[3] = n; }
        for (int idx = tid; idx < p * p; idx += nth) {
            const int i = idx % p, j = idx / p;
            double si = 1.0, sj = 1.0;
            const bool fi = m.flat(i), fj = m.flat(j);
            if (flag & 1) {
                si = (flag == 1) ? sqrt(fmax(m.cen(i, i), 0.0)) / sqrt(n) : sqrt(fmax(m.cen(i, i), 0.0)) * (1.0 / sqrt(n));
                sj = (flag == 1) ? sqrt(fmax(m.cen(j, j), 0.0)) / sqrt(n) : sqrt(fmax(m.cen(j, j), 0.0)) * (1.0 / sqrt(n));
                if (si == 0.0 || fi) si = 1.0;
                if (sj == 0.0 || fj) sj = 1.0;
            }
            const double g = (flag >= 2) ? ((fi || fj) ? 0.0 : m.cen(i, j)) : m.raw(i, j);
            xx[(size_t)j * p + i] = g / (si * sj) / n;
            if (i == 0) {
                const double gy = (flag >= 2) ? (fj ? 0.0 : m.cen(j, p)) : m.raw(j, p);
                xy[j] = gy / (sj * scaley) / n;
                stats[4 + j] = (flag >= 2) ? m.mu(j) : 0.0;
                stats[4 + p + j] = sj;
            }
        }
    } else {
        const int off = intercept ? 1 : 0, qq = p + off;
        if (tid == 0) { stats[0] = 0.0; stats[1] = 1.0; stats[2] = m.raw(p, p); stats[3] = n; }
        for (int idx = tid; idx < p * p; idx += nth) {
            const int i = idx % p, j = idx / p;
            double ci = 1.0, cj = 1.0;
            if (standardize) {
                double a = m.raw(i, i) / (n - 1.0), b = m.raw(j, j) / (n - 1.0);
                if (a == 0.0) a = 1.0;
                if (b == 0.0) b = 1.0;
                ci = 1.0 / sqrt(a); cj = 1.0 / sqrt(b);
            }
            xx[(size_t)(j + off) * qq + (i + off)] = ci * m.raw(i, j) * cj / n;
            if (i == 0) {
                xy[j + off] = m.raw(j, p) * cj / n;
                stats[4 + j] = 0.0;
                stats[4 + p + j] = cj;
                if (intercept) {
                    const double cs = n * m.mu(j) * cj / n;
                    xx[(size_t)(j + 1) * qq] = cs;
                    xx[(size_t)(j + 1)] = cs;
                }
            }
        }
        if (tid == 0 && intercept) { xx[0] = 1.0; xy[0] = n * m.mu(p) / n; }
    }
}

int launch_finalize(hipStream_t s, const double *moments, const double *sums, int p, int sem, int standardize,
                    int intercept, double *xx, double *xy, double *stats)
{
    int blocks = (p * p + 255) / 256;
    if (blocks > 1024) blocks = 1024;
    if (blocks < 1) blocks = 1;
    hipLaunchKernelGGL(finalize_kernel, dim3(blocks), dim3(256), 0, s, moments, sums, p, sem, standardize, intercept, xx,
                       xy, stats);
    OEM_HIP(hipGetLastError());
    return 0;
}

__global__ __launch_bounds__(256) void xtx_prepare_kernel(const double *__restrict__ xtx, const double *__restrict__ xty,
                                                           const double *__restrict__ sinv, int p,
                                                           double *__restrict__ xx, double *__restrict__ xy,
                                                           double *__restrict__ stats)
{
    const size_t tid = (size_t)blockIdx.x * blockDim.x + threadIdx.x, nth = (size_t)gridDim.x * blockDim.x;
    for (size_t idx = tid; idx < (size_t)p * p; idx += nth) {
        const int i = (int)(idx % p), j = (int)(idx / p);
        xx[idx] = sinv ? sinv[i] * xtx[idx] * sinv[j] : xtx[idx];
        if (i == 0) xy[j] = sinv ? xty[j] * sinv[j] : xty[j];
    }
    if (tid == 0) { stats[0] = 0.0; stats[1] = 1.0; stats[2] = 0.0; stats[3] = 1.0; stats[stats_shift_flag(p)] = 0.0; stats[stats_shift_flag(p) + 1] = 0.0; }
}

int launch_xtx_prepare(hipStream_t s, const double *xtx, const double *xty, const double *sf_inv, int p, double *xx,
                       double *xy, double *stats)
{
    size_t blocks = ((size_t)p * p + 255) / 256;
    if (blocks > 2048) blocks = 2048;
    hipLaunchKernelGGL(xtx_prepare_kernel, dim3((unsigned)blocks), dim3(256), 0, s, xtx, xty, sf_inv, p, xx, xy, stats);
    OEM_HIP(hipGetLastError());
    return 0;
}

}
```

### oem_amd/csrc/gram_dev.hpp

```cpp
#pragma once
#include <type_traits>
#include "common.hpp"

namespace oemgpu {

__device__ __forceinline__ bool column_needs_shift(const double *__restrict__ sums, int p, int j)
{
    const double cnt = sums[p + 1], m = sums[j] / cnt;
    double var = sums[p + 2 + j] / cnt - m * m;
    if (!(var > 0.0)) var = 0.0;
    return m * m > 256.0 * var;
}
__device__ __forceinline__ bool shift_needed_wave(const double *__restrict__ sums, int p)
{
    if (!sums) return false;
    bool need = false;
    for (int j = threadIdx.x & 63; j <= p; j += 64) need |= column_needs_shift(sums, p, j);
    return __any(need);
}

#include "gen/acc_tiles.inc"

template <int N, typename F> __device__ __forceinline__ void static_for(F &&f)
{
    if constexpr (N > 0) {
        static_for<N - 1>(f);
        f(std::integral_constant<int, N - 1>{});
    }
}

typedef const double __attribute__((address_space(1))) *gptr_t;
typedef const v2d __attribute__((address_space(1))) *gptr2_t;

template <int NF> struct Slab {
    v2d v[NF];
    v2d y;
};

template <int NF, bool ALIGNED, bool MASKED, bool LOADY>
__device__ __forceinline__ void load_slab(Slab<NF> &s, const gptr_t (&ptr)[NF], gptr_t y, int64_t r, int64_t n)
{
    if (!MASKED) {
        if (ALIGNED) {
#pragma unroll
            for (int f = 0; f < NF; ++f) s.v[f] = *(gptr2_t)(ptr[f] + r);
            if (LOADY) s.y = *(gptr2_t)(y + r);
        } else {
#pragma unroll
            for (int f = 0; f < NF; ++f) { s.v[f].x = ptr[f][r]; s.v[f].y = ptr[f][r + 1]; }
            if (LOADY) { s.y.x = y[r]; s.y.y = y[r + 1]; }
        }
    } else {
        const int64_t r0 = r < n ? r : n - 1, r1 = r + 1 < n ? r + 1 : n - 1;
#pragma unroll
        for (int f = 0; f < NF; ++f) { s.v[f].x = ptr[f][r0]; s.v[f].y = ptr[f][r1]; }
        if (LOADY) { s.y.x = y[r0]; s.y.y = y[r1]; }
    }
}

template <int OFF> __device__ __forceinline__ void gload16(v2d &dst, gptr_t p)
{
    asm volatile("global_load_dwordx4 %0, %1, off offset:%2" : "=v"(dst) : "v"(p), "i"(OFF * 8) : "memory");
}
template <int OFF> __device__ __forceinline__ double gload8(gptr_t p)
{
    double dst;
    asm volatile("global_load_dwordx2 %0, %1, off offset:%2" : "=v"(dst) : "v"(p), "i"(OFF * 8) : "memory");
    return dst;
}
template <int NF, bool ALIGNED, bool LOADY> struct SlabLoads { static constexpr int N = (ALIGNED ? 1 : 2) * (NF + (LOADY ? 1 : 0)); };

template <int NF, bool ALIGNED, bool LOADY, int OFF>
__device__ __forceinline__ void load_slab_asm(Slab<NF> &s, const gptr_t (&ptr)[NF], gptr_t y)
{
    if (ALIGNED) {
#pragma unroll
        for (int f = 0; f < NF; ++f) gload16<OFF>(s.v[f], ptr[f]);
        if (LOADY) gload16<OFF>(s.y, y);
    } else {
#pragma unroll
        for (int f = 0; f < NF; ++f) { s.v[f].x = gload8<OFF>(ptr[f]); s.v[f].y = gload8<OFF + 1>(ptr[f]); }
        if (LOADY) { s.y.x = gload8<OFF>(y); s.y.y = gload8<OFF + 1>(y); }
    }
}
template <int NF, int PENDING> __device__ __forceinline__ void wait_slab(Slab<NF> &s)
{
    asm volatile("s_waitcnt vmcnt(%0)" ::"i"(PENDING) : "memory");
#pragma unroll
    for (int f = 0; f < NF; ++f) asm volatile("" : "+v"(s.v[f]));
    asm volatile("" : "+v"(s.y));
    __builtin_amdgcn_sched_barrier(0);
}

__device__ __forceinline__ void set_m0(unsigned lds_byte_addr)
{
    asm volatile("s_mov_b32 m0, %0\n\ts_nop 0" ::"s"(lds_byte_addr) : "memory");
}
#ifndef OEM_GLDS_POLICY
#define OEM_GLDS_POLICY ""
#endif
template <int OFFB> __device__ __forceinline__ void glds_v(gptr_t src)
{
    asm volatile("global_load_lds_dwordx4 %0, off offset:%1" OEM_GLDS_POLICY ::"v"(src), "i"(OFFB) : "memory");
}
template <int OFFB> __device__ __forceinline__ void glds_s(unsigned voff, gptr_t sbase)
{
    asm volatile("global_load_lds_dwordx4 %0, %1 offset:%2" OEM_GLDS_POLICY ::"v"(voff), "s"(sbase), "i"(OFFB) : "memory");
}
template <int PENDING> __device__ __forceinline__ void wait_vm()
{
    asm volatile("s_waitcnt vmcnt(%0)" ::"i"(PENDING) : "memory");
}

template <int NF> struct VecAcc {
    double sx[NF], sxy[NF];
    double sy, syy;
};

template <int NF> struct LaneXf {
    double c[NF];
    double m_last, o_last;
};

struct NoHook { template <typename M> __device__ __forceinline__ void operator()(M) const {} };


__device__ __forceinline__ double shfl_xor_d(double v, int m)
{
    return __shfl_xor(v, m, 64);
}

struct GramDims {
    int64_t n; int64_t ld; int p;
    int ntc, ntile, nblk, nchunk, steps;
};

int launch_gram_sb(hipStream_t s, const GramPlan &pl, const double *x, const double *y, const double *sums, double *tpart, double *vpart, const GramDims &a);
int launch_gram_wd(hipStream_t s, const GramPlan &pl, const double *x, const double *y, const double *sums, double *tpart, double *vpart, const GramDims &a);
constexpr int SB_KINDS = 7;

}
```

Measured before the change: 2039 solves/s.

## Fuse moments reduction with finalize into one kernel for the tri gram plan

Adds a fused kernel that reduces the per-chunk Gram partials and directly writes the finalized xx/xy/stats, so the separate moments-reduce and finalize launches are skipped on the dense column-major path. The solve then uses the pre-finalized frame instead of re-running finalize. This cuts one kernel launch and a round trip through the moments buffer per fit. In exchange it adds a more complex per-tile kernel, a flag-clearing write inside the gram kernel, and a new selftest entry point.

```diff
diff --git a/include/oemgpu.h b/include/oemgpu.h
--- a/include/oemgpu.h
+++ b/include/oemgpu.h
@@ -279,6 +279,10 @@
     OEMGPU_GRAM_FORM_BLK = 7
 };
 int oemgpu_selftest_gram_form(int64_t n, int64_t ld, int32_t p, int32_t aligned, int32_t num_cu, int64_t *out );
+
+int oemgpu_selftest_fused_finalize(oemgpu_ctx *c, const double *x_dev, int64_t n, int64_t ld, int32_t p, const double *y_dev, const double *sums_dev,
+                                   int32_t semantics, int32_t standardize, int32_t intercept, int32_t fused,
+                                   double *moments_dev, double *xx_dev, double *xy_dev, double *stats_dev);
 
 int oemgpu_fit_logistic_dense(const double *x, int64_t n, int32_t p, const double *y, int32_t standardize, int32_t intercept,
                               int32_t hessian_full, int32_t irls_maxit, double irls_tol, const oemgpu_opts *opts,
diff --git a/oem_amd/_lib.py b/oem_amd/_lib.py
--- a/oem_amd/_lib.py
+++ b/oem_amd/_lib.py
@@ -210,6 +210,8 @@
     "oemgpu_selftest_wcoop_sizing": (C.c_int, [C.c_int32, C.c_int32, C.c_int32, C.c_int32]),
     "oemgpu_selftest_gram_plan": (C.c_int, [C.c_int64, C.c_int32, C.c_int32, C.POINTER(C.c_int64)]),
     "oemgpu_selftest_gram_form": (C.c_int, [C.c_int64, C.c_int64, C.c_int32, C.c_int32, C.c_int32, C.POINTER(C.c_int64)]),
+    "oemgpu_selftest_fused_finalize": (C.c_int, [C.c_void_p, C.c_void_p, C.c_int64, C.c_int64, C.c_int32, C.c_void_p, C.c_void_p, C.c_int32, C.c_int32,
+                                                 C.c_int32, C.c_int32, C.c_void_p, C.c_void_p, C.c_void_p, C.c_void_p]),
     "oemgpu_selftest_plan": (C.c_int, [C.c_int32, C.c_int32, C.c_int32, C.c_int32, C.c_void_p, C.c_int32, C.c_int32, C.c_int64, C.c_int32,
                              C.POINTER(C.c_int32), C.POINTER(C.c_int64), C.POINTER(C.c_int64), C.POINTER(C.c_int64), C.POINTER(C.c_int64)]),
     "oemgpu_reload_switches": (None, []),
diff --git a/oem_amd/csrc/api.hip b/oem_amd/csrc/api.hip
--- a/oem_amd/csrc/api.hip
+++ b/oem_amd/csrc/api.hip
@@ -199,13 +199,14 @@
 }
 
 int shard_moments(oemgpu_ctx *c, const GramPlan &pl, const double *x, int64_t n, int64_t ld, const double *y,
-                  const double *sums, double *tpart, double *vpart, double *moments)
+                  const double *sums, double *tpart, double *vpart, double *moments, const FusedFinal *ff)
 {
     {
         Timer t(c, OEMGPU_T_GRAMK);
-        int rc = launch_gram(c->stream, pl, x, n, ld, y, sums, tpart, vpart);
+        int rc = launch_gram(c->stream, pl, x, n, ld, y, sums, tpart, vpart, ff ? ff->stats + stats_shift_flag(pl.p) + 1 : nullptr);
         if (rc) return rc;
     }
+    if (ff) return launch_moments_fused(c->stream, pl, tpart, sums, ff->sem, ff->standardize, ff->intercept, moments, ff->xx, ff->xy, ff->stats);
     return launch_moments_reduce(c->stream, pl, tpart, vpart, moments);
 }
 
@@ -266,13 +267,14 @@
 }
 
 int dense_src_moments(oemgpu_ctx *c, const MomentPlan &pl, const DenseSrc &X, int64_t n, const double *y, const double *sums, char *scratch,
-                      double *moments)
+                      double *moments, const FusedFinal *ff)
 {
     double *tpart = (double *)scratch;
     if (X.colmajor()) {
         Bump B; B.take(pl.cm.tpart_doubles * 8);
-        return shard_moments(c, pl.cm, X.cm(), n, X.ld, y, sums, tpart, (double *)(scratch + B.off), moments);
-    }
+        return shard_moments(c, pl.cm, X.cm(), n, X.ld, y, sums, tpart, (double *)(scratch + B.off), moments, ff);
+    }
+    if (ff) { set_error("internal: no fused finalize behind the row-major pass"); return OEMGPU_ERR_INTERNAL; }
     {
         Timer t(c, OEMGPU_T_GRAMK);
         int rc = launch_gram_rm(c->stream, pl.rm, X.x, X.dtype, n, X.ld, y, sums, tpart);
@@ -424,6 +426,26 @@
     return 0;
 }
 
+int oemgpu_selftest_fused_finalize(oemgpu_ctx *c, const double *x_dev, int64_t n, int64_t ld, int32_t p, const double *y_dev, const double *sums_dev,
+                                   int32_t semantics, int32_t standardize, int32_t intercept, int32_t fused,
+                                   double *moments_dev, double *xx_dev, double *xy_dev, double *stats_dev)
+{
+    if (!c || !x_dev || !y_dev || !moments_dev || !xx_dev || !xy_dev || !stats_dev || n < 1 || p < 1 || ld < n) { set_error("selftest_fused_finalize: bad argument"); return OEMGPU_ERR_ARG; }
+    if (semantics != OEMGPU_SEM_DENSE && semantics != OEMGPU_SEM_BIG && semantics != OEMGPU_SEM_XVAL) { set_error("unknown semantics %d", semantics); return OEMGPU_ERR_ARG; }
+    if (set_device(c)) return OEMGPU_ERR_HIP;
+    const GramPlan pl = gram_plan(n, p, c->num_cu);
+    if (fused && !moments_fused_ok(pl)) { set_error("selftest_fused_finalize: %lld x %d is no plan of the fused launch (or OEM_NO_FUSED is set)", (long long)n, p); return OEMGPU_ERR_UNSUPPORTED; }
+    Bump B;
+    const size_t a_t = B.take(pl.tpart_doubles * 8), a_v = B.take(pl.vpart_doubles * 8);
+    if (ctx_reserve(c, B.off)) return OEMGPU_ERR_HIP;
+    const FusedFinal ff{semantics, standardize, intercept, xx_dev, xy_dev, stats_dev};
+    int rc = shard_moments(c, pl, x_dev, n, ld, y_dev, sums_dev, (double *)(c->ws + a_t), (double *)(c->ws + a_v), moments_dev, fused ? &ff : nullptr);
+    if (!rc && !fused) rc = launch_finalize(c->stream, moments_dev, sums_dev, p, semantics, standardize, intercept, xx_dev, xy_dev, stats_dev);
+    if (rc) return rc;
+    OEM_HIP(hipStreamSynchronize(c->stream));
+    return 0;
+}
+
 int oemgpu_selftest_hold_cus(oemgpu_ctx *c, int32_t blocks, double ms)
 {
     if (!c || blocks < 1 || blocks > 4096 || !(ms > 0.0) || ms > 30000.0) { set_error("hold_cus: bad argument"); return OEMGPU_ERR_ARG; }
@@ -536,10 +558,21 @@
                            const oemgpu_opts *o, double *beta, double *lambda_out, int32_t *niter, double *loss, double *d,
                            const WideArgs *wd, const double *lmax_xy);
 
+struct SolveFrame { size_t a_xx, a_xy, a_st, bytes; };
+static SolveFrame solve_frame(int p, int q)
+{
+    Bump B;
+    SolveFrame F;
+    F.a_xx = B.take((size_t)q * q * 8); F.a_xy = B.take((size_t)q * 8); F.a_st = B.take((size_t)stats_len(p) * 8);
+    F.bytes = B.off;
+    return F;
+}
+
 static int solve_moments_impl(oemgpu_ctx *c, const double *moments_dev, const double *sums_dev, int32_t p,
                               int32_t semantics, int32_t standardize, int32_t intercept, const oemgpu_opts *o,
                               double *beta, double *lambda_out, int32_t *niter, double *loss, double *d, const double *wpatch,
-                              const PathExtras *ex = nullptr, const double *lmax_xy = nullptr, size_t extra_ws = 0, double *big_xy_std = nullptr);
+                              const PathExtras *ex = nullptr, const double *lmax_xy = nullptr, size_t extra_ws = 0, double *big_xy_std = nullptr,
+                              const double *finalized_xx = nullptr);
 
 int oemgpu_solve_moments_dev(oemgpu_ctx *c, const double *moments_dev, const double *sums_dev, int32_t p,
                              int32_t semantics, int32_t standardize, int32_t intercept, const oemgpu_opts *o,
@@ -551,7 +584,7 @@
 static int solve_moments_impl(oemgpu_ctx *c, const double *moments_dev, const double *sums_dev, int32_t p,
                               int32_t semantics, int32_t standardize, int32_t intercept, const oemgpu_opts *o,
                               double *beta, double *lambda_out, int32_t *niter, double *loss, double *d, const double *wpatch,
-                              const PathExtras *ex, const double *lmax_xy, size_t extra_ws, double *big_xy_std)
+                              const PathExtras *ex, const double *lmax_xy, size_t extra_ws, double *big_xy_std, const double *finalized_xx)
 {
     if (!c || !moments_dev || !beta || !lambda_out || !niter || !loss || !d) { set_error("solve_moments: NULL argument"); return OEMGPU_ERR_ARG; }
     if (semantics != OEMGPU_SEM_DENSE && semantics != OEMGPU_SEM_BIG && semantics != OEMGPU_SEM_XVAL) { set_error("unknown semantics %d", semantics); return OEMGPU_ERR_ARG; }
@@ -563,8 +596,9 @@
         return OEMGPU_ERR_UNSUPPORTED;
     }
     if (set_device(c)) return OEMGPU_ERR_HIP;
-    Bump B;
-    const size_t a_xx = B.take((size_t)q * q * 8), a_xy = B.take((size_t)q * 8), a_st = B.take((size_t)stats_len(p) * 8);
+    const SolveFrame F = solve_frame(p, q);
+    Bump B; B.off = F.bytes;
+    const size_t a_xx = F.a_xx, a_xy = F.a_xy, a_st = F.a_st;
     size_t base = 0;
     if ((const char *)moments_dev >= c->ws && (const char *)moments_dev < c->ws + c->ws_bytes)
         base = ((const char *)moments_dev - c->ws) + (size_t)oemgpu_moments_len(p) * 8;
@@ -580,7 +614,10 @@
     }
     Bump B2; B2.off = base + B.off;
     double *xx = (double *)(c->ws + base + a_xx), *xy = (double *)(c->ws + base + a_xy), *st = (double *)(c->ws + base + a_st);
-    {
+    if (finalized_xx) {
+        if (finalized_xx != xx || wpatch || big_xy_std) { set_error("internal: finalized moments outside the solve's frame"); return OEMGPU_ERR_INTERNAL; }
+        c->ev_used[OEMGPU_T_FINAL] = false;
+    } else {
         Timer t(c, OEMGPU_T_FINAL);
         const bool plain = wpatch || big_xy_std;
         rc = launch_finalize(c->stream, moments_dev, sums_dev, p, semantics, plain ? 0 : standardize, plain ? 0 : intercept, xx, xy, st);
@@ -792,16 +829,23 @@
     Bump B;
     const size_t a_sums = B.take((size_t)oemgpu_sums_len(p) * 8), a_mom = B.take((size_t)oemgpu_moments_len(p) * 8);
     const size_t frame = B.off;
+    const bool fuse = X.colmajor() && moments_fused_ok(pl.cm);
+    const SolveFrame F = solve_frame(p, p);
+    if (fuse) B.off += F.bytes;
     const size_t a_scr = B.take(pl.scratch_bytes);
     if (ctx_reserve(c, moments_solve_ws(frame, B.off, p, o))) return OEMGPU_ERR_HIP;
     double *sums = (double *)(c->ws + a_sums), *mom = (double *)(c->ws + a_mom);
+    FusedFinal ff{OEMGPU_SEM_DENSE, standardize, intercept, (double *)(c->ws + frame + F.a_xx), (double *)(c->ws + frame + F.a_xy),
+                  (double *)(c->ws + frame + F.a_st)};
+    const FusedFinal *ffp = fuse ? &ff : nullptr;
     {
         Timer t(c, OEMGPU_T_MOMENTS);
-        rc = dense_src_moments(c, pl, X, n, y_dev, nullptr, c->ws + a_scr, mom);
+        rc = dense_src_moments(c, pl, X, n, y_dev, nullptr, c->ws + a_scr, mom, ffp);
         if (rc) return rc;
     }
     HT(1);
-    rc = oemgpu_solve_moments_dev(c, mom, nullptr, p, OEMGPU_SEM_DENSE, standardize, intercept, o, beta, lambda_out, niter, loss, d);
+    rc = solve_moments_impl(c, mom, nullptr, p, OEMGPU_SEM_DENSE, standardize, intercept, o, beta, lambda_out, niter, loss, d, nullptr, nullptr, nullptr, 0,
+                            nullptr, fuse ? ff.xx : nullptr);
 #ifdef OEM_HOST_TIMING
     HT(5); g_ht.acc[0] += g_tp[1] - g_tp[0]; g_ht.acc[1] += g_tp[2] - g_tp[1]; g_ht.acc[2] += g_tp[3] - g_tp[2]; g_ht.acc[3] += g_tp[4] - g_tp[3]; g_ht.acc[4] += g_tp[5] - g_tp[4]; ++g_ht.n;
 #endif
@@ -813,10 +857,11 @@
     }
     {
         Timer t(c, OEMGPU_T_MOMENTS);
-        rc = dense_src_moments(c, pl, X, n, y_dev, sums, c->ws + a_scr, mom);
+        rc = dense_src_moments(c, pl, X, n, y_dev, sums, c->ws + a_scr, mom, ffp);
         if (rc) return rc;
     }
-    return oemgpu_solve_moments_dev(c, mom, sums, p, OEMGPU_SEM_DENSE, standardize, intercept, o, beta, lambda_out, niter, loss, d);
+    return solve_moments_impl(c, mom, sums, p, OEMGPU_SEM_DENSE, standardize, intercept, o, beta, lambda_out, niter, loss, d, nullptr, nullptr, nullptr, 0,
+                              nullptr, fuse ? ff.xx : nullptr);
 }
 
 int oemgpu_fit_dense_dev(oemgpu_ctx *c, const double *x_dev, int64_t n, int64_t ld, int32_t p, const double *y_dev,
diff --git a/oem_amd/csrc/common.hpp b/oem_amd/csrc/common.hpp
--- a/oem_amd/csrc/common.hpp
+++ b/oem_amd/csrc/common.hpp
@@ -49,7 +49,8 @@
 
 int launch_shift_sums(hipStream_t s, const double *x, int64_t n, int64_t ld, int p, const double *y, double *sums);
 int launch_gram(hipStream_t s, const GramPlan &pl, const double *x, int64_t n, int64_t ld, const double *y,
-                const double *sums , double *tpart, double *vpart);
+                const double *sums , double *tpart, double *vpart,
+                double *clear = nullptr );
 int launch_moments_reduce(hipStream_t s, const GramPlan &pl, const double *tpart, const double *vpart, double *moments);
 
 constexpr int GRAM_RM_P_MAX = 1024;
@@ -77,9 +78,13 @@
                     int intercept, double *xx , double *xy , double *stats);
 int launch_xtx_prepare(hipStream_t s, const double *xtx, const double *xty, const double *sf_inv , int p,
                        double *xx, double *xy, double *stats);
+struct FusedFinal { int sem, standardize, intercept; double *xx, *xy, *stats; };
+bool moments_fused_ok(const GramPlan &pl);
+int launch_moments_fused(hipStream_t s, const GramPlan &pl, const double *tpart, const double *sums, int sem, int standardize, int intercept,
+                         double *moments, double *xx, double *xy, double *stats);
 
 int shard_moments(oemgpu_ctx *c, const GramPlan &pl, const double *x, int64_t n, int64_t ld, const double *y, const double *sums,
-                  double *tpart, double *vpart, double *moments);
+                  double *tpart, double *vpart, double *moments, const FusedFinal *ff = nullptr);
 int launch_moments_add(hipStream_t s, double *acc, const double *m, size_t len, bool first);
 
 int64_t csc_check(const char *who, int64_t n, int p, const int64_t *colptr, const int32_t *rowidx, const double *values,
diff --git a/oem_amd/csrc/dense_src.hpp b/oem_amd/csrc/dense_src.hpp
--- a/oem_amd/csrc/dense_src.hpp
+++ b/oem_amd/csrc/dense_src.hpp
@@ -25,6 +25,6 @@
 };
 int dense_src_moment_plan(const char *who, const oemgpu_ctx *c, const DenseSrc &X, int64_t n, int32_t p, MomentPlan *pl);
 int dense_src_moments(oemgpu_ctx *c, const MomentPlan &pl, const DenseSrc &X, int64_t n, const double *y, const double *sums, char *scratch,
-                      double *moments);
+                      double *moments, const FusedFinal *ff = nullptr);
 
 }
diff --git a/oem_amd/csrc/gram.hip b/oem_amd/csrc/gram.hip
--- a/oem_amd/csrc/gram.hip
+++ b/oem_amd/csrc/gram.hip
@@ -641,6 +641,7 @@
 {
     extern __shared__ __attribute__((aligned(16))) double lds[];
     const int chunk = blockIdx.x;
+    if (a.clear && chunk == 0 && threadIdx.x == 0) *a.clear = 0.0;
     gram_body<NT, NT, true, ALIGNED, false, true>(x, a.n, a.ld, a.p, y, sums, a.ntc, 0, 0,
                                                   (int64_t)chunk * a.steps * 64, a.steps, true,
                                                   tpart + (size_t)chunk * a.ntile * 256, vpart, lds);
@@ -654,6 +655,7 @@
     extern __shared__ __attribute__((aligned(16))) double lds[];
     (void)vpart;
     const int chunk = blockIdx.x;
+    if (a.clear && chunk == 0 && threadIdx.x == 0) *a.clear = 0.0;
     if (shift_needed_wave(sums, a.p))
         gram_tri_ring_body<NT, true, 0, SADDR>(x, a.n, a.ld, a.p, y, sums, (int64_t)chunk * a.steps * 64, a.steps,
                                                tpart + (size_t)chunk * a.ntile * 256, lds);
@@ -875,10 +877,10 @@
 }
 
 int launch_gram(hipStream_t s, const GramPlan &pl, const double *x, int64_t n, int64_t ld, const double *y,
-                const double *sums, double *tpart, double *vpart)
+                const double *sums, double *tpart, double *vpart, double *clear)
 {
     GramDims a;
-    a.n = n; a.ld = ld; a.p = pl.p;
+    a.n = n; a.ld = ld; a.p = pl.p; a.clear = pl.tri ? clear : nullptr;
     a.ntc = pl.ntc; a.ntile = pl.ntile; a.nblk = pl.nblk; a.nchunk = pl.nchunk; a.steps = pl.steps;
     const bool aligned = (((uintptr_t)x | (uintptr_t)y) & 15) == 0 && (ld & 1) == 0;
     return aligned ? launch_gram_t<true>(s, pl, x, y, sums, tpart, vpart, a)
@@ -1008,23 +1010,111 @@
     return 0;
 }
 
-struct Mom {
-    const double *M; const double *sums; int p, q; double n;
+struct MomBuf {
+    const double *M; int q;
+    __device__ __forceinline__ double at(int i, int j) const { return M[(size_t)j * q + i]; }
+};
+template <class Src>
+struct MomT {
+    Src M; const double *sums; int p; double n;
     bool shift;
-    __device__ double c(int j) const { return shift ? sums[j] / sums[p + 1] : 0.0; }
-    __device__ double s(int j) const { return M[(size_t)j * q + (p + 1)]; }
-    __device__ double mu(int j) const { return c(j) + s(j) / n; }
-    __device__ double cen(int i, int j) const { return M[(size_t)j * q + i] - s(i) * s(j) / n; }
-    __device__ bool flat(int i) const { const double t = 32.0 * 2.220446049250313e-16 * fabs(mu(i)); return cen(i, i) <= n * t * t; }
-    __device__ double raw(int i, int j) const { return cen(i, j) + n * mu(i) * mu(j); }
+    __device__ __forceinline__ double c(int j) const { return shift ? sums[j] / sums[p + 1] : 0.0; }
+    __device__ __forceinline__ double s(int j) const { return M.at(p + 1, j); }
+    __device__ __forceinline__ double mu(int j) const { return c(j) + s(j) / n; }
+    __device__ __forceinline__ double cen(int i, int j) const { return M.at(i, j) - s(i) * s(j) / n; }
+    __device__ __forceinline__ bool flat(int i) const { const double t = 32.0 * 2.220446049250313e-16 * fabs(mu(i)); return cen(i, i) <= n * t * t; }
+    __device__ __forceinline__ double raw(int i, int j) const { return cen(i, j) + n * mu(i) * mu(j); }
 };
+using Mom = MomT<MomBuf>;
+
+__device__ __forceinline__ bool column_advises_shift(double sj, double djj, double n)
+{
+    const double mean = sj / n;
+    double var = djj / n - mean * mean;
+    if (!(var > 0.0)) var = 0.0;
+    return mean * mean > 256.0 * var;
+}
+
+template <class MM>
+__device__ __forceinline__ void fin_dense_y(const MM &m, int flag, double &meany, double &scaley, double &yy)
+{
+    const int p = m.p;
+    const double n = m.n;
+    meany = 0.0; scaley = 1.0;
+    const double cyy = fmax(m.cen(p, p), 0.0);
+    if (flag == 1) { scaley = sqrt(cyy) / sqrt(n); yy = m.raw(p, p) / (scaley * scaley); }
+    else if (flag >= 2) { meany = m.mu(p); scaley = sqrt(cyy) * (1.0 / sqrt(n)); yy = cyy / (scaley * scaley); }
+    else yy = m.raw(p, p);
+}
+template <class MM>
+__device__ __forceinline__ double fin_dense_scale(const MM &m, int flag, int i, bool fi)
+{
+    const double n = m.n;
+    double si = 1.0;
+    if (flag & 1) {
+        si = (flag == 1) ? sqrt(fmax(m.cen(i, i), 0.0)) / sqrt(n) : sqrt(fmax(m.cen(i, i), 0.0)) * (1.0 / sqrt(n));
+        if (si == 0.0 || fi) si = 1.0;
+    }
+    return si;
+}
+template <class MM>
+__device__ __forceinline__ void fin_dense_xx(const MM &m, int flag, int i, int j, double *__restrict__ xx)
+{
+    const bool fi = m.flat(i), fj = m.flat(j);
+    const double si = fin_dense_scale(m, flag, i, fi), sj = fin_dense_scale(m, flag, j, fj);
+    const double g = (flag >= 2) ? ((fi || fj) ? 0.0 : m.cen(i, j)) : m.raw(i, j);
+    xx[(size_t)j * m.p + i] = g / (si * sj) / m.n;
+}
+template <class MM>
+__device__ __forceinline__ void fin_dense_col(const MM &m, int flag, int j, double scaley, double *__restrict__ xy, double *__restrict__ stats)
+{
+    const int p = m.p;
+    const bool fj = m.flat(j);
+    const double sj = fin_dense_scale(m, flag, j, fj);
+    const double gy = (flag >= 2) ? (fj ? 0.0 : m.cen(j, p)) : m.raw(j, p);
+    xy[j] = gy / (sj * scaley) / m.n;
+    stats[4 + j] = (flag >= 2) ? m.mu(j) : 0.0;
+    stats[4 + p + j] = sj;
+}
+template <class MM>
+__device__ __forceinline__ double fin_big_scale(const MM &m, int standardize, int i)
+{
+    double ci = 1.0;
+    if (standardize) {
+        double a = m.raw(i, i) / (m.n - 1.0);
+        if (a == 0.0) a = 1.0;
+        ci = 1.0 / sqrt(a);
+    }
+    return ci;
+}
+template <class MM>
+__device__ __forceinline__ void fin_big_xx(const MM &m, int standardize, int off, int i, int j, double *__restrict__ xx)
+{
+    const double ci = fin_big_scale(m, standardize, i), cj = fin_big_scale(m, standardize, j);
+    xx[(size_t)(j + off) * (m.p + off) + (i + off)] = ci * m.raw(i, j) * cj / m.n;
+}
+template <class MM>
+__device__ __forceinline__ void fin_big_col(const MM &m, int standardize, int off, int j, double *__restrict__ xx, double *__restrict__ xy,
+                                            double *__restrict__ stats)
+{
+    const int p = m.p;
+    const double n = m.n, cj = fin_big_scale(m, standardize, j);
+    xy[j + off] = m.raw(j, p) * cj / n;
+    stats[4 + j] = 0.0;
+    stats[4 + p + j] = cj;
+    if (off) {
+        const double cs = n * m.mu(j) * cj / n;
+        xx[(size_t)(j + 1) * (p + off)] = cs;
+        xx[(size_t)(j + 1)] = cs;
+    }
+}
 
 __global__ __launch_bounds__(256) void finalize_kernel(const double *__restrict__ Mbuf, const double *__restrict__ sums,
                                                         int p, int sem, int standardize, int intercept,
                                                         double *__restrict__ xx, double *__restrict__ xy,
                                                         double *__restrict__ stats)
 {
-    Mom m; m.M = Mbuf; m.sums = sums; m.p = p; m.q = p + 2; m.n = Mbuf[(size_t)(p + 1) * (p + 2) + (p + 1)];
+    Mom m; m.M.M = Mbuf; m.M.q = p + 2; m.sums = sums; m.p = p; m.n = Mbuf[(size_t)(p + 1) * (p + 2) + (p + 1)];
     {
         __shared__ int need_sh;
         if (threadIdx.x == 0) need_sh = 0;
@@ -1040,65 +1130,28 @@
     __syncthreads();
     if (!sums && sem == OEMGPU_SEM_DENSE && blockIdx.x == 0) {
         const int q = p + 2;
-        for (int j = threadIdx.x; j <= p; j += blockDim.x) {
-            const double mean = Mbuf[(size_t)j * q + (p + 1)] / n;
-            double var = Mbuf[(size_t)j * q + j] / n - mean * mean;
-            if (!(var > 0.0)) var = 0.0;
-            if (mean * mean > 256.0 * var) advise = 1;
-        }
+        for (int j = threadIdx.x; j <= p; j += blockDim.x)
+            if (column_advises_shift(Mbuf[(size_t)j * q + (p + 1)], Mbuf[(size_t)j * q + j], n)) advise = 1;
         __syncthreads();
     }
     if (tid == 0) { stats[stats_shift_flag(p)] = m.shift ? 1.0 : 0.0; stats[stats_shift_flag(p) + 1] = advise ? 1.0 : 0.0; }
     if (sem == OEMGPU_SEM_DENSE) {
         const int flag = (standardize ? 1 : 0) + 2 * (intercept ? 1 : 0);
-        double meany = 0.0, scaley = 1.0, yy;
-        const double cyy = fmax(m.cen(p, p), 0.0);
-        if (flag == 1) { scaley = sqrt(cyy) / sqrt(n); yy = m.raw(p, p) / (scaley * scaley); }
-        else if (flag >= 2) { meany = m.mu(p); scaley = sqrt(cyy) * (1.0 / sqrt(n)); yy = cyy / (scaley * scaley); }
-        else yy = m.raw(p, p);
+        double meany, scaley, yy;
+        fin_dense_y(m, flag, meany, scaley, yy);
         if (tid == 0) { stats[0] = meany; stats[1] = scaley; stats[2] = yy; stats[3] = n; }
         for (int idx = tid; idx < p * p; idx += nth) {
             const int i = idx % p, j = idx / p;
-            double si = 1.0, sj = 1.0;
-            const bool fi = m.flat(i), fj = m.flat(j);
-            if (flag & 1) {
-                si = (flag == 1) ? sqrt(fmax(m.cen(i, i), 0.0)) / sqrt(n) : sqrt(fmax(m.cen(i, i), 0.0)) * (1.0 / sqrt(n));
-                sj = (flag == 1) ? sqrt(fmax(m.cen(j, j), 0.0)) / sqrt(n) : sqrt(fmax(m.cen(j, j), 0.0)) * (1.0 / sqrt(n));
-                if (si == 0.0 || fi) si = 1.0;
-                if (sj == 0.0 || fj) sj = 1.0;
-            }
-            const double g = (flag >= 2) ? ((fi || fj) ? 0.0 : m.cen(i, j)) : m.raw(i, j);
-            xx[(size_t)j * p + i] = g / (si * sj) / n;
-            if (i == 0) {
-                const double gy = (flag >= 2) ? (fj ? 0.0 : m.cen(j, p)) : m.raw(j, p);
-                xy[j] = gy / (sj * scaley) / n;
-                stats[4 + j] = (flag >= 2) ? m.mu(j) : 0.0;
-                stats[4 + p + j] = sj;
-            }
+            fin_dense_xx(m, flag, i, j, xx);
+            if (i == 0) fin_dense_col(m, flag, j, scaley, xy, stats);
         }
     } else {
-        const int off = intercept ? 1 : 0, qq = p + off;
+        const int off = intercept ? 1 : 0;
         if (tid == 0) { stats[0] = 0.0; stats[1] = 1.0; stats[2] = m.raw(p, p); stats[3] = n; }
         for (int idx = tid; idx < p * p; idx += nth) {
             const int i = idx % p, j = idx / p;
-            double ci = 1.0, cj = 1.0;
-            if (standardize) {
-                double a = m.raw(i, i) / (n - 1.0), b = m.raw(j, j) / (n - 1.0);
-                if (a == 0.0) a = 1.0;
-                if (b == 0.0) b = 1.0;
-                ci = 1.0 / sqrt(a); cj = 1.0 / sqrt(b);
-            }
-            xx[(size_t)(j + off) * qq + (i + off)] = ci * m.raw(i, j) * cj / n;
-            if (i == 0) {
-                xy[j + off] = m.raw(j, p) * cj / n;
-                stats[4 + j] = 0.0;
-                stats[4 + p + j] = cj;
-                if (intercept) {
-                    const double cs = n * m.mu(j) * cj / n;
-                    xx[(size_t)(j + 1) * qq] = cs;
-                    xx[(size_t)(j + 1)] = cs;
-                }
-            }
+            fin_big_xx(m, standardize, off, i, j, xx);
+            if (i == 0) fin_big_col(m, standardize, off, j, xx, xy, stats);
         }
         if (tid == 0 && intercept) { xx[0] = 1.0; xy[0] = n * m.mu(p) / n; }
     }
@@ -1116,6 +1169,157 @@
     return 0;
 }
 
+constexpr int FB_R = 4, FB_C = 8, FB_NB = (16 / FB_R) * (16 / FB_C);
+constexpr int FB_ONES_C = FB_R * FB_C, FB_ONES_R = FB_ONES_C + FB_C, FB_DIAG_C = FB_ONES_R + FB_R, FB_DIAG_R = FB_DIAG_C + FB_C,
+              FB_N = FB_DIAG_R + FB_R, FB_NSLOT = FB_N + 1;
+__host__ __device__ constexpr int fused_threads(int ng)
+{
+    return ((FB_NSLOT * ng + 1) / 2 + 63) / 64 * 64 < 192 ? 192 : ((FB_NSLOT * ng + 1) / 2 + 63) / 64 * 64;
+}
+
+struct MomBlock {
+    const double *v; int row0, col0, p;
+    __device__ __forceinline__ double ones(int k) const { return (k >= col0 && k < col0 + FB_C) ? v[FB_ONES_C + k - col0] : v[FB_ONES_R + k - row0]; }
+    __device__ __forceinline__ double diag(int k) const { return (k >= col0 && k < col0 + FB_C) ? v[FB_DIAG_C + k - col0] : v[FB_DIAG_R + k - row0]; }
+    __device__ __forceinline__ double at(int i, int j) const
+    {
+        if (i == p + 1 || j == p + 1) return i == j ? v[FB_N] : ones(i == p + 1 ? j : i);
+        if (i == j) return diag(i);
+        const int row = i > j ? i : j, col = i > j ? j : i;
+        return v[(row - row0) * FB_C + (col - col0)];
+    }
+};
+
+__device__ __forceinline__ int tri_index(int a, int b) { return a * (a + 1) / 2 + b; }
+
+template <int NG>
+__global__ __launch_bounds__(fused_threads(NG)) void moments_fused_kernel(const double *__restrict__ tpart, const double *__restrict__ sums,
+                                                                          int p, int ntile, int nchunk, int sem, int standardize,
+                                                                          int intercept, double *__restrict__ M, double *__restrict__ xx,
+                                                                          double *__restrict__ xy, double *__restrict__ stats)
+{
+    constexpr int NTH = fused_threads(NG), NTASK = FB_NSLOT * NG;
+    __shared__ double part[NG][FB_NSLOT];
+    __shared__ double val[FB_NSLOT];
+    const int q = p + 2;
+    const int tile = blockIdx.x / FB_NB, b = blockIdx.x % FB_NB;
+    int I = (int)((sqrtf(8.0f * (float)tile + 1.0f) - 1.0f) * 0.5f);
+    while (I * (I + 1) / 2 > tile) --I;
+    while ((I + 1) * (I + 2) / 2 <= tile) ++I;
+    const int J = tile - I * (I + 1) / 2;
+    const int r0 = (b / (16 / FB_C)) * FB_R, c0 = (b % (16 / FB_C)) * FB_C;
+    const int row0 = 16 * I + r0, col0 = 16 * J + c0;
+    if (row0 >= q || col0 >= q || row0 + FB_R - 1 < col0) return;
+    const int Tn = (p + 1) >> 4, ln = (p + 1) & 15;
+    const size_t stride = (size_t)ntile * 256;
+    double ld[2][16];
+    int grp[2];
+    bool use[2];
+#pragma unroll
+    for (int k = 0; k < 2; ++k) {
+        const int t = threadIdx.x + k * NTH, s = t % FB_NSLOT;
+        grp[k] = t / FB_NSLOT;
+        int tl, el;
+        bool ok;
+        if (s < FB_ONES_C) {
+            const int r = r0 + s / FB_C, c = c0 + s % FB_C;
+            tl = tile; el = 16 * r + c; ok = 16 * I + r < q && 16 * J + c < q && 16 * I + r >= 16 * J + c;
+        } else if (s < FB_ONES_R) { const int c = c0 + s - FB_ONES_C; tl = tri_index(Tn, J); el = 16 * ln + c; ok = 16 * J + c < q; }
+        else if (s < FB_DIAG_C) { const int r = r0 + s - FB_ONES_R; tl = tri_index(Tn, I); el = 16 * ln + r; ok = 16 * I + r < q; }
+        else if (s < FB_DIAG_R) { const int c = c0 + s - FB_DIAG_C; tl = tri_index(J, J); el = 17 * c; ok = 16 * J + c < q; }
+        else if (s < FB_N) { const int r = r0 + s - FB_DIAG_R; tl = tri_index(I, I); el = 17 * r; ok = 16 * I + r < q; }
+        else { tl = tri_index(Tn, Tn); el = 17 * ln; ok = true; }
+        use[k] = ok && t < NTASK;
+        const double *src = tpart + (size_t)tl * 256 + el;
+#pragma unroll
+        for (int u = 0; u < 16; ++u) {
+            const int c = grp[k] + NG * u;
+            ld[k][u] = src[(size_t)(c < nchunk ? c : nchunk - 1) * stride];
+        }
+    }
+    int need = 0;
+    if (sums) for (int j = threadIdx.x; j <= p; j += NTH) need |= column_needs_shift(sums, p, j);
+#pragma unroll
+    for (int k = 0; k < 2; ++k) {
+        const int t = threadIdx.x + k * NTH;
+        double s = 0.0;
+#pragma unroll
+        for (int u = 0; u < 16; ++u) if (grp[k] + NG * u < nchunk) s += ld[k][u];
+        if (t < NTASK) part[grp[k]][t % FB_NSLOT] = use[k] ? s : 0.0;
+    }
+    const bool shift = __syncthreads_or(need) != 0;
+    if (threadIdx.x < FB_NSLOT) {
+        double t[NG];
+#pragma unroll
+        for (int g = 0; g < NG; ++g) t[g] = part[g][threadIdx.x];
+#pragma unroll
+        for (int h = 1; h < NG; h <<= 1)
+#pragma unroll
+            for (int g = 0; g + h < NG; g += 2 * h) t[g] += t[g + h];
+        val[threadIdx.x] = t[0];
+    }
+    __syncthreads();
+    const int w = threadIdx.x >> 6, lane = threadIdx.x & 63;
+    if (w > 2) return;
+    MomT<MomBlock> m;
+    m.M.v = val; m.M.row0 = row0; m.M.col0 = col0; m.M.p = p; m.sums = sums; m.p = p; m.n = val[FB_N]; m.shift = shift;
+    const bool advising = !sums && sem == OEMGPU_SEM_DENSE;
+    const int flag = (standardize ? 1 : 0) + 2 * (intercept ? 1 : 0), off = intercept ? 1 : 0;
+    if (w == 0) {
+        const int slot = lane % FB_ONES_C, swapped = lane / FB_ONES_C;
+        const int row = row0 + slot / FB_C, col = col0 + slot % FB_C;
+        if (row >= q || col >= q || row < col) return;
+        const double v = val[slot];
+        if (swapped) M[(size_t)row * q + col] = v; else M[(size_t)col * q + row] = v;
+        if (advising && swapped && row == col && row <= p && column_advises_shift(m.M.ones(row), v, m.n)) stats[stats_shift_flag(p) + 1] = 1.0;
+        if (row >= p || (swapped && row == col)) return;
+        const int i = swapped ? col : row, j = swapped ? row : col;
+        if (sem == OEMGPU_SEM_DENSE) fin_dense_xx(m, flag, i, j, xx); else fin_big_xx(m, standardize, off, i, j, xx);
+        return;
+    }
+    if (p < row0 || p >= row0 + FB_R) return;
+    if (w == 1) {
+        const int col = col0 + lane;
+        if (lane >= FB_C || col >= p) return;
+        if (sem == OEMGPU_SEM_DENSE) {
+            double meany, scaley, yy;
+            fin_dense_y(m, flag, meany, scaley, yy);
+            fin_dense_col(m, flag, col, scaley, xy, stats);
+        } else fin_big_col(m, standardize, off, col, xx, xy, stats);
+        return;
+    }
+    if (lane != 0 || p < col0 || p >= col0 + FB_C) return;
+    stats[stats_shift_flag(p)] = m.shift ? 1.0 : 0.0;
+    if (!advising) stats[stats_shift_flag(p) + 1] = 0.0;
+    if (sem == OEMGPU_SEM_DENSE) {
+        double meany, scaley, yy;
+        fin_dense_y(m, flag, meany, scaley, yy);
+        stats[0] = meany; stats[1] = scaley; stats[2] = yy; stats[3] = m.n;
+    } else {
+        stats[0] = 0.0; stats[1] = 1.0; stats[2] = m.raw(p, p); stats[3] = m.n;
+        if (intercept) { xx[0] = 1.0; xy[0] = m.n * m.mu(p) / m.n; }
+    }
+}
+
+bool moments_fused_ok(const GramPlan &pl)
+{
+    return pl.tri && pl.nchunk <= 16 * (pl.nchunk >= 64 ? 16 : 4) && !sw().OEM_NO_FUSED.set;
+}
+
+int launch_moments_fused(hipStream_t s, const GramPlan &pl, const double *tpart, const double *sums, int sem, int standardize, int intercept,
+                         double *moments, double *xx, double *xy, double *stats)
+{
+    if (!moments_fused_ok(pl)) { set_error("internal: the fused reduce + finalize does not take this plan"); return OEMGPU_ERR_INTERNAL; }
+    if (pl.nchunk >= 64)
+        hipLaunchKernelGGL(moments_fused_kernel<16>, dim3(pl.ntile * FB_NB), dim3(fused_threads(16)), 0, s, tpart, sums, pl.p, pl.ntile, pl.nchunk,
+                           sem, standardize, intercept, moments, xx, xy, stats);
+    else
+        hipLaunchKernelGGL(moments_fused_kernel<4>, dim3(pl.ntile * FB_NB), dim3(fused_threads(4)), 0, s, tpart, sums, pl.p, pl.ntile, pl.nchunk,
+                           sem, standardize, intercept, moments, xx, xy, stats);
+    OEM_HIP(hipGetLastError());
+    return 0;
+}
+
 __global__ __launch_bounds__(256) void xtx_prepare_kernel(const double *__restrict__ xtx, const double *__restrict__ xty,
                                                            const double *__restrict__ sinv, int p,
                                                            double *__restrict__ xx, double *__restrict__ xy,
diff --git a/oem_amd/csrc/gram_dev.hpp b/oem_amd/csrc/gram_dev.hpp
--- a/oem_amd/csrc/gram_dev.hpp
+++ b/oem_amd/csrc/gram_dev.hpp
@@ -133,6 +133,7 @@
 struct GramDims {
     int64_t n; int64_t ld; int p;
     int ntc, ntile, nblk, nchunk, steps;
+    double *clear = nullptr;
 };
 
 int launch_gram_sb(hipStream_t s, const GramPlan &pl, const double *x, const double *y, const double *sums, double *tpart, double *vpart, const GramDims &a);
```

After: 2048 solves/s, median of 6. No clear change (+0.4%).
